# blachlylab/fade

Hardware: NVIDIA B200
Metric: annotate_reads_per_sec (higher is better)
Workload: dtype int16

## Files before the change

fade_b200/csrc/fadegpu.cu:

```cuda
#include <cuda_runtime.h>
#include <algorithm>
#include <cstdio>
#include <cstdlib>
#include <cstring>
#include <new>
#include <chrono>
#include <condition_variable>
#include <deque>
#include <functional>
#include <exception>
#include <mutex>
#include <thread>
#include <string>
#include <vector>
#ifdef _OPENMP
#include <omp.h>
#endif
#include "../../include/fadegpu.h"
#include "kernels.cuh"

using namespace fade;

static_assert(FADEGPU_MAX_OPS == OPS_CAP, "ABI ops capacity must match the kernels");
static_assert(sizeof(AlnOut) == 32 + 4 * OPS_CAP, "AlnOut layout");
static_assert(sizeof(AlnDesc) == 40, "AlnDesc layout");
static_assert(sizeof(PairResult) == sizeof(fadegpu_pair_result) && sizeof(fadegpu_pair_result) == 32, "fadegpu_pair_result layout");
static_assert(PAIR_R_OVERSIZE == FADEGPU_R_OVERSIZE, "oversize flag");

static thread_local std::string g_last_error;

constexpr int MAX_SETS = 4;

struct fadegpu_ctx {
    int device = 0;
    cudaStream_t stream = nullptr;
    fadegpu_params p{};
    SwConsts k{};
    int32_t n_contigs = 0;
    std::vector<std::string> names;
    std::vector<int64_t> clen, coff;
    int64_t total_bases = 0, padded_bases = 0;
    uint32_t *d_two = nullptr, *d_n = nullptr, *d_x = nullptr;
    int64_t *d_xpos = nullptr;
    uint8_t *d_xchr = nullptr;
    int64_t n_x = 0;
    size_t ref_bytes = 0;
    cudaStream_t tstream = nullptr;
    unsigned next_set = 0;
    struct ScratchSet {
        cudaEvent_t ev_fill = nullptr, ev_trace = nullptr;
        bool used = false;
        uint32_t *d_ck = nullptr;
        size_t ck_bytes = 0;
        uint8_t *d_gen = nullptr;
        size_t gen_bytes = 0;
        unsigned int *d_cursor = nullptr;
        uint8_t *d_trace = nullptr;
        size_t trace_bytes = 0;
        unsigned int *d_qcount = nullptr;
    } scratch[MAX_SETS];
    int n_sets = 3;
    uint32_t *d_alu = nullptr;
    int sm_count = 148;
    int host_threads = 1;
    cudaStream_t stream2 = nullptr;
    cudaStream_t stream3 = nullptr;
    int64_t *d_clen = nullptr, *d_coff = nullptr;
    std::string err;
    std::thread worker;
    std::mutex q_mu;
    std::condition_variable q_cv, done_cv;
    std::deque<std::pair<fadegpu_batch *, int64_t>> jobs;
    bool worker_stop = false, worker_busy = false;
    std::mutex submit_mu;
    std::vector<fadegpu_batch *> batches;
    struct PairBufs {
        fadegpu_batch *b = nullptr;
        char *h_stage = nullptr, *d_raw = nullptr;
        size_t stage_bytes = 0, raw_bytes = 0;
        uint32_t *d_two = nullptr, *d_n = nullptr, *d_x = nullptr, *d_chunk_x = nullptr;
        size_t two_bytes = 0, n_bytes = 0, x_bytes = 0, chunk_bytes = 0;
        int64_t *d_xpos = nullptr, *d_clen = nullptr, *d_coff = nullptr;
        size_t xpos_bytes = 0, clen_bytes = 0, coff_bytes = 0;
        uint8_t *d_xchr = nullptr;
        size_t xchr_bytes = 0;
        uint32_t *d_spill = nullptr, *d_ops = nullptr;
        size_t spill_bytes = 0, ops_bytes = 0;
        fadegpu_pair_result *d_res = nullptr;
        size_t res_bytes = 0;
        int32_t *d_bad = nullptr;
    } pairs;
};

struct AlnTmp {
    int64_t start;
    int64_t so;
    int32_t read, tlen, cls, qlen, tid, key;
    uint32_t clip_left, clip_right;
};

struct Launch {
    int R;
    int aln_first, n_aln;
    int item_first, n_items;
    int tw_stride;
    int nblk_max;
    int qmax, tmax;
};

struct fadegpu_batch {
    fadegpu_ctx *ctx = nullptr;
    fadegpu_batch_view v{};
    AlnDesc *h_aln = nullptr, *d_aln = nullptr;
    WarpItem *h_items = nullptr, *d_items = nullptr;
    uint8_t *h_seq = nullptr, *d_seq = nullptr;
    AlnOut *h_out = nullptr, *d_out = nullptr;
    uint32_t *d_flags = nullptr;
    uint2 *d_fillres = nullptr;
    int64_t cap_items = 0, cap_seq = 0;
    std::vector<Launch> plan;
    int64_t n_reads = 0, n_aln = 0, n_items = 0, seq_bytes = 0;
    int qmax_all = 0, tmax_all = 0;
    fadegpu_stats st{};
    cudaEvent_t ev[6] = { nullptr, nullptr, nullptr, nullptr, nullptr, nullptr };
    bool in_flight = false;
    std::vector<std::vector<AlnTmp>> tl_aln;
    std::vector<uint32_t> order;
    int32_t *h_ridx = nullptr;
    std::vector<AlnTmp> all_aln;
    std::vector<int32_t> cnt;
    std::vector<int64_t> soff, aln_start;
    std::vector<int32_t> sorted_tlen;
    bool dev_binning = false;
    uint8_t *d_in_seq4 = nullptr;
    int64_t *d_in_seq_off = nullptr, *d_in_pos = nullptr, *d_start = nullptr, *d_aln_start = nullptr;
    int32_t *d_in_lq = nullptr, *d_in_tid = nullptr, *d_in_alen = nullptr, *d_in_cl = nullptr, *d_in_cr = nullptr;
    int32_t *d_key = nullptr, *d_tlen = nullptr, *d_hist = nullptr, *d_keybase = nullptr, *d_cursor = nullptr;
    int32_t *d_ridx = nullptr;
    uint8_t *d_rflags = nullptr;
    uint8_t *d_gate = nullptr;
    const uint4 *d_view_meta = nullptr;
    int32_t *d_over = nullptr, *h_over = nullptr;
    unsigned long long *d_stats = nullptr;
    int32_t *h_hist = nullptr, *h_keybase = nullptr;
    unsigned long long *h_stats = nullptr;
    int64_t *h_aln_start = nullptr;
    uint8_t *h_c_seq4 = nullptr;
    int64_t *h_c_seq_off = nullptr, *h_c_pos = nullptr;
    int32_t *h_c_lq = nullptr, *h_c_tid = nullptr, *h_c_alen = nullptr, *h_c_cl = nullptr, *h_c_cr = nullptr, *h_c_read = nullptr;
    int32_t *d_in_read = nullptr;
    int64_t n_c = 0, seq_c = 0;
    bool pulled = false;
    int64_t *d_src_off = nullptr;
    const uint8_t *d_view_seq4 = nullptr;
    std::vector<int32_t> idx;
    BinArgs ba{};
    bool ba_valid = false;
    AlnDesc *d_aln_scratch = nullptr;
    int64_t *d_i64_scratch = nullptr;
    cudaEvent_t ev_prep = nullptr, ev_ready = nullptr;
    int mode = 0;
    int64_t job_seq_bytes = 0;
    cudaEvent_t ev_kernels = nullptr;
    bool queued = false;
    int submit_rc = 0;
    std::string submit_err;
};

extern "C" { static void drain_submits(fadegpu_ctx *c); }

namespace {

std::mutex g_err_mu;

int fail(fadegpu_ctx *ctx, int code, const std::string &msg)
{
    std::lock_guard<std::mutex> g(g_err_mu);
    if (ctx) ctx->err = msg;
    g_last_error = msg;
    return code;
}

int cuda_fail(fadegpu_ctx *ctx, cudaError_t e, const char *what)
{
    std::string m = std::string(what) + ": " + cudaGetErrorString(e);
    return fail(ctx, e == cudaErrorMemoryAllocation ? FADEGPU_E_OOM : FADEGPU_E_CUDA, m);
}

#define CU(ctx, call)                                              \
    do {                                                           \
        cudaError_t e__ = (call);                                  \
        if (e__ != cudaSuccess) return cuda_fail(ctx, e__, #call); \
    } while (0)

template <typename T>
void free_host(T *&p) { if (p) cudaFreeHost(p); p = nullptr; }
template <typename T>
void free_dev(T *&p) { if (p) cudaFree(p); p = nullptr; }

void free_reference(fadegpu_ctx *c)
{
    free_dev(c->d_two); free_dev(c->d_n); free_dev(c->d_x); free_dev(c->d_xpos); free_dev(c->d_xchr);
    free_dev(c->d_clen); free_dev(c->d_coff);
    c->n_x = 0; c->ref_bytes = 0; c->n_contigs = 0; c->total_bases = c->padded_bases = 0;
    c->names.clear(); c->clen.clear(); c->coff.clear();
}

int upload_contig_tables(fadegpu_ctx *c)
{
    const size_t nb = std::max<size_t>(1, (size_t)c->n_contigs) * sizeof(int64_t);
    CU(c, cudaMalloc(&c->d_clen, nb)); CU(c, cudaMalloc(&c->d_coff, nb));
    if (c->n_contigs > 0) {
        CU(c, cudaMemcpy(c->d_clen, c->clen.data(), (size_t)c->n_contigs * 8, cudaMemcpyHostToDevice));
        CU(c, cudaMemcpy(c->d_coff, c->coff.data(), (size_t)c->n_contigs * 8, cudaMemcpyHostToDevice));
    }
    return 0;
}

RefDev ref_dev(const fadegpu_ctx *c)
{
    RefDev r;
    r.planes.two = c->d_two; r.planes.nmask = c->d_n; r.planes.xmask = c->d_x;
    r.xpos = c->d_xpos; r.xchr = c->d_xchr; r.n_x = c->n_x;
    return r;
}

int cls_rank(int cls)
{
    for (int k = 0; k < N_ROW_CLASSES; ++k) if (ROW_CLASSES[k] == cls) return k;
    return N_ROW_CLASSES;
}

int class_of(const fadegpu_ctx *c, int qlen, int tlen)
{
    if (c->p.flags & FADEGPU_F_FORCE_GENERIC) return 0;
    if (qlen > QMAX_FAST || tlen > TMAX_PACKED) return 0;
    for (int k = 0; k < N_ROW_CLASSES; ++k) if (qlen <= FG * ROW_CLASSES[k]) return ROW_CLASSES[k];
    return 0;
}

size_t ck_words_of(int R) { return (size_t)(2 * R + 2); }

int ensure_dev(fadegpu_ctx *c, void **p, size_t *have, size_t bytes)
{
    if (bytes <= *have) return 0;
    if (*p) cudaFree(*p);
    *p = nullptr; *have = 0;
    CU(c, cudaMalloc(p, bytes));
    *have = bytes;
    return 0;
}

size_t align256(size_t x) { return (x + 255) & ~(size_t)255; }

size_t trace_scratch_bytes(int R, int64_t n)
{
    return align256((size_t)n * sizeof(LaneCtl)) + 2 * align256((size_t)n * 8) +
           align256((size_t)((n + 1) / 2) * trace_tile_bytes(R));
}

constexpr int GEN_SLOTS_MAX = 8192;
constexpr size_t GEN_BUDGET = (size_t)4 << 30;

size_t gen_slot_bytes(int qmax, int tmax)
{
    size_t b = (size_t)8 * qmax + (((size_t)qmax + 15) & ~(size_t)15) + (size_t)qmax * tmax;
    return (b + 15) & ~(size_t)15;
}

int build_plan(fadegpu_ctx *c, fadegpu_batch *b, int64_t n_aln, const int64_t *cls_first, const int32_t *sorted_tlen,
               int qmax_all, int tmax_all, int gen_qmax, int gen_tmax)
{
    int64_t n_items = 0;
    size_t ck_needed = 0, gen_needed = 0, trace_needed = 0;
    b->plan.clear();
    b->st.n_generic = 0;
    for (int rk = 0; rk <= N_ROW_CLASSES; ++rk) {
        const int R = rk < N_ROW_CLASSES ? ROW_CLASSES[rk] : 0;
        const int64_t first_aln = cls_first[rk], last_aln = cls_first[rk + 1];
        if (last_aln <= first_aln) continue;
        if (R == 0) {
            Launch L{};
            L.R = 0; L.aln_first = (int)first_aln; L.n_aln = (int)(last_aln - first_aln); L.qmax = gen_qmax; L.tmax = gen_tmax;
            b->plan.push_back(L);
            gen_needed = std::max(gen_needed, gen_slot_bytes(gen_qmax, gen_tmax));
            b->st.n_generic += last_aln - first_aln;
            continue;
        }
        const size_t cw = ck_words_of(R);
        int64_t a0 = first_aln;
        while (a0 < last_aln) {
            Launch L{};
            L.R = R; L.aln_first = (int)a0; L.item_first = (int)n_items; L.qmax = qmax_all; L.tmax = tmax_all;
            size_t words = 0;
            int nblk_max = 1;
            int64_t a1 = a0;
            while (a1 < last_aln) {
                const int nblk = num_blocks(sorted_tlen[a1]);
                const size_t wds = (size_t)(nblk - 1) * cw * 32;
                if (a1 > a0 && (words + wds) * 4 > (size_t)c->p.scratch_bytes) break;
                if (n_items >= b->cap_items) return fail(c, FADEGPU_E_STATE, "fadegpu_submit: internal error (item capacity)");
                WarpItem &it = b->h_items[n_items++];
                it.ck_off = (int64_t)words;
                it.first = (int32_t)(a1 - a0);
                it.nblk = (int16_t)nblk;
                it.pad = 0;
                it.nsteps = sorted_tlen[a1] + FG - 1;
                words += wds;
                nblk_max = std::max(nblk_max, nblk);
                a1 = std::min<int64_t>(a1 + 8, last_aln);
            }
            L.n_aln = (int)(a1 - a0);
            L.n_items = (int)(n_items - L.item_first);
            L.tw_stride = tw_stride_for(nblk_max);
            L.nblk_max = nblk_max;
            ck_needed = std::max(ck_needed, words * 4);
            trace_needed = std::max(trace_needed, trace_scratch_bytes(R, L.n_aln));
            b->plan.push_back(L);
            a0 = a1;
        }
    }
    b->n_aln = n_aln; b->n_items = n_items;
    b->qmax_all = qmax_all; b->tmax_all = tmax_all;
    b->st.n_aligned = n_aln;
    b->st.scratch_bytes = (int64_t)ck_needed;
    if (n_aln > 0) gen_needed = std::max(gen_needed, gen_slot_bytes(qmax_all, tmax_all));
    for (int l = 0; l < (b->plan.empty() ? 0 : c->n_sets); ++l) {
        fadegpu_ctx::ScratchSet &ln = c->scratch[l];
        if (ck_needed) { int rc = ensure_dev(c, (void **)&ln.d_ck, &ln.ck_bytes, ck_needed); if (rc) return rc; }
        if (trace_needed) { int rc = ensure_dev(c, (void **)&ln.d_trace, &ln.trace_bytes, trace_needed); if (rc) return rc; }
        if (gen_needed) {
            const size_t want = std::min<size_t>(GEN_BUDGET, gen_needed * 1024);
            int rc = ensure_dev(c, (void **)&ln.d_gen, &ln.gen_bytes, std::max(want, gen_needed));
            if (rc) return rc;
        }
    }
    return 0;
}

struct PlanTarget {
    RefDev ref;
    int tags_only;
    uint32_t *ops_spill;
    int ops_cap;
};

PlanTarget batch_target(const fadegpu_ctx *c)
{
    return PlanTarget{ ref_dev(c), (c->p.flags & FADEGPU_F_TAGS_ONLY) ? 1 : 0, nullptr, 0 };
}

int run_plan(fadegpu_ctx *c, fadegpu_batch *b, const PlanTarget &pt, float *fill_ms, float *trace_ms, float *gen_ms,
             int *launches, cudaEvent_t dep)
{
    const bool timed = fill_ms != nullptr;
    cudaEvent_t e0 = nullptr, e1 = nullptr, e2 = nullptr;
    if (timed) {
        CU(c, cudaEventCreate(&e0)); CU(c, cudaEventCreate(&e1)); CU(c, cudaEventCreate(&e2));
        *fill_ms = *trace_ms = *gen_ms = 0.f;
    }
    int nl = 0;
    cudaStream_t sf = c->stream, st = c->tstream;
    if (dep) CU(c, cudaStreamWaitEvent(sf, dep, 0));
    for (const Launch &L : b->plan) {
        fadegpu_ctx::ScratchSet &ln = c->scratch[c->next_set++ % (unsigned)c->n_sets];
        if (ln.used) CU(c, cudaStreamWaitEvent(sf, ln.ev_trace, 0));
        ln.used = true;
        const uint8_t *seq = b->dev_binning ? b->d_in_seq4 : b->d_seq;
        if (L.R != 0) {
            KernelArgs a;
            a.aln = b->d_aln + L.aln_first;
            a.n_aln = L.n_aln;
            a.items = b->d_items + L.item_first;
            a.n_items = L.n_items;
            a.seq = seq;
            a.ref = pt.ref;
            a.ck = ln.d_ck;
            a.fillres = b->d_fillres + (size_t)L.item_first * 32;
            a.aln_flags = b->d_flags + L.aln_first;
            a.out = b->d_out + L.aln_first;
            a.k = c->k;
            a.min_length = c->p.min_length;
            a.tw_stride = L.tw_stride;
            {
                uint8_t *p = ln.d_trace;
                a.state = reinterpret_cast<LaneCtl *>(p); p += align256((size_t)L.n_aln * sizeof(LaneCtl));
                a.queue[0] = reinterpret_cast<unsigned long long *>(p); p += align256((size_t)L.n_aln * 8);
                a.queue[1] = reinterpret_cast<unsigned long long *>(p); p += align256((size_t)L.n_aln * 8);
                a.tiles = reinterpret_cast<uint32_t *>(p);
                a.qcount = ln.d_qcount;
                a.round = 0;
                a.max_rounds = L.nblk_max + FG;
                a.tags_only = pt.tags_only;
            }
            a.ops_spill = pt.ops_spill ? pt.ops_spill + (size_t)L.aln_first * pt.ops_cap : nullptr;
            a.ops_cap = pt.ops_cap;
            CU(c, cudaMemsetAsync(a.aln_flags, 0, (size_t)L.n_aln * sizeof(uint32_t), sf));
            CU(c, cudaMemsetAsync(ln.d_qcount, 0, 2 * sizeof(unsigned int), sf));
            if (timed) CU(c, cudaEventRecord(e0, sf));
            CU(c, launch_fill(L.R, a, sf));
            if (timed) CU(c, cudaEventRecord(e1, sf));
            CU(c, cudaEventRecord(ln.ev_fill, sf));
            CU(c, cudaStreamWaitEvent(st, ln.ev_fill, 0));
            nl += 1;
            CU(c, launch_trace(L.R, a, st, c->sm_count, &nl));
            GenericArgs ga;
            ga.aln = a.aln; ga.n_aln = L.n_aln; ga.aln_flags = a.aln_flags; ga.seq = a.seq; ga.ref = a.ref;
            ga.out = a.out; ga.cursor = ln.d_cursor; ga.scratch = ln.d_gen;
            ga.qmax = L.qmax; ga.tmax = L.tmax;
            ga.slot_bytes = (int64_t)gen_slot_bytes(L.qmax, L.tmax);
            ga.n_slots = (int)std::max<size_t>(1, std::min<size_t>(GEN_SLOTS_MAX, ln.gen_bytes / (size_t)ga.slot_bytes));
            ga.chunk = 64;
            ga.open = c->p.gap_open; ga.extend = c->p.gap_extend; ga.match = c->p.match; ga.mismatch = c->p.mismatch;
            ga.min_length = c->p.min_length; ga.tags_only = pt.tags_only;
            ga.ops_spill = a.ops_spill; ga.ops_cap = a.ops_cap;
            if (timed) CU(c, cudaEventRecord(e2, st));
            CU(c, cudaMemsetAsync(ln.d_cursor, 0, sizeof(unsigned int), st));
            CU(c, launch_generic(ga, ga.n_slots, st));
            nl += 1;
            if (timed) {
                cudaEvent_t e3;
                CU(c, cudaEventCreate(&e3));
                CU(c, cudaEventRecord(e3, st));
                CU(c, cudaEventSynchronize(e3));
                float t;
                cudaEventElapsedTime(&t, e0, e1); *fill_ms += t;
                cudaEventElapsedTime(&t, e1, e2); *trace_ms += t;
                cudaEventElapsedTime(&t, e2, e3); *gen_ms += t;
                cudaEventDestroy(e3);
            }
            CU(c, cudaEventRecord(ln.ev_trace, st));
        } else {
            GenericArgs ga;
            ga.aln = b->d_aln + L.aln_first; ga.n_aln = L.n_aln; ga.aln_flags = nullptr; ga.seq = seq;
            ga.ref = pt.ref; ga.out = b->d_out + L.aln_first; ga.cursor = ln.d_cursor; ga.scratch = ln.d_gen;
            ga.qmax = L.qmax; ga.tmax = L.tmax;
            ga.slot_bytes = (int64_t)gen_slot_bytes(L.qmax, L.tmax);
            ga.n_slots = (int)std::max<size_t>(1, std::min<size_t>(GEN_SLOTS_MAX, ln.gen_bytes / (size_t)ga.slot_bytes));
            ga.n_slots = std::min(ga.n_slots, std::max(L.n_aln, 1));
            ga.chunk = 1;
            ga.open = c->p.gap_open; ga.extend = c->p.gap_extend; ga.match = c->p.match; ga.mismatch = c->p.mismatch;
            ga.min_length = c->p.min_length; ga.tags_only = pt.tags_only;
            ga.ops_spill = pt.ops_spill ? pt.ops_spill + (size_t)L.aln_first * pt.ops_cap : nullptr;
            ga.ops_cap = pt.ops_cap;
            CU(c, cudaEventRecord(ln.ev_fill, sf));
            CU(c, cudaStreamWaitEvent(st, ln.ev_fill, 0));
            if (timed) CU(c, cudaEventRecord(e0, st));
            CU(c, cudaMemsetAsync(ln.d_cursor, 0, sizeof(unsigned int), st));
            CU(c, launch_generic(ga, ga.n_slots, st));
            nl += 1;
            if (timed) {
                CU(c, cudaEventRecord(e1, st));
                CU(c, cudaEventSynchronize(e1));
                float t;
                cudaEventElapsedTime(&t, e0, e1); *gen_ms += t;
            }
            CU(c, cudaEventRecord(ln.ev_trace, st));
        }
    }
    if (timed) { cudaEventDestroy(e0); cudaEventDestroy(e1); cudaEventDestroy(e2); }
    CU(c, cudaEventRecord(b->ev[5], sf));
    CU(c, cudaEventRecord(b->ev_kernels, b->plan.empty() ? sf : st));
    if (launches) *launches = nl;
    return 0;
}

int join_kernels(fadegpu_ctx *c, fadegpu_batch *b, cudaStream_t s)
{
    CU(c, cudaStreamWaitEvent(s, b->ev_kernels, 0));
    return 0;
}

}

extern "C" {

int fadegpu_abi_version(void) { return FADEGPU_ABI_VERSION; }

int fadegpu_device_count(int *n)
{
    if (!n) return fail(nullptr, FADEGPU_E_ARG, "fadegpu_device_count: null argument");
    int c = 0;
    cudaError_t e = cudaGetDeviceCount(&c);
    if (e != cudaSuccess) { *n = 0; return cuda_fail(nullptr, e, "cudaGetDeviceCount"); }
    *n = c;
    return FADEGPU_OK;
}

int fadegpu_default_params(fadegpu_params *p)
{
    if (!p) return fail(nullptr, FADEGPU_E_ARG, "fadegpu_default_params: null argument");
    p->window_size = 300;
    p->min_length = 5;
    p->gap_open = 10;
    p->gap_extend = 2;
    p->match = 2;
    p->mismatch = -3;
    p->flags = 0;
    p->scratch_bytes = 0;
    p->host_threads = 0;
    p->reserved = 0;
    return FADEGPU_OK;
}

const char *fadegpu_last_error(const fadegpu_ctx *ctx)
{
    static thread_local std::string copy;
    std::lock_guard<std::mutex> g(g_err_mu);
    copy = ctx ? ctx->err : g_last_error;
    return copy.c_str();
}

int fadegpu_create(int device, const fadegpu_params *p, fadegpu_ctx **out)
{
    if (!out) return fail(nullptr, FADEGPU_E_ARG, "fadegpu_create: null out");
    *out = nullptr;
    fadegpu_params pp;
    fadegpu_default_params(&pp);
    if (p) pp = *p;
    if (pp.gap_open < pp.gap_extend || pp.gap_extend <= 0 || pp.match <= 0 || pp.mismatch > 0 ||
        pp.match > 100 || pp.mismatch < -100 || pp.gap_open > 1000 || pp.window_size < 0)
        return fail(nullptr, FADEGPU_E_ARG, "fadegpu_create: unsupported scoring / window parameters");
    setenv("CUDA_DEVICE_MAX_CONNECTIONS", "32", 0);
    int n = 0;
    cudaError_t e = cudaGetDeviceCount(&n);
    if (e != cudaSuccess || n <= 0)
        return fail(nullptr, FADEGPU_E_NODEV, std::string("fadegpu_create: no CUDA device (") +
                                                  (e != cudaSuccess ? cudaGetErrorString(e) : "count 0") + "); there is no CPU fallback");
    if (device < 0 || device >= n) return fail(nullptr, FADEGPU_E_ARG, "fadegpu_create: bad device index");
    fadegpu_ctx *c = new (std::nothrow) fadegpu_ctx();
    if (!c) return fail(nullptr, FADEGPU_E_OOM, "fadegpu_create: out of host memory");
    c->device = device;
    c->p = pp;
    if (c->p.scratch_bytes <= 0) c->p.scratch_bytes = (int64_t)8 << 30;
    {
        int hw = 1;
#ifdef _OPENMP
        hw = std::max(1, omp_get_num_procs());
#endif
        c->host_threads = c->p.host_threads > 0 ? std::min(c->p.host_threads, 4 * hw) : hw;
    }
    c->k = make_consts(pp.gap_open, pp.gap_extend, pp.match, pp.mismatch);
    if (pp.flags & FADEGPU_F_NO_SHORTCUT) c->k.shortcut = 0;
    int prio[4] = { 0, -1, -2, -2 };
    if (const char *pv = getenv("FADEGPU_PRIO")) sscanf(pv, "%d,%d,%d,%d", &prio[0], &prio[1], &prio[2], &prio[3]);
    if ((e = cudaSetDevice(device)) != cudaSuccess || (e = cudaStreamCreateWithPriority(&c->stream, cudaStreamNonBlocking, prio[0])) != cudaSuccess ||
        (e = cudaMalloc(&c->d_alu, 64)) != cudaSuccess ||
        (e = cudaStreamCreateWithPriority(&c->tstream, cudaStreamNonBlocking, prio[1])) != cudaSuccess ||
        (e = cudaStreamCreateWithPriority(&c->stream2, cudaStreamNonBlocking, prio[2])) != cudaSuccess ||
        (e = cudaStreamCreateWithPriority(&c->stream3, cudaStreamNonBlocking, prio[3])) != cudaSuccess ||
        (e = cudaDeviceGetAttribute(&c->sm_count, cudaDevAttrMultiProcessorCount, device)) != cudaSuccess) {
        int rc = cuda_fail(nullptr, e, "fadegpu_create");
        delete c;
        return rc;
    }
    if (const char *ev = getenv("FADEGPU_SCRATCH_SETS")) c->n_sets = std::min(MAX_SETS, std::max(2, atoi(ev)));
    for (int l = 0; l < c->n_sets; ++l) {
        fadegpu_ctx::ScratchSet &ln = c->scratch[l];
        if ((e = cudaEventCreateWithFlags(&ln.ev_fill, cudaEventDisableTiming)) != cudaSuccess ||
            (e = cudaEventCreateWithFlags(&ln.ev_trace, cudaEventDisableTiming)) != cudaSuccess ||
            (e = cudaMalloc(&ln.d_cursor, sizeof(unsigned int))) != cudaSuccess ||
            (e = cudaMalloc(&ln.d_qcount, 2 * sizeof(unsigned int))) != cudaSuccess) {
            int rc = cuda_fail(nullptr, e, "fadegpu_create");
            fadegpu_destroy(c);
            return rc;
        }
    }
    *out = c;
    return FADEGPU_OK;
}

void fadegpu_destroy(fadegpu_ctx *c)
{
    if (!c) return;
    if (c->worker.joinable()) {
        { std::lock_guard<std::mutex> lk(c->q_mu); c->worker_stop = true; }
        c->q_cv.notify_all();
        c->worker.join();
    }
    cudaSetDevice(c->device);
    {
        fadegpu_ctx::PairBufs &pb = c->pairs;
        if (pb.b) fadegpu_free_batch(pb.b);
        free_host(pb.h_stage);
        free_dev(pb.d_raw); free_dev(pb.d_two); free_dev(pb.d_n); free_dev(pb.d_x); free_dev(pb.d_chunk_x);
        free_dev(pb.d_xpos); free_dev(pb.d_xchr); free_dev(pb.d_clen); free_dev(pb.d_coff); free_dev(pb.d_spill);
        free_dev(pb.d_ops); free_dev(pb.d_res); free_dev(pb.d_bad);
    }
    if (c->stream) cudaStreamSynchronize(c->stream);
    if (c->stream2) { cudaStreamSynchronize(c->stream2); cudaStreamDestroy(c->stream2); }
    if (c->stream3) { cudaStreamSynchronize(c->stream3); cudaStreamDestroy(c->stream3); }
    free_reference(c);
    if (c->tstream) { cudaStreamSynchronize(c->tstream); cudaStreamDestroy(c->tstream); }
    for (auto &ln : c->scratch) {
        if (ln.ev_fill) cudaEventDestroy(ln.ev_fill);
        if (ln.ev_trace) cudaEventDestroy(ln.ev_trace);
    }
    for (auto &ln : c->scratch) { free_dev(ln.d_ck); free_dev(ln.d_gen); free_dev(ln.d_cursor); free_dev(ln.d_trace); free_dev(ln.d_qcount); }
    free_dev(c->d_alu);
    if (c->stream) cudaStreamDestroy(c->stream);
    delete c;
}

int fadegpu_load_reference(fadegpu_ctx *c, int32_t n_contigs, const char *const *names,
                           const int64_t *lengths, const char *const *seqs)
{
    if (!c) return fail(nullptr, FADEGPU_E_ARG, "fadegpu_load_reference: null ctx");
    if (n_contigs <= 0 || !lengths || !seqs) return fail(c, FADEGPU_E_ARG, "fadegpu_load_reference: bad arguments");
    drain_submits(c);
    std::lock_guard<std::mutex> submit_guard(c->submit_mu);
    CU(c, cudaSetDevice(c->device));
    { CU(c, cudaStreamSynchronize(c->stream)); CU(c, cudaStreamSynchronize(c->tstream)); }
    free_reference(c);
    c->n_contigs = n_contigs;
    int64_t off = 0, total = 0;
    for (int t = 0; t < n_contigs; ++t) {
        if (lengths[t] < 0 || !seqs[t]) { free_reference(c); return fail(c, FADEGPU_E_ARG, "fadegpu_load_reference: bad contig"); }
        c->names.emplace_back(names && names[t] ? names[t] : "");
        c->clen.push_back(lengths[t]);
        c->coff.push_back(off);
        total += lengths[t];
        off += (lengths[t] + 31) & ~(int64_t)31;
    }
    c->total_bases = total;
    c->padded_bases = off + 32;
    const size_t w2 = (size_t)(c->padded_bases / 16), w1 = (size_t)(c->padded_bases / 32);
    std::vector<uint32_t> two, nm, xm;
    try { two.assign(w2, 0u); nm.assign(w1, 0u); xm.assign(w1, 0u); }
    catch (...) { free_reference(c); return fail(c, FADEGPU_E_OOM, "fadegpu_load_reference: out of host memory"); }
    uint8_t lut[256];
    for (int i = 0; i < 256; ++i) lut[i] = 8;
    lut['A'] = lut['a'] = 0; lut['C'] = lut['c'] = 1; lut['T'] = lut['t'] = 2; lut['G'] = lut['g'] = 3;
    lut['N'] = lut['n'] = 4;
    for (int t = 0; t < n_contigs; ++t) {
        const unsigned char *s = reinterpret_cast<const unsigned char *>(seqs[t]);
        const int64_t len = lengths[t], base = c->coff[t];
        const int64_t nwords = (len + 31) / 32;
#pragma omp parallel for schedule(static) num_threads(std::max(1, c->host_threads))
        for (int64_t wd = 0; wd < nwords; ++wd) {
            uint32_t a0 = 0, a1 = 0, n = 0, x = 0;
            const int64_t p0 = wd * 32;
            const int lim = (int)std::min<int64_t>(32, len - p0);
            for (int b = 0; b < lim; ++b) {
                const uint8_t v = lut[s[p0 + b]];
                const uint32_t code = v & 3u;
                if (b < 16) a0 |= code << (2 * b); else a1 |= code << (2 * (b - 16));
                n |= (uint32_t)((v >> 2) & 1u) << b;
                x |= (uint32_t)((v >> 3) & 1u) << b;
            }
            const size_t gw = (size_t)((base + p0) / 32);
            two[2 * gw] = a0; two[2 * gw + 1] = a1; nm[gw] = n; xm[gw] = x;
        }
    }
    std::vector<int64_t> xpos;
    std::vector<uint8_t> xchr;
    for (int t = 0; t < n_contigs; ++t) {
        const unsigned char *s = reinterpret_cast<const unsigned char *>(seqs[t]);
        const int64_t len = lengths[t], base = c->coff[t];
        for (int64_t wd = 0; wd * 32 < len; ++wd) {
            const uint32_t x = xm[(size_t)((base + wd * 32) / 32)];
            if (!x) continue;
            for (int b = 0; b < 32; ++b)
                if ((x >> b) & 1u) {
                    unsigned char ch = s[wd * 32 + b];
                    if (ch >= 'a' && ch <= 'z') ch = (unsigned char)(ch - 32);
                    xpos.push_back(base + wd * 32 + b);
                    xchr.push_back(ch);
                }
        }
    }
    c->n_x = (int64_t)xpos.size();
    cudaError_t e;
    if ((e = cudaMalloc(&c->d_two, w2 * 4)) != cudaSuccess || (e = cudaMalloc(&c->d_n, w1 * 4)) != cudaSuccess ||
        (e = cudaMalloc(&c->d_x, w1 * 4)) != cudaSuccess ||
        (e = cudaMalloc(&c->d_xpos, std::max<size_t>(1, xpos.size()) * 8)) != cudaSuccess ||
        (e = cudaMalloc(&c->d_xchr, std::max<size_t>(1, xchr.size()))) != cudaSuccess) {
        free_reference(c);
        return cuda_fail(c, e, "fadegpu_load_reference: cudaMalloc");
    }
    CU(c, cudaMemcpy(c->d_two, two.data(), w2 * 4, cudaMemcpyHostToDevice));
    CU(c, cudaMemcpy(c->d_n, nm.data(), w1 * 4, cudaMemcpyHostToDevice));
    CU(c, cudaMemcpy(c->d_x, xm.data(), w1 * 4, cudaMemcpyHostToDevice));
    if (!xpos.empty()) {
        CU(c, cudaMemcpy(c->d_xpos, xpos.data(), xpos.size() * 8, cudaMemcpyHostToDevice));
        CU(c, cudaMemcpy(c->d_xchr, xchr.data(), xchr.size(), cudaMemcpyHostToDevice));
    }
    c->ref_bytes = w2 * 4 + 2 * w1 * 4 + xpos.size() * 9;
    { int rc = upload_contig_tables(c); if (rc) return rc; }
    return FADEGPU_OK;
}

int fadegpu_share_reference(fadegpu_ctx *dst, const fadegpu_ctx *src)
{
    if (!dst || !src) return fail(dst, FADEGPU_E_ARG, "fadegpu_share_reference: null ctx");
    if (!src->d_two) return fail(dst, FADEGPU_E_STATE, "fadegpu_share_reference: source has no reference");
    drain_submits(dst);
    std::lock_guard<std::mutex> submit_guard(dst->submit_mu);
    CU(dst, cudaSetDevice(dst->device));
    { CU(dst, cudaStreamSynchronize(dst->stream)); CU(dst, cudaStreamSynchronize(dst->tstream)); }
    if (dst->device != src->device) {
        int can = 0;
        if (cudaDeviceCanAccessPeer(&can, dst->device, src->device) == cudaSuccess && can) {
            const cudaError_t pe = cudaDeviceEnablePeerAccess(src->device, 0);
            if (pe != cudaSuccess) cudaGetLastError();
        }
    }
    free_reference(dst);
    dst->n_contigs = src->n_contigs; dst->names = src->names; dst->clen = src->clen; dst->coff = src->coff;
    dst->total_bases = src->total_bases; dst->padded_bases = src->padded_bases; dst->n_x = src->n_x;
    const size_t w2 = (size_t)(src->padded_bases / 16), w1 = (size_t)(src->padded_bases / 32);
    const size_t nx = std::max<size_t>(1, (size_t)src->n_x);
    CU(dst, cudaMalloc(&dst->d_two, w2 * 4)); CU(dst, cudaMalloc(&dst->d_n, w1 * 4)); CU(dst, cudaMalloc(&dst->d_x, w1 * 4));
    CU(dst, cudaMalloc(&dst->d_xpos, nx * 8)); CU(dst, cudaMalloc(&dst->d_xchr, nx));
    CU(dst, cudaMemcpyPeer(dst->d_two, dst->device, src->d_two, src->device, w2 * 4));
    CU(dst, cudaMemcpyPeer(dst->d_n, dst->device, src->d_n, src->device, w1 * 4));
    CU(dst, cudaMemcpyPeer(dst->d_x, dst->device, src->d_x, src->device, w1 * 4));
    if (src->n_x > 0) {
        CU(dst, cudaMemcpyPeer(dst->d_xpos, dst->device, src->d_xpos, src->device, (size_t)src->n_x * 8));
        CU(dst, cudaMemcpyPeer(dst->d_xchr, dst->device, src->d_xchr, src->device, (size_t)src->n_x));
    }
    dst->ref_bytes = src->ref_bytes;
    { int rc = upload_contig_tables(dst); if (rc) return rc; }
    return FADEGPU_OK;
}

int fadegpu_reference_info(const fadegpu_ctx *c, int32_t *n_contigs, int64_t *total_bases, int64_t *device_bytes)
{
    if (!c) return fail(nullptr, FADEGPU_E_ARG, "fadegpu_reference_info: null ctx");
    if (n_contigs) *n_contigs = c->n_contigs;
    if (total_bases) *total_bases = c->total_bases;
    if (device_bytes) *device_bytes = (int64_t)c->ref_bytes;
    return FADEGPU_OK;
}

void fadegpu_free_batch(fadegpu_batch *b)
{
    if (!b) return;
    fadegpu_ctx *c = b->ctx;
    if (c) {
        std::unique_lock<std::mutex> lk(c->q_mu);
        c->done_cv.wait(lk, [&] { return !b->queued; });
        c->batches.erase(std::remove(c->batches.begin(), c->batches.end(), b), c->batches.end());
    }
    if (c) { cudaSetDevice(c->device); if (c->stream) cudaStreamSynchronize(c->stream); if (c->tstream) cudaStreamSynchronize(c->tstream); if (c->stream2) cudaStreamSynchronize(c->stream2); if (c->stream3) cudaStreamSynchronize(c->stream3); }
    fadegpu_batch_view &v = b->v;
    free_host(v.seq4); free_host(v.seq_off); free_host(v.l_qseq); free_host(v.tid); free_host(v.pos);
    free_host(v.aligned_len); free_host(v.clip_left); free_host(v.clip_right);
    free_host(v.gate); free_host(v.meta);
    free_host(v.flags); free_host(v.score); free_host(v.beg_query); free_host(v.end_query);
    free_host(v.beg_ref); free_host(v.end_ref); free_host(v.win_start); free_host(v.n_ops); free_host(v.ops);
    free_host(b->h_aln); free_host(b->h_items); free_host(b->h_seq); free_host(b->h_out); free_host(b->h_ridx);
    free_dev(b->d_aln); free_dev(b->d_items); free_dev(b->d_seq); free_dev(b->d_out); free_dev(b->d_flags);
    free_dev(b->d_fillres);
    free_dev(b->d_in_seq4); free_dev(b->d_in_seq_off); free_dev(b->d_in_pos); free_dev(b->d_in_lq); free_dev(b->d_in_tid);
    free_dev(b->d_in_alen); free_dev(b->d_in_cl); free_dev(b->d_in_cr); free_dev(b->d_key); free_dev(b->d_tlen); free_dev(b->d_start);
    free_dev(b->d_aln_start); free_dev(b->d_hist); free_dev(b->d_keybase); free_dev(b->d_cursor);
    free_dev(b->d_ridx); free_dev(b->d_rflags);
    free_dev(b->d_gate); free_dev(b->d_over); free_host(b->h_over); free_dev(b->d_stats);
    free_host(b->h_hist); free_host(b->h_keybase); free_host(b->h_stats); free_host(b->h_aln_start);
    free_host(b->h_c_seq4); free_host(b->h_c_seq_off); free_host(b->h_c_pos); free_host(b->h_c_lq); free_host(b->h_c_tid);
    free_host(b->h_c_alen); free_host(b->h_c_cl); free_host(b->h_c_cr); free_host(b->h_c_read); free_dev(b->d_in_read); free_dev(b->d_src_off);
    free_dev(b->d_aln_scratch); free_dev(b->d_i64_scratch);
    if (b->ev_prep) cudaEventDestroy(b->ev_prep);
    if (b->ev_ready) cudaEventDestroy(b->ev_ready);
    if (b->ev_kernels) cudaEventDestroy(b->ev_kernels);
    for (auto &e : b->ev) if (e) { cudaEventDestroy(e); e = nullptr; }
    delete b;
}

int fadegpu_alloc_batch(fadegpu_ctx *c, int64_t max_reads, int64_t max_seq_bytes, fadegpu_batch **out)
{
    if (!c || !out) return fail(c, FADEGPU_E_ARG, "fadegpu_alloc_batch: null argument");
    *out = nullptr;
    if (max_reads <= 0 || max_seq_bytes <= 0 || max_reads > (int64_t)1 << 30)
        return fail(c, FADEGPU_E_ARG, "fadegpu_alloc_batch: bad sizes");
    CU(c, cudaSetDevice(c->device));
    fadegpu_batch *b = new (std::nothrow) fadegpu_batch();
    if (!b) return fail(c, FADEGPU_E_OOM, "fadegpu_alloc_batch: out of host memory");
    b->ctx = c;
    fadegpu_batch_view &v = b->v;
    v.max_reads = max_reads; v.max_seq_bytes = max_seq_bytes;
    const size_t n = (size_t)max_reads;
    b->cap_items = (max_reads + 7) / 8 + 8;
    b->cap_seq = max_seq_bytes + 16;
    cudaError_t e = cudaSuccess;
    auto H = [&](auto **p, size_t bytes) { if (e == cudaSuccess) e = cudaHostAlloc((void **)p, std::max<size_t>(bytes, 16), cudaHostAllocDefault); };
    auto D = [&](auto **p, size_t bytes) { if (e == cudaSuccess) e = cudaMalloc((void **)p, std::max<size_t>(bytes, 16)); };
    H(&v.seq4, (size_t)max_seq_bytes + 16); H(&v.seq_off, (n + 1) * 8); H(&v.l_qseq, n * 4); H(&v.tid, n * 4);
    H(&v.pos, n * 8); H(&v.aligned_len, n * 4); H(&v.clip_left, n * 4); H(&v.clip_right, n * 4);
    H(&v.flags, n); H(&v.gate, n); H(&v.meta, n * sizeof(fadegpu_read_meta));
    if (!(c->p.flags & FADEGPU_F_NO_SCATTER)) {
        H(&v.score, n * 4); H(&v.beg_query, n * 4); H(&v.end_query, n * 4); H(&v.beg_ref, n * 4);
        H(&v.end_ref, n * 4); H(&v.win_start, n * 8); H(&v.n_ops, n * 4); H(&v.ops, n * 4 * FADEGPU_MAX_OPS);
    }
    H(&b->h_items, (size_t)b->cap_items * sizeof(WarpItem));
    H(&b->h_out, n * sizeof(AlnOut)); H(&b->h_ridx, n * 4);
    D(&b->d_aln, n * sizeof(AlnDesc)); D(&b->d_items, (size_t)b->cap_items * sizeof(WarpItem));
    D(&b->d_out, n * sizeof(AlnOut)); D(&b->d_flags, n * 4);
    D(&b->d_fillres, (size_t)b->cap_items * 32 * sizeof(uint2));
    D(&b->d_in_seq4, (size_t)max_seq_bytes + 32 * n + 16); D(&b->d_in_seq_off, (n + 1) * 8); D(&b->d_in_pos, n * 8);
    D(&b->d_in_read, n * 4);
    D(&b->d_in_lq, n * 4); D(&b->d_in_tid, n * 4); D(&b->d_in_alen, n * 4); D(&b->d_in_cl, n * 4); D(&b->d_in_cr, n * 4);
    D(&b->d_key, n * 4); D(&b->d_tlen, n * 4); D(&b->d_start, n * 8); D(&b->d_aln_start, n * 8);
    D(&b->d_hist, (size_t)BIN_KEYS * 4); D(&b->d_keybase, (size_t)BIN_KEYS * 4); D(&b->d_cursor, (size_t)BIN_KEYS * 4);
    D(&b->d_ridx, n * 4); D(&b->d_rflags, n);
    D(&b->d_gate, n); D(&b->d_over, (size_t)OVER_CAP * 4); H(&b->h_over, (size_t)OVER_CAP * 4);
    D(&b->d_stats, 128); D(&b->d_src_off, n * 8);
    H(&b->h_hist, (size_t)BIN_KEYS * 4); H(&b->h_keybase, (size_t)BIN_KEYS * 4); H(&b->h_stats, 128); H(&b->h_aln_start, n * 8);
    if (e == cudaSuccess) e = cudaHostGetDevicePointer((void **)&b->d_view_seq4, v.seq4, 0);
    if (e == cudaSuccess) e = cudaHostGetDevicePointer((void **)&b->d_view_meta, v.meta, 0);
    if (e == cudaSuccess) e = cudaEventCreate(&b->ev_prep);
    if (e == cudaSuccess) e = cudaEventCreate(&b->ev_ready);
    if (e == cudaSuccess) e = cudaEventCreateWithFlags(&b->ev_kernels, cudaEventDisableTiming);
    for (auto &ev : b->ev) if (e == cudaSuccess) e = cudaEventCreate(&ev);
    if (e != cudaSuccess) {
        int rc = cuda_fail(c, e, "fadegpu_alloc_batch");
        fadegpu_free_batch(b);
        return rc;
    }
    { std::lock_guard<std::mutex> lk(c->q_mu); c->batches.push_back(b); }
    *out = b;
    return FADEGPU_OK;
}

int fadegpu_get_batch_view(fadegpu_batch *b, fadegpu_batch_view *view)
{
    if (!b || !view) return fail(b ? b->ctx : nullptr, FADEGPU_E_ARG, "fadegpu_get_batch_view: null argument");
    *view = b->v;
    return FADEGPU_OK;
}

static int ensure_host_staging(fadegpu_ctx *c, fadegpu_batch *b)
{
    if (b->h_aln) return 0;
    const size_t n = (size_t)b->v.max_reads;
    CU(c, cudaHostAlloc((void **)&b->h_aln, n * sizeof(AlnDesc), cudaHostAllocDefault));
    CU(c, cudaHostAlloc((void **)&b->h_seq, (size_t)b->cap_seq, cudaHostAllocDefault));
    CU(c, cudaMalloc((void **)&b->d_seq, (size_t)b->cap_seq));
    return 0;
}

static int gather_reads(fadegpu_ctx *c, fadegpu_batch *b, int64_t n, const fadegpu_inputs &in);
static int queue_submit(fadegpu_ctx *c, fadegpu_batch *b, int64_t n, int mode, int64_t seq_bytes);
static bool batch_in_flight(fadegpu_ctx *c, fadegpu_batch *b);

int fadegpu_submit_inputs(fadegpu_ctx *c, fadegpu_batch *b, int64_t n_reads, const fadegpu_inputs *in)
{
    if (!c || !b || b->ctx != c || !in) return fail(c, FADEGPU_E_ARG, "fadegpu_submit: bad ctx/batch/inputs");
    if (!c->d_two) return fail(c, FADEGPU_E_STATE, "fadegpu_submit: no reference loaded");
    if (batch_in_flight(c, b)) return fail(c, FADEGPU_E_STATE, "fadegpu_submit: batch already in flight (call fadegpu_wait)");
    if (n_reads < 0 || n_reads > b->v.max_reads) return fail(c, FADEGPU_E_ARG, "fadegpu_submit: n_reads out of range");
    if (n_reads > 0 && (!in->seq4 || !in->seq_off || !in->l_qseq || !in->tid || !in->pos || !in->aligned_len ||
                        !in->clip_left || !in->clip_right))
        return fail(c, FADEGPU_E_ARG, "fadegpu_submit: null input array");
    if (!(c->p.flags & FADEGPU_F_HOST_BINNING)) {
        CU(c, cudaSetDevice(c->device));
        { int rc = gather_reads(c, b, n_reads, *in); if (rc) return rc; }
        return queue_submit(c, b, n_reads, 0 , 0);
    }
    std::lock_guard<std::mutex> submit_guard(c->submit_mu);
    CU(c, cudaSetDevice(c->device));
    { int rc = ensure_host_staging(c, b); if (rc) return rc; }
    const int64_t n = n_reads;
    b->n_reads = n;
    b->plan.clear();
    b->dev_binning = false;
    memset(&b->st, 0, sizeof(b->st));
    b->st.n_reads = n;

    const auto t_begin = std::chrono::steady_clock::now();
    auto ms_since = [](std::chrono::steady_clock::time_point t0) {
        return std::chrono::duration<float, std::milli>(std::chrono::steady_clock::now() - t0).count();
    };
    const int nthr = std::max(1, c->host_threads);
    b->st.host_threads = nthr;
    if ((int)b->tl_aln.size() < nthr) b->tl_aln.resize((size_t)nthr);
    const uint32_t floor_u = (uint32_t)c->p.min_length;
    const int64_t W = c->p.window_size;
    const int64_t seq_total = n > 0 ? in->seq_off[n] : 0;
    int64_t cells = 0, n_over = 0;
    int bad = 0;
#pragma omp parallel num_threads(nthr) reduction(+ : cells) reduction(| : bad)
    {
        int tix = 0, tn = 1;
#ifdef _OPENMP
        tix = omp_get_thread_num(); tn = omp_get_num_threads();
#endif
        std::vector<AlnTmp> &loc = b->tl_aln[(size_t)tix];
        loc.clear();
        const int64_t lo = n * tix / tn, hi = n * (tix + 1) / tn;
        for (int64_t r = lo; r < hi; ++r) {
            const uint32_t cl = (uint32_t)in->clip_left[r], cr = (uint32_t)in->clip_right[r];
            const bool need = (cl != 0 && !(cl <= floor_u)) || (cr != 0 && !(cr <= floor_u));
            if (!need) continue;
            const int32_t tid = in->tid[r];
            const int32_t ql = in->l_qseq[r];
            if (tid < 0 || tid >= c->n_contigs || ql <= 0) continue;
            const int64_t so = in->seq_off[r];
            if (so < 0 || so + (ql + 1) / 2 > seq_total) { bad = 1; continue; }
            int64_t start = in->pos[r] - W;
            if (start < 0) start = 0;
            int64_t end = in->pos[r] + (int64_t)in->aligned_len[r] + W;
            if (end > c->clen[tid]) end = c->clen[tid];
            if (end <= start) continue;
            if (end - start > 0x7fffffff || (end - start) * (int64_t)ql > ((int64_t)1 << 31)) {
#pragma omp critical(fadegpu_oversize)
                { if (n_over < OVER_CAP) b->h_over[n_over] = (int32_t)r; ++n_over; }
                continue;
            }
            const int tlen = (int)(end - start);
            const int cls = class_of(c, ql, tlen);
            const int rk = cls_rank(cls);
            const int key = bin_key(rk, tlen);
            loc.push_back(AlnTmp{ start, so, (int32_t)r, tlen, cls, ql, tid, key, cl, cr });
            cells += (int64_t)ql * tlen;
        }
    }
    if (bad & 1) return fail(c, FADEGPU_E_ARG, "fadegpu_submit: seq_off / l_qseq inconsistent");
    b->st.cells = cells;
    b->st.n_oversize = n_over;
    b->st.host_classify_ms = ms_since(t_begin);
    const auto t_sort = std::chrono::steady_clock::now();

    int64_t n_aln = 0;
    for (int t = 0; t < nthr; ++t) n_aln += (int64_t)b->tl_aln[(size_t)t].size();
    std::vector<AlnTmp> &all = b->all_aln;
    std::vector<uint32_t> &order = b->order;
    all.resize((size_t)n_aln);
    order.resize((size_t)n_aln);
    const int KEYS = BIN_KEYS;
    std::vector<int32_t> &hist = b->cnt;
    hist.resize((size_t)nthr * (size_t)(KEYS + 1));
    std::vector<int64_t> toff((size_t)nthr + 1, 0);
    std::vector<int> kmin((size_t)nthr, KEYS), kmax((size_t)nthr, -1);
    for (int t = 0; t < nthr; ++t) toff[(size_t)t + 1] = toff[(size_t)t] + (int64_t)b->tl_aln[(size_t)t].size();
#pragma omp parallel num_threads(nthr)
    {
        int t = 0;
#ifdef _OPENMP
        t = omp_get_thread_num();
#endif
        if (t < nthr) {
            const auto &loc = b->tl_aln[(size_t)t];
            int32_t *h = hist.data() + (size_t)t * (size_t)(KEYS + 1);
            memset(h, 0, (size_t)(KEYS + 1) * sizeof(int32_t));
            if (!loc.empty()) memcpy(all.data() + toff[(size_t)t], loc.data(), loc.size() * sizeof(AlnTmp));
            int lo = KEYS, hi = -1;
            for (const AlnTmp &a : loc) { ++h[a.key]; lo = std::min(lo, a.key); hi = std::max(hi, a.key); }
            kmin[(size_t)t] = lo; kmax[(size_t)t] = hi;
        }
    }
    int64_t cls_first[N_ROW_CLASSES + 2];
    {
        int64_t run = 0;
        int klo = KEYS, khi = -1;
        for (int t = 0; t < nthr; ++t) { klo = std::min(klo, kmin[(size_t)t]); khi = std::max(khi, kmax[(size_t)t]); }
        for (int rk = 0; rk <= N_ROW_CLASSES; ++rk) cls_first[rk] = -1;
        for (int key = std::max(klo, 0); key <= khi; ++key) {
            const int rk = key / KEYS_PER_CLASS;
            if (cls_first[rk] < 0) cls_first[rk] = run;
            for (int t = 0; t < nthr; ++t) {
                int32_t &hv = hist[(size_t)t * (size_t)(KEYS + 1) + (size_t)key];
                const int32_t c0 = hv;
                hv = (int32_t)run;
                run += c0;
            }
        }
        cls_first[N_ROW_CLASSES + 1] = n_aln;
        for (int rk = N_ROW_CLASSES; rk >= 0; --rk) if (cls_first[rk] < 0) cls_first[rk] = cls_first[rk + 1];
    }
#pragma omp parallel num_threads(nthr)
    {
        int t = 0;
#ifdef _OPENMP
        t = omp_get_thread_num();
#endif
        if (t < nthr) {
            int32_t *h = hist.data() + (size_t)t * (size_t)(KEYS + 1);
            const int64_t o0 = toff[(size_t)t], o1 = toff[(size_t)t + 1];
            for (int64_t kx = o0; kx < o1; ++kx) order[(size_t)h[all[(size_t)kx].key]++] = (uint32_t)kx;
        }
    }

    b->st.host_sort_ms = ms_since(t_sort);
    const auto t_gather = std::chrono::steady_clock::now();
    std::vector<int64_t> &soff = b->soff;
    soff.resize((size_t)n_aln + 1);
    int qmax_all = 1, tmax_all = 1;
    {
        int64_t o = 0;
        for (int64_t kx = 0; kx < n_aln; ++kx) {
            soff[(size_t)kx] = o;
            const AlnTmp &a = all[order[(size_t)kx]];
            o += (a.qlen + 1) / 2;
            qmax_all = std::max(qmax_all, a.qlen);
            tmax_all = std::max(tmax_all, a.tlen);
        }
        soff[(size_t)n_aln] = o;
    }
    const int64_t seq_bytes = soff[(size_t)n_aln];
    if (seq_bytes > b->cap_seq) return fail(c, FADEGPU_E_ARG, "fadegpu_submit: read bases exceed max_seq_bytes");
    b->aln_start.resize((size_t)n_aln);
#pragma omp parallel for schedule(static) num_threads(nthr)
    for (int64_t kx = 0; kx < n_aln; ++kx) {
        const AlnTmp &a = all[order[(size_t)kx]];
        if (kx + 8 < n_aln) {
            const uint8_t *pf = in->seq4 + all[order[(size_t)kx + 8]].so;
            __builtin_prefetch(pf); __builtin_prefetch(pf + 64);
        }
        AlnDesc &d = b->h_aln[kx];
        const int ql = a.qlen;
        d.gstart = c->coff[a.tid] + a.start;
        d.seq_off = soff[(size_t)kx];
        d.tlen = a.tlen;
        d.qlen = ql;
        d.clip_left = a.clip_left;
        d.clip_right = a.clip_right;
        d.read = a.read;
        d.pad = 0;
        b->aln_start[(size_t)kx] = a.start;
        memcpy(b->h_seq + d.seq_off, in->seq4 + a.so, (size_t)((ql + 1) / 2));
    }

    b->st.host_gather_ms = ms_since(t_gather);
    std::vector<int32_t> &stl = b->sorted_tlen;
    stl.resize((size_t)n_aln);
    for (int64_t kx = 0; kx < n_aln; ++kx) {
        const AlnTmp &t = all[order[(size_t)kx]];
        stl[(size_t)kx] = (t.cls != 0 && t.tlen > TMAX_FAST) ? key_tlen(t.key % KEYS_PER_CLASS) : t.tlen;
    }
    int gq = 1, gt = 1;
    for (int64_t kx = cls_first[N_ROW_CLASSES]; kx < n_aln; ++kx) { gq = std::max(gq, b->h_aln[kx].qlen); gt = std::max(gt, b->h_aln[kx].tlen); }
    b->seq_bytes = seq_bytes;
    { int rc = build_plan(c, b, n_aln, cls_first, stl.data(), qmax_all, tmax_all, gq, gt); if (rc) return rc; }
    const int64_t n_items = b->n_items;

    CU(c, cudaEventRecord(b->ev[0], c->stream2));
    if (n_aln > 0) {
        CU(c, cudaMemcpyAsync(b->d_aln, b->h_aln, (size_t)n_aln * sizeof(AlnDesc), cudaMemcpyHostToDevice, c->stream2));
        if (n_items > 0)
            CU(c, cudaMemcpyAsync(b->d_items, b->h_items, (size_t)n_items * sizeof(WarpItem), cudaMemcpyHostToDevice, c->stream2));
        CU(c, cudaMemcpyAsync(b->d_seq, b->h_seq, (size_t)seq_bytes, cudaMemcpyHostToDevice, c->stream2));
    }
    b->st.h2d_bytes = n_aln * (int64_t)sizeof(AlnDesc) + n_items * (int64_t)sizeof(WarpItem) + seq_bytes;
    CU(c, cudaEventRecord(b->ev_ready, c->stream2));
    CU(c, cudaStreamWaitEvent(c->stream, b->ev_ready, 0));
    CU(c, cudaEventRecord(b->ev[1], c->stream));
    int nl = 0;
    { int rc = run_plan(c, b, batch_target(c), nullptr, nullptr, nullptr, &nl, b->ev_ready); if (rc) return rc; }
    b->st.kernel_launches = nl;
    { int rc = join_kernels(c, b, c->stream3); if (rc) return rc; }
    CU(c, cudaEventRecord(b->ev[2], c->stream3));
    if (n_aln > 0)
        CU(c, cudaMemcpyAsync(b->h_out, b->d_out, (size_t)n_aln * sizeof(AlnOut), cudaMemcpyDeviceToHost, c->stream3));
    b->st.d2h_bytes = n_aln * (int64_t)sizeof(AlnOut);
    CU(c, cudaEventRecord(b->ev[3], c->stream3));
    b->in_flight = true;
    b->st.host_submit_ms = ms_since(t_begin);
    return FADEGPU_OK;
}

static int gather_reads(fadegpu_ctx *c, fadegpu_batch *b, int64_t n, const fadegpu_inputs &in)
{
    const auto t0 = std::chrono::steady_clock::now();
    if (!b->h_c_seq4) {
        const size_t m = (size_t)b->v.max_reads;
        auto H = [&](auto **p, size_t bytes) { return cudaHostAlloc((void **)p, std::max<size_t>(bytes, 16), cudaHostAllocDefault); };
        CU(c, H(&b->h_c_seq4, (size_t)b->cap_seq + 16)); CU(c, H(&b->h_c_seq_off, (m + 1) * 8)); CU(c, H(&b->h_c_pos, m * 8));
        CU(c, H(&b->h_c_lq, m * 4)); CU(c, H(&b->h_c_tid, m * 4)); CU(c, H(&b->h_c_alen, m * 4));
        CU(c, H(&b->h_c_cl, m * 4)); CU(c, H(&b->h_c_cr, m * 4)); CU(c, H(&b->h_c_read, m * 4));
    }
    const uint32_t floor_u = (uint32_t)c->p.min_length;
    const int T = (int)std::max<int64_t>(1, std::min<int64_t>(std::min(c->host_threads, 64), n / 4096));
    std::vector<int64_t> cnt((size_t)T + 1, 0), bytes((size_t)T + 1, 0);
    b->idx.resize((size_t)std::max<int64_t>(n, 1));
    int32_t *const idx = b->idx.data();
#pragma omp parallel for schedule(static, 1) num_threads(T)
    for (int t = 0; t < T; ++t) {
        const int64_t r0 = n * t / T, r1 = n * (t + 1) / T;
        int64_t k = 0, by = 0;
        int32_t *out = idx + r0;
        for (int64_t r = r0; r < r1; ++r) {
            const uint32_t cl = (uint32_t)in.clip_left[r], cr = (uint32_t)in.clip_right[r];
            const int nd = (int)(cl > floor_u) | (int)(cr > floor_u);
            const int ql = in.l_qseq[r];
            out[k] = (int32_t)r;
            k += nd;
            by += nd ? (int64_t)((ql > 0 ? ql + 1 : 0) >> 1) : 0;
        }
        cnt[(size_t)t + 1] = k; bytes[(size_t)t + 1] = by;
    }
    for (int t = 0; t < T; ++t) { cnt[(size_t)t + 1] += cnt[(size_t)t]; bytes[(size_t)t + 1] += bytes[(size_t)t]; }
    if (bytes[(size_t)T] > b->cap_seq) return fail(c, FADEGPU_E_ARG, "fadegpu_submit: sequence bytes exceed max_seq_bytes");
    int bad = 0;
#pragma omp parallel for schedule(static, 1) reduction(| : bad) num_threads(T)
    for (int t = 0; t < T; ++t) {
        const int32_t *ix = idx + n * t / T;
        const int64_t m = cnt[(size_t)t + 1] - cnt[(size_t)t];
        int64_t k = cnt[(size_t)t], by = bytes[(size_t)t];
        constexpr int D = 12;
        for (int64_t i = 0; i < m; ++i) {
            if (i + 2 * D < m) {
                const int64_t rr = ix[i + 2 * D];
                __builtin_prefetch(&in.seq_off[rr]); __builtin_prefetch(&in.pos[rr]); __builtin_prefetch(&in.tid[rr]);
                __builtin_prefetch(&in.aligned_len[rr]); __builtin_prefetch(&in.l_qseq[rr]);
            }
            if (i + D < m) {
                const uint8_t *p = in.seq4 + in.seq_off[ix[i + D]];
                __builtin_prefetch(p); __builtin_prefetch(p + 64);
            }
            const int64_t r = ix[i];
            const int ql = in.l_qseq[r];
            const int64_t nb = ql > 0 ? (ql + 1) / 2 : 0;
            if (in.seq_off[r] < 0 || (nb > 0 && in.seq_off[r + 1] - in.seq_off[r] < nb)) bad = 1;
            else memcpy(b->h_c_seq4 + by, in.seq4 + in.seq_off[r], (size_t)nb);
            b->h_c_seq_off[k] = by; b->h_c_pos[k] = in.pos[r];
            b->h_c_lq[k] = ql; b->h_c_tid[k] = in.tid[r]; b->h_c_alen[k] = in.aligned_len[r];
            b->h_c_cl[k] = in.clip_left[r]; b->h_c_cr[k] = in.clip_right[r]; b->h_c_read[k] = (int32_t)r;
            ++k; by += nb;
        }
    }
    if (bad) return fail(c, FADEGPU_E_ARG, "fadegpu_submit: seq_off / l_qseq inconsistent");
    b->n_c = cnt[(size_t)T]; b->seq_c = bytes[(size_t)T];
    b->h_c_seq_off[b->n_c] = b->seq_c;
    b->n_reads = n;
    b->st.host_gather_ms = std::chrono::duration<float, std::milli>(std::chrono::steady_clock::now() - t0).count();
    b->st.host_threads = T;
    return FADEGPU_OK;
}

enum SubmitMode : int {
    MODE_GATHERED = 0,
    MODE_VIEW = 1,
    MODE_COMPACT = 2
};

static int plan_from_histogram(fadegpu_ctx *c, fadegpu_batch *b, int64_t n_aln)
{
    int64_t cls_first[N_ROW_CLASSES + 2];
    std::vector<int32_t> &stl = b->sorted_tlen;
    stl.resize((size_t)n_aln);
    int64_t run = 0;
    for (int rk = 0; rk <= N_ROW_CLASSES; ++rk) {
        cls_first[rk] = run;
        const int k0 = rk * KEYS_PER_CLASS, k1 = k0 + KEYS_PER_CLASS;
        for (int key = k0; key < k1; ++key) {
            const int32_t cnt = b->h_hist[key];
            b->h_keybase[key] = (int32_t)run;
            if (!cnt) continue;
            const int tl = rk == N_ROW_CLASSES ? (int)b->h_stats[5] : key_tlen(key - k0);
            std::fill(stl.begin() + run, stl.begin() + run + cnt, tl);
            run += cnt;
        }
    }
    cls_first[N_ROW_CLASSES + 1] = run;
    if (run != n_aln) return fail(c, FADEGPU_E_CUDA, "fadegpu_submit: internal error (histogram does not add up)");
    return build_plan(c, b, n_aln, cls_first, stl.data(), std::max(1, (int)b->h_stats[2]), std::max(1, (int)b->h_stats[3]),
                      std::max(1, (int)b->h_stats[4]), std::max(1, (int)b->h_stats[5]));
}

static int submit_device_binning(fadegpu_ctx *c, fadegpu_batch *b, int64_t n_reads, int mode, int64_t seq_bytes)
{
    const auto t_begin = std::chrono::steady_clock::now();
    auto ms_since = [](std::chrono::steady_clock::time_point t0) {
        return std::chrono::duration<float, std::milli>(std::chrono::steady_clock::now() - t0).count();
    };
    const bool pull = mode != MODE_GATHERED;
    b->n_reads = n_reads;
    b->plan.clear();
    b->dev_binning = true;
    b->mode = mode;
    {
        const float g = pull ? 0.f : b->st.host_gather_ms; const int32_t th = pull ? 1 : b->st.host_threads;
        memset(&b->st, 0, sizeof(b->st));
        b->st.host_gather_ms = g; b->st.host_threads = th;
    }
    b->st.n_reads = n_reads;
    b->n_aln = 0; b->n_items = 0;
    b->ba_valid = false;
    cudaStream_t s2 = c->stream2;
    CU(c, cudaEventRecord(b->ev[0], s2));
    b->pulled = pull;
    const fadegpu_batch_view &v = b->v;
    const int64_t n = pull ? n_reads : b->n_c;
    const int64_t seq_total = mode == MODE_COMPACT ? seq_bytes : mode == MODE_VIEW ? (n > 0 ? v.seq_off[n] : 0) : b->seq_c;
    int64_t n_aln = 0, up_bytes = 0;
    memset(b->h_stats, 0, 128);
    if (n > 0) {
        auto up = [&](void *d, const void *h, size_t bytes) { up_bytes += (int64_t)bytes; return cudaMemcpyAsync(d, h, bytes, cudaMemcpyHostToDevice, s2); };
        if (mode == MODE_COMPACT) CU(c, up(b->d_gate, v.gate, (size_t)n));
        else {
            if (!pull) CU(c, up(b->d_in_seq4, b->h_c_seq4, (size_t)seq_total));
            CU(c, up(b->d_in_seq_off, pull ? v.seq_off : b->h_c_seq_off, (size_t)(n + 1) * 8));
            CU(c, up(b->d_in_lq, pull ? v.l_qseq : b->h_c_lq, (size_t)n * 4)); CU(c, up(b->d_in_tid, pull ? v.tid : b->h_c_tid, (size_t)n * 4));
            CU(c, up(b->d_in_pos, pull ? v.pos : b->h_c_pos, (size_t)n * 8)); CU(c, up(b->d_in_alen, pull ? v.aligned_len : b->h_c_alen, (size_t)n * 4));
            CU(c, up(b->d_in_cl, pull ? v.clip_left : b->h_c_cl, (size_t)n * 4)); CU(c, up(b->d_in_cr, pull ? v.clip_right : b->h_c_cr, (size_t)n * 4));
            if (!pull) CU(c, up(b->d_in_read, b->h_c_read, (size_t)n * 4));
        }
        CU(c, cudaMemsetAsync(b->d_hist, 0, (size_t)BIN_KEYS * 4, s2));
        CU(c, cudaMemsetAsync(b->d_cursor, 0, (size_t)BIN_KEYS * 4, s2));
        CU(c, cudaMemsetAsync(b->d_stats, 0, 128, s2));
        BinArgs ba{};
        ba.seq4 = b->d_in_seq4; ba.seq_off = b->d_in_seq_off; ba.l_qseq = b->d_in_lq; ba.tid = b->d_in_tid; ba.pos = b->d_in_pos;
        ba.aligned_len = b->d_in_alen; ba.clip_left = b->d_in_cl; ba.clip_right = b->d_in_cr;
        ba.read = pull ? nullptr : b->d_in_read;
        ba.seq_cursor = pull ? b->d_stats + 8 : nullptr; ba.src_off = b->d_src_off;
        ba.gate = mode == MODE_COMPACT ? b->d_gate : nullptr; ba.host_meta = b->d_view_meta; ba.over_list = b->d_over;
        ba.n = n; ba.seq_total = seq_total; ba.clen = c->d_clen; ba.coff = c->d_coff; ba.n_contigs = c->n_contigs;
        ba.window = c->p.window_size; ba.min_length = c->p.min_length; ba.flags = c->p.flags;
        ba.key = b->d_key; ba.tlen = b->d_tlen; ba.start = b->d_start; ba.hist = b->d_hist; ba.stats = b->d_stats;
        ba.keybase = b->d_keybase; ba.cursor = b->d_cursor; ba.aln = b->d_aln; ba.aln_start = b->d_aln_start;
        b->ba = ba; b->ba_valid = true;
        CU(c, launch_bin_classify(ba, c->sm_count, s2));
        CU(c, cudaMemcpyAsync(b->h_hist, b->d_hist, (size_t)BIN_KEYS * 4, cudaMemcpyDeviceToHost, s2));
        CU(c, cudaMemcpyAsync(b->h_stats, b->d_stats, 128, cudaMemcpyDeviceToHost, s2));
        CU(c, cudaMemcpyAsync(b->h_over, b->d_over, (size_t)OVER_CAP * 4, cudaMemcpyDeviceToHost, s2));
        CU(c, cudaEventRecord(b->ev_prep, s2));
        CU(c, cudaEventSynchronize(b->ev_prep));
        b->st.host_classify_ms = ms_since(t_begin);
        if (b->h_stats[6] & 1ull) return fail(c, FADEGPU_E_ARG, "fadegpu_submit: seq_off / l_qseq inconsistent");
        b->st.n_oversize = (int64_t)b->h_stats[11];
        const auto t_sort = std::chrono::steady_clock::now();
        n_aln = (int64_t)b->h_stats[1];
        b->st.cells = (int64_t)b->h_stats[0];
        { int rc = plan_from_histogram(c, b, n_aln); if (rc) return rc; }
        b->st.host_sort_ms = ms_since(t_sort);
        if (n_aln > 0) {
            CU(c, up(b->d_keybase, b->h_keybase, (size_t)BIN_KEYS * 4));
            if (b->n_items > 0) CU(c, up(b->d_items, b->h_items, (size_t)b->n_items * sizeof(WarpItem)));
            CU(c, launch_bin_scatter(ba, c->sm_count, s2));
            if (pull) CU(c, launch_seq_pull(b->d_view_seq4, b->d_aln, b->d_src_off, (int)n_aln, b->d_in_seq4, c->sm_count, s2));
        }
    }
    if (n_reads > 0) {
        CU(c, cudaMemsetAsync(b->d_rflags, 0, (size_t)n_reads, s2));
        CU(c, cudaMemsetAsync(b->d_ridx, 0xff, (size_t)n_reads * 4, s2));
    }
    CU(c, cudaEventRecord(b->ev_ready, s2));
    CU(c, cudaEventRecord(b->ev[4], s2));
    CU(c, cudaStreamWaitEvent(c->stream, b->ev_ready, 0));
    CU(c, cudaEventRecord(b->ev[1], c->stream));
    int nl = 0;
    { int rc = run_plan(c, b, batch_target(c), nullptr, nullptr, nullptr, &nl, b->ev_ready); if (rc) return rc; }
    b->st.kernel_launches = nl + (n > 0 ? 1 : 0) + (n_aln > 0 ? (pull ? 3 : 2) : 0);
    cudaStream_t s3 = c->stream3;
    { int rc = join_kernels(c, b, s3); if (rc) return rc; }
    CU(c, cudaEventRecord(b->ev[2], s3));
    if (n_aln > 0) CU(c, launch_result_index(b->d_out, (int)n_aln, n_reads, b->d_rflags, b->d_ridx, b->d_stats + 7, c->sm_count, s3));
    if (n_reads > 0) {
        CU(c, cudaMemcpyAsync(b->v.flags, b->d_rflags, (size_t)n_reads, cudaMemcpyDeviceToHost, s3));
        CU(c, cudaMemcpyAsync(b->h_ridx, b->d_ridx, (size_t)n_reads * 4, cudaMemcpyDeviceToHost, s3));
    }
    if (n_aln > 0) CU(c, cudaMemcpyAsync(b->h_stats + 7, b->d_stats + 7, 8, cudaMemcpyDeviceToHost, s3));
    if (n_aln > 0) {
        CU(c, cudaMemcpyAsync(b->h_out, b->d_out, (size_t)n_aln * sizeof(AlnOut), cudaMemcpyDeviceToHost, s3));
        CU(c, cudaMemcpyAsync(b->h_aln_start, b->d_aln_start, (size_t)n_aln * 8, cudaMemcpyDeviceToHost, s3));
    }
    b->st.h2d_bytes = up_bytes + (pull ? (int64_t)b->h_stats[10] * (int64_t)sizeof(fadegpu_read_meta) : 0);
    b->st.d2h_bytes = n_aln * (int64_t)(sizeof(AlnOut) + 8) + n_reads * 5 + (n > 0 ? (int64_t)BIN_KEYS * 4 + 128 + OVER_CAP * 4 : 0);
    if (pull && n_aln > 0) CU(c, cudaMemcpyAsync(b->h_stats + 8, b->d_stats + 8, 8, cudaMemcpyDeviceToHost, s3));
    CU(c, cudaEventRecord(b->ev[3], s3));
    b->in_flight = true;
    b->st.host_submit_ms = ms_since(t_begin);
    return FADEGPU_OK;
}

static void worker_main(fadegpu_ctx *c);

static fadegpu_inputs view_inputs(const fadegpu_batch_view &v)
{
    fadegpu_inputs in;
    in.seq4 = v.seq4; in.seq_off = v.seq_off; in.l_qseq = v.l_qseq; in.tid = v.tid; in.pos = v.pos;
    in.aligned_len = v.aligned_len; in.clip_left = v.clip_left; in.clip_right = v.clip_right;
    return in;
}

static int submit_stages(fadegpu_ctx *c, fadegpu_batch *b, int64_t n, int mode, int64_t seq_bytes)
{
    if (cudaSetDevice(c->device) != cudaSuccess) return fail(c, FADEGPU_E_CUDA, "fadegpu_submit: cudaSetDevice failed");
    return submit_device_binning(c, b, n, mode, seq_bytes);
}

static int queue_submit(fadegpu_ctx *c, fadegpu_batch *b, int64_t n, int mode, int64_t seq_bytes)
{
    if (c->p.flags & FADEGPU_F_SYNC_SUBMIT) {
        std::lock_guard<std::mutex> g(c->submit_mu);
        return submit_stages(c, b, n, mode, seq_bytes);
    }
    std::lock_guard<std::mutex> lk(c->q_mu);
    if (!c->worker.joinable()) {
        try { c->worker = std::thread(worker_main, c); }
        catch (const std::exception &e) { return fail(c, FADEGPU_E_STATE, std::string("fadegpu_submit: cannot start the submit thread: ") + e.what()); }
    }
    b->queued = true; b->submit_rc = 0; b->mode = mode; b->job_seq_bytes = seq_bytes;
    b->in_flight = true;
    c->jobs.emplace_back(b, n);
    c->q_cv.notify_one();
    return FADEGPU_OK;
}

static void worker_main(fadegpu_ctx *c)
{
    cudaSetDevice(c->device);
    std::unique_lock<std::mutex> lk(c->q_mu);
    for (;;) {
        c->q_cv.wait(lk, [&] { return c->worker_stop || !c->jobs.empty(); });
        if (c->jobs.empty()) return;
        auto job = c->jobs.front();
        c->jobs.pop_front();
        c->worker_busy = true;
        const int mode = job.first->mode;
        const int64_t seq_bytes = job.first->job_seq_bytes;
        lk.unlock();
        int rc;
        std::string err;
        {
            std::lock_guard<std::mutex> g(c->submit_mu);
            rc = submit_stages(c, job.first, job.second, mode, seq_bytes);
            if (rc) { std::lock_guard<std::mutex> ge(g_err_mu); err = c->err; }
        }
        lk.lock();
        job.first->submit_rc = rc;
        job.first->submit_err = err;
        job.first->queued = false;
        c->worker_busy = false;
        c->done_cv.notify_all();
    }
}

static void drain_submits(fadegpu_ctx *c)
{
    std::unique_lock<std::mutex> lk(c->q_mu);
    c->done_cv.wait(lk, [&] { return c->jobs.empty() && !c->worker_busy; });
}

static bool batch_in_flight(fadegpu_ctx *c, fadegpu_batch *b)
{
    std::lock_guard<std::mutex> lk(c->q_mu);
    return b->in_flight;
}

int fadegpu_submit(fadegpu_ctx *c, fadegpu_batch *b, int64_t n_reads)
{
    if (!c || !b || b->ctx != c) return fail(c, FADEGPU_E_ARG, "fadegpu_submit: bad ctx/batch");
    const fadegpu_batch_view &v = b->v;
    if (n_reads < 0 || n_reads > v.max_reads) return fail(c, FADEGPU_E_ARG, "fadegpu_submit: n_reads out of range");
    if (n_reads > 0 && (v.seq_off[n_reads] < 0 || v.seq_off[n_reads] > v.max_seq_bytes))
        return fail(c, FADEGPU_E_ARG, "fadegpu_submit: seq_off[n] exceeds max_seq_bytes");
    if (!(c->p.flags & FADEGPU_F_HOST_BINNING)) {
        if (!c->d_two) return fail(c, FADEGPU_E_STATE, "fadegpu_submit: no reference loaded");
        if (batch_in_flight(c, b)) return fail(c, FADEGPU_E_STATE, "fadegpu_submit: batch already in flight (call fadegpu_wait)");
        return queue_submit(c, b, n_reads, MODE_VIEW, 0);
    }
    fadegpu_inputs in = view_inputs(v);
    return fadegpu_submit_inputs(c, b, n_reads, &in);
}

int fadegpu_submit_compact(fadegpu_ctx *c, fadegpu_batch *b, int64_t n_reads, int64_t seq_bytes)
{
    if (!c || !b || b->ctx != c) return fail(c, FADEGPU_E_ARG, "fadegpu_submit_compact: bad ctx/batch");
    const fadegpu_batch_view &v = b->v;
    if (n_reads < 0 || n_reads > v.max_reads) return fail(c, FADEGPU_E_ARG, "fadegpu_submit_compact: n_reads out of range");
    if (seq_bytes < 0 || seq_bytes > v.max_seq_bytes || seq_bytes > (int64_t)0xffffffffll)
        return fail(c, FADEGPU_E_ARG, "fadegpu_submit_compact: seq_bytes out of range");
    if (!c->d_two) return fail(c, FADEGPU_E_STATE, "fadegpu_submit_compact: no reference loaded");
    if (batch_in_flight(c, b)) return fail(c, FADEGPU_E_STATE, "fadegpu_submit_compact: batch already in flight (call fadegpu_wait)");
    if (c->p.flags & FADEGPU_F_HOST_BINNING) {
        fadegpu_batch_view &w = b->v;
        for (int64_t k = 0; k < n_reads; ++k) {
            const fadegpu_read_meta &m = w.meta[k];
            w.seq_off[k] = m.seq_off; w.l_qseq[k] = m.l_qseq; w.tid[k] = m.tid; w.pos[k] = m.pos;
            w.aligned_len[k] = m.aligned_len; w.clip_left[k] = (int32_t)m.clip_left; w.clip_right[k] = (int32_t)m.clip_right;
        }
        w.seq_off[n_reads] = seq_bytes;
        fadegpu_inputs in = view_inputs(w);
        return fadegpu_submit_inputs(c, b, n_reads, &in);
    }
    return queue_submit(c, b, n_reads, MODE_COMPACT, seq_bytes);
}

int fadegpu_wait(fadegpu_ctx *c, fadegpu_batch *b)
{
    if (!c || !b || b->ctx != c) return fail(c, FADEGPU_E_ARG, "fadegpu_wait: bad ctx/batch");
    {
        std::unique_lock<std::mutex> lk(c->q_mu);
        if (!b->in_flight) { lk.unlock(); return fail(c, FADEGPU_E_STATE, "fadegpu_wait: batch not submitted"); }
        c->done_cv.wait(lk, [&] { return !b->queued; });
        b->in_flight = false;
        if (b->submit_rc) {
            const int rc = b->submit_rc;
            b->submit_rc = 0;
            lk.unlock();
            return fail(c, rc, b->submit_err);
        }
    }
    CU(c, cudaSetDevice(c->device));
    CU(c, cudaEventSynchronize(b->ev[3]));
    float t;
    if (cudaEventElapsedTime(&t, b->ev[1], b->ev[2]) == cudaSuccess) b->st.kernel_ms = t;
    if (cudaEventElapsedTime(&t, b->ev[0], b->ev[3]) == cudaSuccess) b->st.total_ms = t;
    if (b->dev_binning && b->pulled) {
        if (b->n_aln > 0) b->st.h2d_bytes += (int64_t)b->h_stats[8];
        b->pulled = false;
    }
    const auto t_scatter = std::chrono::steady_clock::now();
    fadegpu_batch_view &v = b->v;
    const int64_t n = b->n_reads;
    const bool scatter = !(c->p.flags & FADEGPU_F_NO_SCATTER) && v.score != nullptr;
    const bool walk = scatter || !b->dev_binning;
    const int nthr = walk ? (int)std::max<int64_t>(1, std::min<int64_t>(c->host_threads, b->n_aln / 8192 + 1)) : 1;
    const int64_t *wstart = b->dev_binning ? b->h_aln_start : b->aln_start.data();
    int64_t bad = 0;
    if (b->dev_binning) {
        if (b->n_aln > 0 && (int64_t)b->h_stats[7] != b->n_aln) bad = 1;
    } else {
        memset(v.flags, 0, (size_t)n);
        memset(b->h_ridx, 0xff, (size_t)n * sizeof(int32_t));
    }
#pragma omp parallel for schedule(static) reduction(+ : bad) num_threads(nthr) if (nthr > 1)
    for (int64_t k = 0; k < (walk ? b->n_aln : 0); ++k) {
        const AlnOut &o = b->h_out[k];
        const int64_t r = o.read;
        if (r < 0 || r >= n || (o.flags & 0x80000000u) || !(o.flags & 1u) || (!b->dev_binning && b->h_aln[k].read != (int32_t)r)) { ++bad; continue; }
        if (!b->dev_binning) {
            v.flags[r] = (uint8_t)(o.flags & 0xff);
            b->h_ridx[r] = (int32_t)k;
        } else if (b->h_ridx[r] != (int32_t)k) { ++bad; continue; }
        if (!scatter) continue;
        v.score[r] = o.score; v.beg_query[r] = o.beg_query; v.end_query[r] = o.end_query;
        v.beg_ref[r] = o.beg_ref; v.end_ref[r] = o.end_ref; v.n_ops[r] = o.n_ops;
        v.win_start[r] = wstart[k];
        memcpy(v.ops + (size_t)r * FADEGPU_MAX_OPS, o.ops, sizeof(o.ops));
    }
    for (int64_t k = 0; k < std::min<int64_t>(b->st.n_oversize, OVER_CAP); ++k) {
        const int64_t r = b->h_over[k];
        if (r >= 0 && r < n) v.flags[r] = FADEGPU_R_OVERSIZE;
    }
    b->st.host_wait_ms = std::chrono::duration<float, std::milli>(std::chrono::steady_clock::now() - t_scatter).count();
    if (bad) return fail(c, FADEGPU_E_CUDA, "fadegpu_wait: a kernel did not produce a result record (internal error)");
    return FADEGPU_OK;
}

int fadegpu_get_results(const fadegpu_batch *b, fadegpu_results_view *r)
{
    if (!b || !r) return fail(nullptr, FADEGPU_E_ARG, "fadegpu_get_results: null argument");
    if (b->in_flight) return fail(b->ctx, FADEGPU_E_STATE, "fadegpu_get_results: batch in flight (call fadegpu_wait)");
    static_assert(sizeof(fadegpu_result) == sizeof(AlnOut), "fadegpu_result must mirror AlnOut");
    r->n_results = b->n_aln;
    r->results = reinterpret_cast<const fadegpu_result *>(b->h_out);
    r->win_start = b->dev_binning ? b->h_aln_start : b->aln_start.data();
    r->result_index = b->h_ridx;
    return FADEGPU_OK;
}

int fadegpu_get_stats(const fadegpu_batch *b, fadegpu_stats *s)
{
    if (!b || !s) return fail(nullptr, FADEGPU_E_ARG, "fadegpu_get_stats: null argument");
    *s = b->st;
    return FADEGPU_OK;
}

int fadegpu_get_timeline(const fadegpu_batch *b, const fadegpu_batch *origin, float ms[6])
{
    if (!b || !origin || !ms || b->ctx != origin->ctx) return fail(b ? b->ctx : nullptr, FADEGPU_E_ARG, "fadegpu_get_timeline: bad arguments");
    for (int k = 0; k < 6; ++k)
        if (cudaEventElapsedTime(&ms[k], origin->ev[0], b->ev[k]) != cudaSuccess) { cudaGetLastError(); ms[k] = -1.f; }
    return FADEGPU_OK;
}

static int replay_binning(fadegpu_ctx *c, fadegpu_batch *b, cudaEvent_t *dep)
{
    *dep = nullptr;
    if (!b->dev_binning || !b->ba_valid) return 0;
    const size_t n = (size_t)b->v.max_reads;
    if (!b->d_aln_scratch) {
        CU(c, cudaMalloc((void **)&b->d_aln_scratch, n * sizeof(AlnDesc)));
        CU(c, cudaMalloc((void **)&b->d_i64_scratch, 2 * n * sizeof(int64_t)));
    }
    cudaStream_t s2 = c->stream2;
    CU(c, cudaMemsetAsync(b->d_hist, 0, (size_t)BIN_KEYS * 4, s2));
    CU(c, cudaMemsetAsync(b->d_cursor, 0, (size_t)BIN_KEYS * 4, s2));
    CU(c, cudaMemsetAsync(b->d_stats, 0, 128, s2));
    BinArgs ba = b->ba;
    ba.gate = nullptr;
    CU(c, launch_bin_classify(ba, c->sm_count, s2));
    if (b->n_aln > 0) {
        ba.aln = b->d_aln_scratch; ba.aln_start = b->d_i64_scratch; ba.src_off = b->d_i64_scratch + n;
        if (ba.seq_cursor) ba.seq_cursor = b->d_stats + 9;
        CU(c, launch_bin_scatter(ba, c->sm_count, s2));
    }
    CU(c, cudaEventRecord(b->ev_ready, s2));
    *dep = b->ev_ready;
    return 0;
}

static int replay_pass(fadegpu_ctx *c, fadegpu_batch *b)
{
    cudaEvent_t dep = nullptr;
    { int rc = replay_binning(c, b, &dep); if (rc) return rc; }
    { int rc = run_plan(c, b, batch_target(c), nullptr, nullptr, nullptr, nullptr, dep); if (rc) return rc; }
    return 0;
}

static int replay_join(fadegpu_ctx *c, fadegpu_batch *b)
{
    { int rc = join_kernels(c, b, c->stream); if (rc) return rc; }
    return 0;
}

int fadegpu_replay_batches(fadegpu_ctx *c, fadegpu_batch *const *batches, int32_t n_batches, int32_t iters, float *ms_out)
{
    if (!c || !batches || n_batches <= 0 || iters <= 0) return fail(c, FADEGPU_E_ARG, "fadegpu_replay_batches: bad arguments");
    for (int32_t i = 0; i < n_batches; ++i) {
        fadegpu_batch *b = batches[i];
        if (!b || b->ctx != c) return fail(c, FADEGPU_E_ARG, "fadegpu_replay_batches: bad batch");
        if (b->in_flight) return fail(c, FADEGPU_E_STATE, "fadegpu_replay_batches: batch in flight");
        if (b->plan.empty() && b->n_aln > 0) return fail(c, FADEGPU_E_STATE, "fadegpu_replay_batches: nothing submitted");
    }
    drain_submits(c);
    std::lock_guard<std::mutex> submit_guard(c->submit_mu);
    CU(c, cudaSetDevice(c->device));
    cudaEvent_t e0, e1;
    CU(c, cudaEventCreate(&e0)); CU(c, cudaEventCreate(&e1));
    CU(c, cudaDeviceSynchronize());
    CU(c, cudaEventRecord(e0, c->stream));
    CU(c, cudaStreamWaitEvent(c->stream2, e0, 0));
    for (int32_t it = 0; it < iters; ++it)
        for (int32_t i = 0; i < n_batches; ++i) { int rc = replay_pass(c, batches[i]); if (rc) return rc; }
    for (int32_t i = 0; i < n_batches; ++i) { int rc = replay_join(c, batches[i]); if (rc) return rc; }
    CU(c, cudaEventRecord(e1, c->stream));
    CU(c, cudaEventSynchronize(e1));
    float ms = 0;
    CU(c, cudaEventElapsedTime(&ms, e0, e1));
    cudaEventDestroy(e0); cudaEventDestroy(e1);
    if (ms_out) *ms_out = ms;
    return FADEGPU_OK;
}

int fadegpu_replay_kernels(fadegpu_ctx *c, fadegpu_batch *b, int32_t iters, float *ms_out)
{
    if (!c || !b || b->ctx != c || iters <= 0) return fail(c, FADEGPU_E_ARG, "fadegpu_replay_kernels: bad arguments");
    if (b->in_flight) return fail(c, FADEGPU_E_STATE, "fadegpu_replay_kernels: batch in flight");
    if (b->plan.empty() && b->n_aln > 0) return fail(c, FADEGPU_E_STATE, "fadegpu_replay_kernels: nothing submitted");
    drain_submits(c);
    {
        std::lock_guard<std::mutex> submit_guard(c->submit_mu);
        CU(c, cudaSetDevice(c->device));
        float f = 0, t = 0, g = 0;
        int rc = run_plan(c, b, batch_target(c), &f, &t, &g, nullptr, nullptr);
        if (rc) return rc;
        b->st.fill_ms = f; b->st.trace_ms = t; b->st.generic_ms = g;
    }
    fadegpu_batch *one[1] = { b };
    return fadegpu_replay_batches(c, one, 1, iters, ms_out);
}

static void parallel_copy(char *dst, const char *src, size_t bytes, int nthr)
{
    const int T = (int)std::max<size_t>(1, std::min<size_t>((size_t)std::max(1, nthr), bytes >> 20));
#pragma omp parallel for schedule(static, 1) num_threads(T) if (T > 1)
    for (int t = 0; t < T; ++t) {
        const size_t lo = bytes * (size_t)t / (size_t)T, hi = bytes * (size_t)(t + 1) / (size_t)T;
        memcpy(dst + lo, src + lo, hi - lo);
    }
}

static size_t align16(size_t x) { return (x + 15) & ~(size_t)15; }

static int refuse_in_flight(fadegpu_ctx *c, const char *fn)
{
    std::lock_guard<std::mutex> lk(c->q_mu);
    for (const fadegpu_batch *b : c->batches)
        if (b->in_flight)
            return fail(c, FADEGPU_E_STATE, std::string(fn) + ": a batch of this ctx is in flight (call fadegpu_wait)");
    return 0;
}

struct StagedCall {
    const char *fn, *item;
    int64_t n, qbytes, n_over;
    int32_t max_ops;
    size_t raw;
    size_t o_tbeg, o_tend;
    std::function<void(char *h_stage)> stage;
    std::function<int(fadegpu_batch *b, const char *d_raw, BinArgs &ba, int *launches)> prep;
    std::function<int(fadegpu_batch *b, RefDev *ref, int *launches)> reference;
};

static int align_staged(fadegpu_ctx *c, const StagedCall &sc, fadegpu_pair_result *out, uint32_t *ops_out,
                        fadegpu_stats *stats_out, std::chrono::steady_clock::time_point t_begin)
{
    const int64_t n = sc.n, qbytes = sc.qbytes;
    const int32_t max_ops = sc.max_ops;
    fadegpu_stats st{};
    st.n_reads = n;
    st.n_oversize = sc.n_over;
    if (n == 0) {
        if (stats_out) *stats_out = st;
        return FADEGPU_OK;
    }
    std::lock_guard<std::mutex> submit_guard(c->submit_mu);
    CU(c, cudaSetDevice(c->device));
    fadegpu_ctx::PairBufs &pb = c->pairs;
    if (!pb.b || pb.b->v.max_reads < n || pb.b->v.max_seq_bytes < qbytes + 16) {
        int64_t nr = n, sb = qbytes + 16;
        if (pb.b) {
            nr = std::max(nr, pb.b->v.max_reads); sb = std::max(sb, pb.b->v.max_seq_bytes);
            fadegpu_free_batch(pb.b);
            pb.b = nullptr;
        }
        int rc = fadegpu_alloc_batch(c, nr, sb, &pb.b);
        if (rc) return rc;
    }
    fadegpu_batch *b = pb.b;
    const size_t raw = sc.raw;
    if (pb.stage_bytes < raw) {
        free_host(pb.h_stage);
        pb.stage_bytes = 0;
        CU(c, cudaHostAlloc((void **)&pb.h_stage, raw, cudaHostAllocDefault));
        pb.stage_bytes = raw;
    }
    sc.stage(pb.h_stage);
    {
        int rc = 0;
        auto grow = [&](auto **p, size_t *have, size_t bytes) { if (!rc) rc = ensure_dev(c, (void **)p, have, std::max<size_t>(bytes, 16)); };
        grow(&pb.d_raw, &pb.raw_bytes, raw);
        grow(&pb.d_res, &pb.res_bytes, (size_t)n * sizeof(fadegpu_pair_result));
        if (max_ops > 0) {
            grow(&pb.d_spill, &pb.spill_bytes, (size_t)n * (size_t)max_ops * 4);
            grow(&pb.d_ops, &pb.ops_bytes, (size_t)n * (size_t)max_ops * 4);
        }
        if (rc) return rc;
        if (!pb.d_bad) CU(c, cudaMalloc((void **)&pb.d_bad, sizeof(int32_t)));
    }
    b->n_reads = n;
    b->plan.clear();
    b->dev_binning = true;
    b->ba_valid = false;
    b->n_aln = 0; b->n_items = 0;
    memset(&b->st, 0, sizeof(b->st));
    memset(b->h_stats, 0, 128);
    cudaStream_t s2 = c->stream2;
    CU(c, cudaEventRecord(b->ev[0], s2));
    CU(c, cudaMemcpyAsync(pb.d_raw, pb.h_stage, raw, cudaMemcpyHostToDevice, s2));
    int64_t h2d = (int64_t)raw;
    CU(c, cudaEventRecord(b->ev[4], s2));
    CU(c, cudaMemsetAsync(b->d_hist, 0, (size_t)BIN_KEYS * 4, s2));
    CU(c, cudaMemsetAsync(b->d_cursor, 0, (size_t)BIN_KEYS * 4, s2));
    CU(c, cudaMemsetAsync(b->d_stats, 0, 128, s2));
    CU(c, cudaMemsetAsync(pb.d_bad, 0x7f, sizeof(int32_t), s2));
    BinArgs ba{};
    ba.seq4 = b->d_in_seq4; ba.seq_off = b->d_in_seq_off; ba.l_qseq = b->d_in_lq; ba.tid = b->d_in_tid; ba.pos = b->d_in_pos;
    ba.aligned_len = b->d_in_alen; ba.clip_left = b->d_in_cl; ba.clip_right = b->d_in_cr;
    ba.read = nullptr; ba.seq_cursor = nullptr; ba.src_off = b->d_src_off; ba.gate = nullptr; ba.host_meta = nullptr;
    ba.over_list = b->d_over;
    ba.n = n; ba.seq_total = qbytes; ba.window = 0; ba.min_length = 0; ba.flags = c->p.flags;
    ba.key = b->d_key; ba.tlen = b->d_tlen; ba.start = b->d_start; ba.hist = b->d_hist; ba.stats = b->d_stats;
    ba.keybase = b->d_keybase; ba.cursor = b->d_cursor; ba.aln = b->d_aln; ba.aln_start = b->d_aln_start;
    int n_prep = 0;
    { int rc = sc.prep(b, pb.d_raw, ba, &n_prep); if (rc) return rc; }
    CU(c, launch_bin_classify(ba, c->sm_count, s2));
    CU(c, cudaMemcpyAsync(b->h_hist, b->d_hist, (size_t)BIN_KEYS * 4, cudaMemcpyDeviceToHost, s2));
    CU(c, cudaMemcpyAsync(b->h_stats, b->d_stats, 128, cudaMemcpyDeviceToHost, s2));
    CU(c, cudaMemcpyAsync(b->h_over, pb.d_bad, sizeof(int32_t), cudaMemcpyDeviceToHost, s2));
    CU(c, cudaEventRecord(b->ev_prep, s2));
    CU(c, cudaEventSynchronize(b->ev_prep));
    const int32_t bad = b->h_over[0];
    if (bad >= 0 && bad < n)
        return fail(c, FADEGPU_E_ARG, std::string(sc.fn) + ": the query of " + sc.item + " " + std::to_string(bad) +
                                          " holds a letter outside the BAM nt16 alphabet =ACMGRSVTWYHKDBN");
    if (b->h_stats[6] & 1ull) return fail(c, FADEGPU_E_CUDA, std::string(sc.fn) + ": internal error (query offsets)");
    const int64_t n_aln = (int64_t)b->h_stats[1];
    PlanTarget pt{};
    { int rc = sc.reference(b, &pt.ref, &n_prep); if (rc) return rc; }
    { int rc = plan_from_histogram(c, b, n_aln); if (rc) return rc; }
    if (n_aln > 0) {
        CU(c, cudaMemcpyAsync(b->d_keybase, b->h_keybase, (size_t)BIN_KEYS * 4, cudaMemcpyHostToDevice, s2));
        if (b->n_items > 0)
            CU(c, cudaMemcpyAsync(b->d_items, b->h_items, (size_t)b->n_items * sizeof(WarpItem), cudaMemcpyHostToDevice, s2));
        h2d += (int64_t)BIN_KEYS * 4 + b->n_items * (int64_t)sizeof(WarpItem);
        CU(c, launch_bin_scatter(ba, c->sm_count, s2));
    }
    CU(c, cudaEventRecord(b->ev_ready, s2));
    CU(c, cudaStreamWaitEvent(c->stream, b->ev_ready, 0));
    CU(c, cudaEventRecord(b->ev[1], c->stream));
    pt.tags_only = 0;
    pt.ops_spill = max_ops > 0 ? pb.d_spill : nullptr;
    pt.ops_cap = max_ops;
    int nl = 0;
    { int rc = run_plan(c, b, pt, nullptr, nullptr, nullptr, &nl, b->ev_ready); if (rc) return rc; }
    cudaStream_t s3 = c->stream3;
    { int rc = join_kernels(c, b, s3); if (rc) return rc; }
    CU(c, cudaEventRecord(b->ev[2], s3));
    CU(c, launch_pair_results(n, reinterpret_cast<const int64_t *>(pb.d_raw), reinterpret_cast<const int64_t *>(pb.d_raw + sc.o_tbeg),
                              reinterpret_cast<const int64_t *>(pb.d_raw + sc.o_tend), b->d_aln, b->d_out, (int)n_aln, pb.d_spill,
                              max_ops, reinterpret_cast<PairResult *>(pb.d_res), pb.d_ops, b->d_stats + 7, c->sm_count, s3));
    CU(c, cudaMemcpyAsync(out, pb.d_res, (size_t)n * sizeof(fadegpu_pair_result), cudaMemcpyDeviceToHost, s3));
    if (max_ops > 0)
        CU(c, cudaMemcpyAsync(ops_out, pb.d_ops, (size_t)n * (size_t)max_ops * 4, cudaMemcpyDeviceToHost, s3));
    CU(c, cudaMemcpyAsync(b->h_stats + 7, b->d_stats + 7, 8, cudaMemcpyDeviceToHost, s3));
    CU(c, cudaEventRecord(b->ev[3], s3));
    CU(c, cudaEventSynchronize(b->ev[3]));
    if ((int64_t)b->h_stats[7] != n_aln)
        return fail(c, FADEGPU_E_CUDA, std::string(sc.fn) + ": a kernel did not produce a result record (internal error)");
    st.n_aligned = n_aln;
    st.n_generic = b->st.n_generic;
    st.cells = (int64_t)b->h_stats[0];
    st.h2d_bytes = h2d;
    st.d2h_bytes = n * (int64_t)(sizeof(fadegpu_pair_result) + 4 * (size_t)max_ops) + (int64_t)BIN_KEYS * 4 + 128 + 4 + 8;
    st.kernel_launches = nl + n_prep + 1 + (n_aln > 0 ? 2 : 1);
    st.scratch_bytes = b->st.scratch_bytes;
    float t;
    if (cudaEventElapsedTime(&t, b->ev[1], b->ev[2]) == cudaSuccess) st.kernel_ms = t;
    if (cudaEventElapsedTime(&t, b->ev[0], b->ev[3]) == cudaSuccess) st.total_ms = t;
    st.host_threads = c->host_threads;
    st.host_submit_ms = std::chrono::duration<float, std::milli>(std::chrono::steady_clock::now() - t_begin).count();
    b->st = st;
    if (stats_out) *stats_out = st;
    return FADEGPU_OK;
}

int fadegpu_align_pairs(fadegpu_ctx *c, int64_t n_pairs, const fadegpu_pairs *in, int32_t max_ops,
                        fadegpu_pair_result *out, uint32_t *ops_out, fadegpu_stats *stats_out)
{
    if (!c) return fail(nullptr, FADEGPU_E_ARG, "fadegpu_align_pairs: null ctx");
    if (n_pairs < 0 || n_pairs > ((int64_t)1 << 30) || max_ops < 0)
        return fail(c, FADEGPU_E_ARG, "fadegpu_align_pairs: n_pairs or max_ops out of range");
    if (n_pairs > 0 && (!in || !in->query_off || !in->target_off || !out || (max_ops > 0 && !ops_out)))
        return fail(c, FADEGPU_E_ARG, "fadegpu_align_pairs: null argument");
    { int rc = refuse_in_flight(c, "fadegpu_align_pairs"); if (rc) return rc; }
    const auto t_begin = std::chrono::steady_clock::now();
    const int64_t n = n_pairs;
    int64_t qbytes = 0, tbytes = 0, n_over = 0;
    if (n > 0) {
        const int64_t *qo = in->query_off, *to = in->target_off;
        if (qo[0] < 0 || to[0] < 0) return fail(c, FADEGPU_E_ARG, "fadegpu_align_pairs: negative offset");
        for (int64_t k = 0; k < n; ++k) {
            const int64_t ql = qo[k + 1] - qo[k], tl = to[k + 1] - to[k];
            if (ql < 0 || tl < 0)
                return fail(c, FADEGPU_E_ARG, "fadegpu_align_pairs: offsets decrease at pair " + std::to_string(k));
            if (ql > 0 && tl > 0 && (tl > 0x7fffffff || ql * tl > PAIR_MAX_CELLS)) ++n_over;
        }
        qbytes = qo[n] - qo[0]; tbytes = to[n] - to[0];
        if ((qbytes > 0 && !in->query) || (tbytes > 0 && !in->target))
            return fail(c, FADEGPU_E_ARG, "fadegpu_align_pairs: null sequence array");
    }
    const size_t o_toff = align16((size_t)(n + 1) * 8), o_q = o_toff + align16((size_t)(n + 1) * 8);
    const size_t o_t = o_q + align16((size_t)qbytes);
    const int64_t n_words = n + (tbytes >> 5) + 2;
    const int64_t n_chunks = (n_words + PAIR_CHUNK_WORDS - 1) / PAIR_CHUNK_WORDS;
    fadegpu_ctx::PairBufs &pb = c->pairs;
    PairArgs pa{};
    StagedCall sc;
    sc.fn = "fadegpu_align_pairs"; sc.item = "pair";
    sc.n = n; sc.qbytes = qbytes; sc.n_over = n_over; sc.max_ops = max_ops;
    sc.raw = o_t + align16((size_t)tbytes);
    sc.o_tbeg = o_toff; sc.o_tend = o_toff + 8;
    sc.stage = [&](char *h) {
        int64_t *hq = reinterpret_cast<int64_t *>(h), *ht = reinterpret_cast<int64_t *>(h + o_toff);
        const int64_t q0 = in->query_off[0], t0 = in->target_off[0];
        for (int64_t k = 0; k <= n; ++k) { hq[k] = in->query_off[k] - q0; ht[k] = in->target_off[k] - t0; }
        if (qbytes) parallel_copy(h + o_q, in->query + q0, (size_t)qbytes, c->host_threads);
        if (tbytes) parallel_copy(h + o_t, in->target + t0, (size_t)tbytes, c->host_threads);
    };
    sc.prep = [&](fadegpu_batch *b, const char *d, BinArgs &ba, int *launches) -> int {
        int rc = 0;
        auto grow = [&](auto **p, size_t *have, size_t bytes) { if (!rc) rc = ensure_dev(c, (void **)p, have, std::max<size_t>(bytes, 16)); };
        grow(&pb.d_two, &pb.two_bytes, (size_t)n_words * 8); grow(&pb.d_n, &pb.n_bytes, (size_t)n_words * 4);
        grow(&pb.d_x, &pb.x_bytes, (size_t)n_words * 4); grow(&pb.d_chunk_x, &pb.chunk_bytes, (size_t)n_chunks * 4);
        grow(&pb.d_clen, &pb.clen_bytes, (size_t)n * 8); grow(&pb.d_coff, &pb.coff_bytes, (size_t)n * 8);
        if (rc) return rc;
        pa.n = n;
        pa.qoff = reinterpret_cast<const int64_t *>(d); pa.toff = reinterpret_cast<const int64_t *>(d + o_toff);
        pa.query = d + o_q; pa.target = d + o_t;
        pa.seq_off = b->d_in_seq_off; pa.pos = b->d_in_pos; pa.l_qseq = b->d_in_lq; pa.tid = b->d_in_tid;
        pa.aligned_len = b->d_in_alen; pa.clip_left = b->d_in_cl; pa.clip_right = b->d_in_cr;
        pa.clen = pb.d_clen; pa.coff = pb.d_coff; pa.seq4 = b->d_in_seq4; pa.bad = pb.d_bad;
        pa.two = pb.d_two; pa.nmask = pb.d_n; pa.xmask = pb.d_x; pa.n_words = n_words;
        pa.chunk_x = pb.d_chunk_x; pa.n_x = b->d_stats + 12;
        CU(c, launch_pair_prep(pa, c->sm_count, c->stream2));
        CU(c, launch_pair_pack_targets(pa, c->stream2));
        *launches += 2;
        ba.clen = pb.d_clen; ba.coff = pb.d_coff; ba.n_contigs = (int32_t)n;
        return 0;
    };
    sc.reference = [&](fadegpu_batch *b, RefDev *ref, int *launches) -> int {
        const int64_t n_x = (int64_t)b->h_stats[12];
        int rc = ensure_dev(c, (void **)&pb.d_xpos, &pb.xpos_bytes, std::max<size_t>(16, (size_t)n_x * 8));
        if (!rc) rc = ensure_dev(c, (void **)&pb.d_xchr, &pb.xchr_bytes, std::max<size_t>(16, (size_t)n_x));
        if (rc) return rc;
        pa.xpos = pb.d_xpos; pa.xchr = pb.d_xchr;
        if (n_x > 0) { CU(c, launch_pair_xlist(pa, c->stream2)); ++*launches; }
        ref->planes.two = pb.d_two; ref->planes.nmask = pb.d_n; ref->planes.xmask = pb.d_x;
        ref->xpos = pb.d_xpos; ref->xchr = pb.d_xchr; ref->n_x = n_x;
        return 0;
    };
    return align_staged(c, sc, out, ops_out, stats_out, t_begin);
}

int fadegpu_align_regions(fadegpu_ctx *c, int64_t n_regions, const fadegpu_regions *in, int32_t max_ops,
                          fadegpu_pair_result *out, uint32_t *ops_out, fadegpu_stats *stats_out)
{
    if (!c) return fail(nullptr, FADEGPU_E_ARG, "fadegpu_align_regions: null ctx");
    if (n_regions < 0 || n_regions > ((int64_t)1 << 30) || max_ops < 0)
        return fail(c, FADEGPU_E_ARG, "fadegpu_align_regions: n_regions or max_ops out of range");
    if (n_regions > 0 && (!in || !in->query_off || !in->tid || !in->start || !in->end || !in->strand || !out ||
                          (max_ops > 0 && !ops_out)))
        return fail(c, FADEGPU_E_ARG, "fadegpu_align_regions: null argument");
    { int rc = refuse_in_flight(c, "fadegpu_align_regions"); if (rc) return rc; }
    if (c->n_contigs <= 0) return fail(c, FADEGPU_E_STATE, "fadegpu_align_regions: no reference is loaded");
    const auto t_begin = std::chrono::steady_clock::now();
    const int64_t n = n_regions;
    int64_t qbytes = 0, n_over = 0;
    if (n > 0) {
        const int64_t *qo = in->query_off;
        if (qo[0] < 0) return fail(c, FADEGPU_E_ARG, "fadegpu_align_regions: negative offset");
        for (int64_t k = 0; k < n; ++k) {
            const int64_t ql = qo[k + 1] - qo[k];
            if (ql < 0) return fail(c, FADEGPU_E_ARG, "fadegpu_align_regions: offsets decrease at region " + std::to_string(k));
            const int32_t tid = in->tid[k];
            const int64_t s = in->start[k], e = in->end[k];
            if (tid < 0 || tid >= c->n_contigs || s < 0 || s > e || e > c->clen[(size_t)tid] || in->strand[k] > 1) {
                const std::string at = "fadegpu_align_regions: region " + std::to_string(k) + ": ";
                if (tid < 0 || tid >= c->n_contigs)
                    return fail(c, FADEGPU_E_ARG, at + "tid " + std::to_string(tid) + " is not a contig of the reference");
                if (s < 0 || s > e || e > c->clen[(size_t)tid])
                    return fail(c, FADEGPU_E_ARG, at + "[" + std::to_string(s) + ", " + std::to_string(e) +
                                                      ") is not an interval of contig " + std::to_string(tid) + " (length " +
                                                      std::to_string(c->clen[(size_t)tid]) + ")");
                return fail(c, FADEGPU_E_ARG, at + "strand " + std::to_string(in->strand[k]) + " is neither 0 nor 1");
            }
            const int64_t tl = e - s;
            if (ql > 0 && tl > 0 && (tl > 0x7fffffff || ql * tl > PAIR_MAX_CELLS)) ++n_over;
        }
        qbytes = qo[n] - qo[0];
        if (qbytes > 0 && !in->query) return fail(c, FADEGPU_E_ARG, "fadegpu_align_regions: null sequence array");
    }
    const size_t o_tid = align16((size_t)(n + 1) * 8), o_start = o_tid + align16((size_t)n * 4);
    const size_t o_end = o_start + align16((size_t)n * 8), o_strand = o_end + align16((size_t)n * 8);
    const size_t o_q = o_strand + align16((size_t)n);
    StagedCall sc;
    sc.fn = "fadegpu_align_regions"; sc.item = "region";
    sc.n = n; sc.qbytes = qbytes; sc.n_over = n_over; sc.max_ops = max_ops;
    sc.raw = o_q + align16((size_t)qbytes);
    sc.o_tbeg = o_start; sc.o_tend = o_end;
    sc.stage = [&](char *h) {
        int64_t *hq = reinterpret_cast<int64_t *>(h);
        const int64_t q0 = in->query_off[0];
        for (int64_t k = 0; k <= n; ++k) hq[k] = in->query_off[k] - q0;
        memcpy(h + o_tid, in->tid, (size_t)n * 4);
        memcpy(h + o_start, in->start, (size_t)n * 8);
        memcpy(h + o_end, in->end, (size_t)n * 8);
        memcpy(h + o_strand, in->strand, (size_t)n);
        if (qbytes) parallel_copy(h + o_q, in->query + q0, (size_t)qbytes, c->host_threads);
    };
    sc.prep = [&](fadegpu_batch *b, const char *d, BinArgs &ba, int *launches) -> int {
        RegionArgs ra{};
        ra.n = n;
        ra.query = d + o_q; ra.qoff = reinterpret_cast<const int64_t *>(d);
        ra.rtid = reinterpret_cast<const int32_t *>(d + o_tid);
        ra.start = reinterpret_cast<const int64_t *>(d + o_start); ra.end = reinterpret_cast<const int64_t *>(d + o_end);
        ra.strand = reinterpret_cast<const uint8_t *>(d + o_strand);
        ra.seq_off = b->d_in_seq_off; ra.pos = b->d_in_pos; ra.l_qseq = b->d_in_lq; ra.tid = b->d_in_tid;
        ra.aligned_len = b->d_in_alen; ra.clip_left = b->d_in_cl; ra.clip_right = b->d_in_cr;
        ra.seq4 = b->d_in_seq4; ra.bad = c->pairs.d_bad;
        CU(c, launch_region_prep(ra, c->sm_count, c->stream2));
        *launches += 1;
        ba.clen = c->d_clen; ba.coff = c->d_coff; ba.n_contigs = c->n_contigs;
        return 0;
    };
    sc.reference = [&](fadegpu_batch *, RefDev *ref, int *) -> int { *ref = ref_dev(c); return 0; };
    return align_staged(c, sc, out, ops_out, stats_out, t_begin);
}

int fadegpu_measure_alu_peak(fadegpu_ctx *c, double *ops_per_sec_out, double *sm_clock_mhz_out)
{
    if (!c || !ops_per_sec_out) return fail(c, FADEGPU_E_ARG, "fadegpu_measure_alu_peak: null argument");
    CU(c, cudaSetDevice(c->device));
    cudaDeviceProp prop;
    CU(c, cudaGetDeviceProperties(&prop, c->device));
    const int blocks = prop.multiProcessorCount * 8, threads = 256, iters = 4096;
    cudaEvent_t e0, e1;
    CU(c, cudaEventCreate(&e0)); CU(c, cudaEventCreate(&e1));
    double best = 0;
    for (int rep = 0; rep < 5; ++rep) {
        CU(c, cudaEventRecord(e0, c->stream));
        CU(c, launch_alu_peak(c->d_alu, iters, blocks, threads, c->stream));
        CU(c, cudaEventRecord(e1, c->stream));
        CU(c, cudaEventSynchronize(e1));
        float ms = 0;
        CU(c, cudaEventElapsedTime(&ms, e0, e1));
        const double ops = (double)blocks * threads * (double)iters * 64.0;
        if (rep > 0 && ms > 0) best = std::max(best, ops / (ms * 1e-3));
    }
    cudaEventDestroy(e0); cudaEventDestroy(e1);
    *ops_per_sec_out = best;
    if (sm_clock_mhz_out) {
        int khz = 0;
        cudaDeviceGetAttribute(&khz, cudaDevAttrClockRate, c->device);
        *sm_clock_mhz_out = khz / 1000.0;
    }
    return FADEGPU_OK;
}

}
```

fade_b200/csrc/kernels.cu:

```cuda
#include "kernels.cuh"
#include <algorithm>
#include <cstdio>
#include <cstdlib>

namespace fade {

namespace {

constexpr unsigned FULL = 0xffffffffu;

#define FADE_SMALL_KERNEL __launch_bounds__(128, 16)


__device__ __forceinline__ uint32_t stage_targets(const KernelArgs &a, const AlnDesc &da, const AlnDesc &db, int g,
                                                  int step0, int nsteps, uint16_t *tw)
{
    const int TW = nsteps + FG + 1;
    uint32_t w = 0;
    for (int idx = g; idx < TW; idx += FG) {
        const int j = step0 + idx - FG;
        int ca = C_TPAD, cb = C_TPAD;
        if (j >= 0 && j < da.tlen) ca = ref_code(a.ref.planes, da.gstart + j);
        if (j >= 0 && j < db.tlen) cb = ref_code(a.ref.planes, db.gstart + j);
        w |= (ca == C_WILD ? 1u : 0u) | (cb == C_WILD ? 2u : 0u);
        tw[idx] = (uint16_t)t_sel(ca, cb);
    }
    return w;
}

template <int R, int STEP>
__device__ __forceinline__ void stage_pair(const KernelArgs &a, const AlnDesc &da, const AlnDesc &db,
                                           int g, int nblk, uint16_t *tw, uint32_t (&qs)[query_words<R, STEP>()],
                                           uint8_t *qc, uint32_t &wild)
{
    uint32_t w = stage_targets(a, da, db, g, 0, FBLK * min(nblk, FILL_CHUNK_BLOCKS), tw);
    const uint8_t *sa = a.seq + da.seq_off, *sb = a.seq + db.seq_off;
#pragma unroll
    for (int r = 0; r < R; ++r) {
        const int i = g * R + r;
        int ca = C_QPAD, cb = C_QPAD;
        if (i < da.qlen) ca = rc_query_code(sa, da.qlen, i);
        if (i < db.qlen) cb = rc_query_code(sb, db.qlen, i);
        w |= (ca == C_WILD ? 1u : 0u) | (cb == C_WILD ? 2u : 0u);
        set_query<STEP>(qs, r, ca, cb);
        if (qc) qc[i] = (uint8_t)(ca | (cb << 4));
    }
    wild = w;
}

__device__ __forceinline__ AlnDesc load_desc(const KernelArgs &a, int idx)
{
    AlnDesc d;
    if (idx < a.n_aln) d = a.aln[idx];
    else { d.gstart = 0; d.seq_off = 0; d.tlen = 0; d.qlen = 0; d.clip_left = d.clip_right = 0; d.read = -1; d.pad = 0; }
    return d;
}

template <int R, int STEP>
__global__ void __launch_bounds__(FILL_THREADS, (R <= 19 ? 5 : 1)) sw_fill_kernel(const KernelArgs a)
{
    extern __shared__ __align__(16) unsigned char smem_raw[];
    const int lane = threadIdx.x & 31, wib = threadIdx.x >> 5;
    const int g = lane & (FG - 1), q = lane >> 3;
    const int w = blockIdx.x * (FILL_THREADS / 32) + wib;
    if (w >= a.n_items) return;
    const WarpItem item = a.items[w];
    const int ia = item.first + 2 * q, ib = ia + 1;
    const AlnDesc da = load_desc(a, ia), db = load_desc(a, ib);
    uint16_t *tw = reinterpret_cast<uint16_t *>(smem_raw) + (size_t)(wib * 4 + q) * a.tw_stride;
    const int nblk = item.nblk;
    const SwConsts k = a.k;

    uint32_t H[R], E[R], qs[query_words<R, STEP>()];
    uint32_t wild;
    stage_pair<R, STEP>(a, da, db, g, nblk, tw, qs, nullptr, wild);
#pragma unroll
    for (int r = 0; r < R; ++r) { H[r] = 0u; E[r] = k.neg_o; }
    uint32_t hu_prev = 0u, fout = k.neg_o, M = 0u, Mprev = 0u;
    int blk_lo = 0, blk_hi = 0;
    __syncwarp();

    constexpr int CW = ck_words<R>();
    uint32_t *ckw = a.ck + item.ck_off + lane;
    const uint16_t *twp = tw + (FG - g);
    const int nsteps = item.nsteps;
    for (int c = 0; c < nblk; ++c) {
        if (c > 0 && (c % FILL_CHUNK_BLOCKS) == 0) {
            __syncwarp();
            wild |= stage_targets(a, da, db, g, c * FBLK, FBLK * min(nblk - c, FILL_CHUNK_BLOCKS), tw);
            twp = tw + (FG - g) - c * FBLK;
            __syncwarp();
        }
        const int ulim = min(FBLK, nsteps - c * FBLK);
#pragma unroll 2
        for (int u = 0; u < ulim; ++u) {
            const int t = c * FBLK + u;
            uint32_t hu = __shfl_up_sync(FULL, H[R - 1], 1, FG);
            uint32_t fin = __shfl_up_sync(FULL, fout, 1, FG);
            if (g == 0) { hu = 0u; fin = k.neg_o; }
            const uint32_t ts = twp[t];
            score_step<R, STEP>(H, E, qs, M, ts, hu_prev, fin, fout, k);
            hu_prev = hu;
        }
        if (c + 1 < nblk) {
            uint32_t *p = ckw + (size_t)c * CW * 32;
#pragma unroll
            for (int r = 0; r < R; ++r) { p[r * 32] = H[r]; p[(R + r) * 32] = E[r]; }
            p[(2 * R) * 32] = hu_prev;
            p[(2 * R + 1) * 32] = fout;
        }
        if (M != Mprev) {
            if ((M ^ Mprev) & 0xffffu) blk_lo = c;
            if ((M ^ Mprev) >> 16) blk_hi = c;
            Mprev = M;
        }
    }
    a.fillres[(size_t)w * 32 + lane] = make_uint2(M, (uint32_t)blk_lo | ((uint32_t)blk_hi << 16));
    if ((wild & 1u) && ia < a.n_aln) a.aln_flags[ia] = 1u;
    if ((wild & 2u) && ib < a.n_aln) a.aln_flags[ib] = 1u;
}

__device__ __forceinline__ unsigned long long pack_req(int aln, int blk, uint32_t scanmask)
{
    return (unsigned long long)(uint32_t)aln | ((unsigned long long)(uint32_t)(blk & 0xffff) << 32) |
           ((unsigned long long)(scanmask & 0xffu) << 48);
}

struct GlobalAcc {
    const uint8_t *seq;
    int qlen;
    RefPlanes planes;
    int64_t gstart;
    __device__ __forceinline__ int qcode(int i) const { return rc_query_code(seq, qlen, i); }
    __device__ __forceinline__ int tcode(int j) const { return ref_code(planes, gstart + j); }
};

template <int R>
__global__ void FADE_SMALL_KERNEL trace_init_kernel(const KernelArgs a)
{
    for (int aln = blockIdx.x * blockDim.x + threadIdx.x; aln < a.n_aln; aln += gridDim.x * blockDim.x) {
        a.out[aln].read = -1;
        a.out[aln].flags = 0x80000000u;
        if (a.aln_flags[aln] & 1u) continue;
        const AlnDesc d = a.aln[aln];
        LaneCtl &c = a.state[aln];
        const int w = aln >> 3, q = (aln & 7) >> 1, half = aln & 1;
        const uint2 *fr = a.fillres + (size_t)w * 32 + q * FG;
        for (int g = 0; g < FG; ++g) {
            const uint2 v = fr[g];
            c.best[g] = half ? lane_hi(v.x) : lane_lo(v.x);
            c.blk[g] = half ? (int)(v.y >> 16) : (int)(v.y & 0xffffu);
        }
        ctl_init(c, d.qlen, d.tlen);
        if (c.phase != 2 && a.tags_only && !score_may_accept(c.S, d.clip_left, d.clip_right, a.min_length)) {
            AlnOut o;
            o.score = c.S; o.end_query = o.end_ref = o.beg_query = o.beg_ref = 0; o.n_ops = 0;
            o.flags = R_ALIGNED | R_SCORE_ONLY; o.read = d.read;
            for (int k = 0; k < OPS_CAP; ++k) o.ops[k] = 0;
            a.out[aln] = o;
        } else if (c.phase == 2) {
            AlnOut o;
            finalize_result(c, o, d.read, d.clip_left, d.clip_right, a.min_length);
            a.out[aln] = o;
        } else {
            const unsigned slot = atomicAdd(&a.qcount[0], 1u);
            a.queue[0][slot] = pack_req(aln, c.next_blk, ctl_scanmask(c));
        }
    }
}

template <int R, int MODE, int STEP = 0>
__device__ __forceinline__ void replay_round(const KernelArgs &a, int round, unsigned warp0, unsigned nwarps,
                                             uint16_t (*tws_all)[40])
{
    constexpr bool TAGGED = MODE == 0;
    constexpr bool SCAN_ONLY = MODE == 2;
    constexpr int RW = trace_words<R>();
    constexpr int CW = ck_words<R>();
    constexpr int MUL = TAGGED ? 16 : 1;
    const int lane = threadIdx.x & 31, wib = threadIdx.x >> 5;
    const int g = lane & (FG - 1), q = lane >> 3;
    const int rin = round & 1;
    const unsigned cnt = a.qcount[rin];
    const unsigned long long *queue = a.queue[rin];
    const unsigned npairs = (cnt + 1u) >> 1;
    const unsigned nquads = (npairs + 3u) >> 2;
    const SwConsts k = a.k;
    const uint32_t e_init = TAGGED ? k.neg_o16 : k.neg_o;
    uint16_t *tws = tws_all[wib * 4 + q];
    for (unsigned quad = warp0; quad < nquads; quad += nwarps) {
        const unsigned pair = quad * 4u + (unsigned)q;
        int aln[2], blk[2], half[2], S[2];
        uint32_t smask[2];
        AlnDesc d[2];
        const uint32_t *ckp[2];
#pragma unroll
        for (int L = 0; L < 2; ++L) {
            const unsigned ri = pair * 2u + (unsigned)L;
            if (ri < cnt) {
                const unsigned long long rq = queue[ri];
                aln[L] = (int)(uint32_t)(rq & 0xffffffffu);
                blk[L] = (int)((rq >> 32) & 0xffffu);
                smask[L] = (uint32_t)((rq >> 48) & 0xffu);
                d[L] = a.aln[aln[L]];
                const WarpItem it = a.items[aln[L] >> 3];
                ckp[L] = a.ck + it.ck_off + (((aln[L] & 7) >> 1) * FG + g);
                half[L] = aln[L] & 1;
                S[L] = a.state[aln[L]].S * MUL;
            } else {
                aln[L] = -1; blk[L] = 0; smask[L] = 0; half[L] = 0; S[L] = -1; ckp[L] = a.ck;
                d[L].gstart = 0; d[L].seq_off = 0; d[L].tlen = 0; d[L].qlen = 0;
            }
        }
        uint32_t H[R], E[R], qs[query_words<R, STEP>()], hu_prev, fout;
        {
            const uint32_t *p0 = ckp[0] + (size_t)(blk[0] > 0 ? blk[0] - 1 : 0) * CW * 32;
            const uint32_t *p1 = ckp[1] + (size_t)(blk[1] > 0 ? blk[1] - 1 : 0) * CW * 32;
            const bool z0 = blk[0] == 0, z1 = blk[1] == 0;
            const int sh0 = half[0] * 16, sh1 = half[1] * 16;
            auto mix = [&](uint32_t w0, uint32_t w1) {
                const uint32_t w = ((w0 >> sh0) & 0xffffu) | ((w1 >> sh1) << 16);
                return TAGGED ? to_tagged(w) : w;
            };
#pragma unroll
            for (int r = 0; r < R; ++r) {
                H[r] = mix(z0 ? 0u : p0[r * 32], z1 ? 0u : p1[r * 32]);
                E[r] = mix(z0 ? k.neg_o : p0[(R + r) * 32], z1 ? k.neg_o : p1[(R + r) * 32]);
            }
            hu_prev = mix(z0 ? 0u : p0[(2 * R) * 32], z1 ? 0u : p1[(2 * R) * 32]);
            fout = mix(z0 ? k.neg_o : p0[(2 * R + 1) * 32], z1 ? k.neg_o : p1[(2 * R + 1) * 32]);
        }
        {
            const uint8_t *s0 = a.seq + d[0].seq_off, *s1 = a.seq + d[1].seq_off;
#pragma unroll
            for (int r = 0; r < R; ++r) {
                const int i = g * R + r;
                const int ca = i < d[0].qlen ? rc_query_code(s0, d[0].qlen, i) : C_QPAD;
                const int cb = i < d[1].qlen ? rc_query_code(s1, d[1].qlen, i) : C_QPAD;
                set_query<STEP>(qs, r, ca, cb);
            }
            __syncwarp();
            for (int x = g; x < FBLK + FG - 1; x += FG) {
                const int j0 = blk[0] * FBLK - (FG - 1) + x, j1 = blk[1] * FBLK - (FG - 1) + x;
                const int ca = (j0 >= 0 && j0 < d[0].tlen) ? ref_code(a.ref.planes, d[0].gstart + j0) : C_TPAD;
                const int cb = (j1 >= 0 && j1 < d[1].tlen) ? ref_code(a.ref.planes, d[1].gstart + j1) : C_TPAD;
                tws[x] = (uint16_t)t_sel(ca, cb);
            }
            __syncwarp();
        }
        uint32_t *tile = a.tiles + (size_t)pair * tile_words<R>();
        const bool store = aln[0] >= 0;
        bool need0 = (smask[0] >> g) & 1u, need1 = (smask[1] >> g) & 1u;
        const uint16_t *twp = tws + (FG - 1 - g);
        for (int u = 0; u < FBLK; ++u) {
            uint32_t hu = __shfl_up_sync(FULL, H[R - 1], 1, FG);
            uint32_t fin = __shfl_up_sync(FULL, fout, 1, FG);
            if (g == 0) { hu = 0u; fin = e_init; }
            const uint32_t ts = twp[u];
            uint32_t cmax = 0u;
            if constexpr (SCAN_ONLY) {
                score_step<R, STEP>(H, E, qs, cmax, ts, hu_prev, fin, fout, k);
            } else {
                uint32_t trw[RW];
                if (TAGGED) trace_step_tagged<R>(H, E, qs, ts, hu_prev, fin, fout, k, trw, cmax);
                else trace_step_plain<R>(H, E, qs, ts, hu_prev, fin, fout, k, trw, cmax);
                if (store) {
#pragma unroll
                    for (int w = 0; w < RW; ++w) tile[tile_index<R>(u, g, w)] = trw[w];
                }
            }
            hu_prev = hu;
            if (need0 && lane_lo(cmax) == S[0]) {
                need0 = false;
                int fr = 0;
#pragma unroll
                for (int r = R - 1; r >= 0; --r) if (lane_lo(H[r]) == S[0]) fr = r;
                a.state[aln[0]].fj[g] = blk[0] * FBLK + u - g;
                a.state[aln[0]].fr[g] = fr;
            }
            if (need1 && lane_hi(cmax) == S[1]) {
                need1 = false;
                int fr = 0;
#pragma unroll
                for (int r = R - 1; r >= 0; --r) if (lane_hi(H[r]) == S[1]) fr = r;
                a.state[aln[1]].fj[g] = blk[1] * FBLK + u - g;
                a.state[aln[1]].fr[g] = fr;
            }
            if (SCAN_ONLY && !__any_sync(FULL, need0 || need1)) break;
        }
    }
}

template <int R, int MODE, int STEP = 0>
__global__ void __launch_bounds__(128) trace_replay_kernel(const KernelArgs a)
{
    __shared__ uint16_t tws_all[16][40];
    if (blockIdx.x == 0 && threadIdx.x == 0) a.qcount[(a.round & 1) ^ 1] = 0u;
    replay_round<R, MODE, STEP>(a, a.round, blockIdx.x * (blockDim.x >> 5) + (threadIdx.x >> 5),
                                gridDim.x * (blockDim.x >> 5), tws_all);
}

struct AdvanceSmem {
    LaneCtl ctl;
    AlnOut out;
};
static_assert(sizeof(LaneCtl) % 4 == 0 && sizeof(AlnOut) % 4 == 0, "word-copyable");

template <int R, bool SPILL>
__device__ __forceinline__ void advance_round(const KernelArgs &a, int round, unsigned warp0, unsigned nwarps,
                                              AdvanceSmem *smem_all)
{
    constexpr int RW = trace_words<R>();
    constexpr int CTLW = (int)(sizeof(LaneCtl) / 4), OUTW = (int)(sizeof(AlnOut) / 4);
    AdvanceSmem &sm = smem_all[threadIdx.x >> 5];
    const int rin = round & 1;
    const unsigned cnt = a.qcount[rin];
    const unsigned long long *queue = a.queue[rin];
    const int l = threadIdx.x & 31;
    const SwConsts &k = a.k;
    const bool tile_valid = !(round == 0 && k.shortcut);
    for (unsigned idx = warp0; idx < cnt; idx += nwarps) {
        const int aln = (int)(uint32_t)(queue[idx] & 0xffffffffu);
        const AlnDesc d = a.aln[aln];
        LaneCtl &c = sm.ctl;
        {
            const uint32_t *src = reinterpret_cast<const uint32_t *>(&a.state[aln]);
            uint32_t *dst = reinterpret_cast<uint32_t *>(&c);
            for (int w = l; w < CTLW; w += 32) dst[w] = src[w];
        }
        __syncwarp();
        const uint32_t *tile = a.tiles + (size_t)(idx >> 1) * tile_words<R>();
        const int sh = 16 * (int)(idx & 1u);
        GlobalAcc acc;
        acc.seq = a.seq + d.seq_off; acc.qlen = d.qlen; acc.planes = a.ref.planes; acc.gstart = d.gstart;
        int go = 1;
        if (l == 0) {
            c.cur_blk = c.next_blk;
            if (c.phase == 0 && !ctl_select_end<R>(c)) go = 0;
        }
        go = __shfl_sync(FULL, go, 0);
        __syncwarp();
        bool done = false;
        int need = -1;
        if (go) {
            int i = 0, j = 0, mode = 0, hval = 0, gval = 0, nrev = 0, cur_blk_ = 0;
            uint32_t cur = 0;
            if (l == 0) {
                i = c.i; j = c.j; mode = c.mode; hval = c.hval; gval = c.gval; nrev = c.nrev; cur = c.cur;
                cur_blk_ = c.cur_blk;
            }
            i = __shfl_sync(FULL, i, 0); j = __shfl_sync(FULL, j, 0); mode = __shfl_sync(FULL, mode, 0);
            hval = __shfl_sync(FULL, hval, 0); gval = __shfl_sync(FULL, gval, 0); nrev = __shfl_sync(FULL, nrev, 0);
            cur = __shfl_sync(FULL, cur, 0);
            const int cur_blk = __shfl_sync(FULL, cur_blk_, 0);
            auto push_n = [&](uint32_t op, int n) {
                if (cur != 0 && (cur & 0xf) == op) { cur += 16u * (uint32_t)n; return; }
                if (cur != 0) {
                    if (l == 0) {
                        c.ring[nrev % OPS_CAP] = cur;
                        if (SPILL && a.ops_spill) a.ops_spill[(size_t)aln * a.ops_cap + nrev % a.ops_cap] = cur;
                    }
                    ++nrev;
                }
                cur = ((uint32_t)n << 4) | op;
            };
            int forced = 0;
            for (;;) {
                if (i < 0 || j < 0) { done = true; break; }
                if (mode == 0 && hval <= 0) { done = true; break; }
                if (mode == 0) {
                    const int ii = i - l, jj = j - l;
                    const bool valid = ii >= 0 && jj >= 0;
                    const int g = valid ? ii / R : 0, r = valid ? ii - g * R : 0;
                    const int t = jj + g;
                    const bool inblk = valid && tile_valid && (t / FBLK) == cur_blk;
                    uint32_t nib = 0;
                    int sc = 0;
                    bool eq = false;
                    if (valid && (inblk || forced > 0)) {
                        eq = acc.qcode(ii) == acc.tcode(jj);
                        sc = eq ? k.match : k.mismatch;
                    }
                    if (inblk && forced == 0)
                        nib = (tile[tile_index<R>(t % FBLK, g, r >> 2)] >> (sh + 4 * (r & 3))) & 0xfu;
                    const bool diag = forced > 0 ? (valid && l < forced) : (inblk && (nib >> 2) == 2u);
                    if (!diag) sc = 0;
                    int pre = sc;
#pragma unroll
                    for (int o = 1; o < 32; o <<= 1) {
                        const int v = __shfl_up_sync(FULL, pre, o);
                        if (l >= o) pre += v;
                    }
                    const int hv = hval - (pre - sc);
                    const bool ok = diag && hv > 0;
                    const unsigned bad = __ballot_sync(FULL, !ok);
                    const int L = bad ? __ffs(bad) - 1 : 32;
                    if (L > 0) {
                        const unsigned lim = L == 32 ? 0xffffffffu : ((1u << L) - 1u);
                        const unsigned eqm = __ballot_sync(FULL, eq) & lim;
                        int kx = 0;
                        while (kx < L) {
                            const unsigned bit = (eqm >> kx) & 1u;
                            const unsigned diff = ((bit ? ~eqm : eqm) & lim) >> kx;
                            int run = diff ? __ffs(diff) - 1 : L - kx;
                            push_n(bit ? OP_EQ : OP_X, run);
                            kx += run;
                        }
                        const int hlast = __shfl_sync(FULL, hv - sc, L - 1);
                        hval = hlast;
                        i -= L; j -= L;
                        if (forced > 0) forced -= L;
                        continue;
                    }
                    if (!__shfl_sync(FULL, (int)inblk, 0)) {
                        bool proven = false;
                        int steps = 0;
                        if (k.shortcut) {
                            int rem = hval, pi = i, pj = j;
                            for (;;) {
                                const int qi = pi - l, qj = pj - l;
                                const bool v2 = qi >= 0 && qj >= 0;
                                int s2 = 0;
                                if (v2) s2 = acc.qcode(qi) == acc.tcode(qj) ? k.match : k.mismatch;
                                int p2 = s2;
#pragma unroll
                                for (int o = 1; o < 32; o <<= 1) {
                                    const int v = __shfl_up_sync(FULL, p2, o);
                                    if (l >= o) p2 += v;
                                }
                                const int rl = rem - p2;
                                const unsigned hit = __ballot_sync(FULL, v2 && rl <= 0);
                                const unsigned inv = __ballot_sync(FULL, !v2);
                                const int fh = hit ? __ffs(hit) - 1 : 32, fi = inv ? __ffs(inv) - 1 : 32;
                                if (fh < fi) {
                                    proven = __shfl_sync(FULL, rl, fh) == 0;
                                    steps += fh + 1;
                                    break;
                                }
                                if (fi < 32) break;
                                rem = __shfl_sync(FULL, rl, 31);
                                steps += 32; pi -= 32; pj -= 32;
                            }
                        }
                        if (proven) { forced = steps; continue; }
                        const int g0 = i / R;
                        need = (j + g0) / FBLK;
                        break;
                    }
                    const uint32_t n0 = __shfl_sync(FULL, nib, 0);
                    if ((n0 >> 2) == 1u) { push_n(OP_I, 1); --i; mode = 1; gval = hval; }
                    else { push_n(OP_D, 1); --j; mode = 2; gval = hval; }
                } else {
                    const int g = i / R, r = i - g * R;
                    const int t = j + g;
                    if (t / FBLK != cur_blk || !tile_valid) { need = t / FBLK; break; }
                    const uint32_t nib = (tile[tile_index<R>(t % FBLK, g, r >> 2)] >> (sh + 4 * (r & 3))) & 0xfu;
                    if (mode == 1) {
                        if (!(nib & 2u)) { hval = gval + k.open; mode = 0; }
                        else { push_n(OP_I, 1); --i; gval += k.extend; }
                    } else {
                        if (!(nib & 1u)) { hval = gval + k.open; mode = 0; }
                        else { push_n(OP_D, 1); --j; gval += k.extend; }
                    }
                }
            }
            if (done && cur != 0) {
                if (l == 0) {
                    c.ring[nrev % OPS_CAP] = cur;
                    if (SPILL && a.ops_spill) a.ops_spill[(size_t)aln * a.ops_cap + nrev % a.ops_cap] = cur;
                }
                ++nrev; cur = 0;
            }
            if (l == 0) {
                c.i = i; c.j = j; c.mode = mode; c.hval = hval; c.gval = gval; c.cur = cur; c.nrev = nrev;
                if (done) { c.phase = 2; c.next_blk = -1; } else c.next_blk = need;
            }
        }
        __syncwarp();
        const bool fin = c.phase == 2;
        if (l == 0) {
            if (fin) finalize_result(c, sm.out, d.read, d.clip_left, d.clip_right, a.min_length);
            else if (round + 1 < a.max_rounds) {
                const unsigned slot = atomicAdd(&a.qcount[rin ^ 1], 1u);
                a.queue[rin ^ 1][slot] = pack_req(aln, c.next_blk, ctl_scanmask(c));
            }
        }
        __syncwarp();
        if (fin) {
            const uint32_t *src = reinterpret_cast<const uint32_t *>(&sm.out);
            uint32_t *dst = reinterpret_cast<uint32_t *>(&a.out[aln]);
            for (int w = l; w < OUTW; w += 32) dst[w] = src[w];
        } else {
            const uint32_t *src = reinterpret_cast<const uint32_t *>(&c);
            uint32_t *dst = reinterpret_cast<uint32_t *>(&a.state[aln]);
            for (int w = l; w < CTLW; w += 32) dst[w] = src[w];
        }
        __syncwarp();
    }
}

template <int R, bool SPILL>
__global__ void FADE_SMALL_KERNEL trace_advance_kernel(const KernelArgs a)
{
    __shared__ AdvanceSmem adv[4];
    advance_round<R, SPILL>(a, a.round, blockIdx.x * (blockDim.x >> 5) + (threadIdx.x >> 5), gridDim.x * (blockDim.x >> 5), adv);
}

template <int R, bool TAGGED>
__global__ void __launch_bounds__(128) trace_tail_kernel(const KernelArgs a)
{
    __shared__ uint16_t tws_all[16][40];
    __shared__ AdvanceSmem adv[4];
    for (int r = a.round; r < a.max_rounds; ++r) {
        if (a.qcount[r & 1] == 0u) break;
        __syncthreads();
        if (threadIdx.x == 0) a.qcount[(r & 1) ^ 1] = 0u;
        __syncthreads();
        replay_round<R, TAGGED ? 0 : 1>(a, r, threadIdx.x >> 5, blockDim.x >> 5, tws_all);
        __threadfence_block();
        __syncthreads();
        advance_round<R, true>(a, r, threadIdx.x >> 5, blockDim.x >> 5, adv);
        __threadfence_block();
        __syncthreads();
    }
}

__device__ __forceinline__ int map_char(int c)
{
    switch (c) {
    case 'A': return 0;
    case 'C': return 1;
    case 'T': return 2;
    case 'G': return 3;
    case 'N': return 4;
    default: return 5;
    }
}

__device__ int ref_char(const RefDev &rf, int64_t p)
{
    const int c = ref_code(rf.planes, p);
    if (c < 4) return "ACTG"[c];
    if (c == C_N) return 'N';
    int64_t lo = 0, hi = rf.n_x - 1;
    while (lo <= hi) {
        const int64_t mid = (lo + hi) >> 1;
        const int64_t v = rf.xpos[mid];
        if (v == p) return rf.xchr[mid];
        if (v < p) lo = mid + 1; else hi = mid - 1;
    }
    return '?';
}

__global__ void __launch_bounds__(128) sw_generic_kernel(const GenericArgs a)
{
    const int slot = blockIdx.x * blockDim.x + threadIdx.x;
    if (slot >= a.n_slots) return;
    uint8_t *sc = a.scratch + (size_t)slot * a.slot_bytes;
    int32_t *Hc = reinterpret_cast<int32_t *>(sc);
    int32_t *Ec = Hc + a.qmax;
    uint8_t *qch = reinterpret_cast<uint8_t *>(Ec + a.qmax);
    uint8_t *trc = qch + ((a.qmax + 15) & ~15);
    const int o = a.open, e = a.extend;
    const char nt16[] = "=ACMGRSVTWYHKDBN";
    const uint8_t comp16[16] = { 0, 8, 4, 12, 2, 10, 6, 14, 1, 9, 5, 13, 3, 11, 7, 15 };
    unsigned idx = 0, idx_end = 0;
    for (;;) {
        if (idx >= idx_end) {
            idx = atomicAdd(a.cursor, (unsigned)a.chunk);
            if (idx >= (unsigned)a.n_aln) break;
            idx_end = min(idx + (unsigned)a.chunk, (unsigned)a.n_aln);
        }
        const unsigned cur_idx = idx++;
        if (a.aln_flags && !(a.aln_flags[cur_idx] & 1u)) continue;
        const AlnDesc d = a.aln[cur_idx];
        const int qlen = d.qlen, tlen = d.tlen;
        AlnOut out;
        out.read = d.read;
        for (int kk = 0; kk < OPS_CAP; ++kk) out.ops[kk] = 0;
        if (qlen <= 0 || tlen <= 0 || qlen > a.qmax || tlen > a.tmax) {
            out.score = out.end_query = out.end_ref = out.beg_query = out.beg_ref = out.n_ops = 0;
            out.flags = R_ALIGNED | R_GENERIC;
            a.out[cur_idx] = out;
            continue;
        }
        const uint8_t *s4 = a.seq + d.seq_off;
        for (int i = 0; i < qlen; ++i) {
            qch[i] = (uint8_t)nt16[comp16[nt16_at(s4, qlen - 1 - i)]];
            Hc[i] = 0;
            Ec[i] = -(1 << 28);
        }
        int best = 0, bi = 0, bj = 0;
        for (int j = 0; j < tlen; ++j) {
            const int tch = ref_char(a.ref, d.gstart + j);
            const int tcd = map_char(tch);
            int hdiag = 0, hup = 0, f = -(1 << 28);
            for (int i = 0; i < qlen; ++i) {
                const int hleft = Hc[i];
                const int e_opn = hleft - o, e_ext = Ec[i] - e;
                int tb = 0, ev, fv;
                if (e_opn > e_ext) { ev = e_opn; tb |= T_EOPEN; } else ev = e_ext;
                const int f_opn = hup - o, f_ext = f - e;
                if (f_opn > f_ext) { fv = f_opn; tb |= T_FOPEN; } else fv = f_ext;
                const int qcd = map_char(qch[i]);
                const int s = (qcd == 5 || tcd == 5) ? 0 : (qcd == tcd ? a.match : a.mismatch);
                int hd = hdiag + s;
                if (hd < 0) hd = 0;
                int h = hd;
                if (ev > h) h = ev;
                if (fv > h) h = fv;
                if (h == hd) tb |= (h == 0) ? T_ZERO : T_DIAG;
                else tb |= (h == fv) ? T_F : T_E;
                trc[(size_t)i * tlen + j] = (uint8_t)tb;
                hdiag = hleft; hup = h; f = fv;
                Ec[i] = ev; Hc[i] = h;
                if (h > best) { best = h; bi = i; bj = j; }
            }
        }
        out.score = best;
        if (best > 0 && a.tags_only && !score_may_accept(best, d.clip_left, d.clip_right, a.min_length)) {
            out.end_query = out.end_ref = out.beg_query = out.beg_ref = out.n_ops = 0;
            out.flags = R_ALIGNED | R_GENERIC | R_SCORE_ONLY;
            a.out[cur_idx] = out;
            continue;
        }
        if (best <= 0) {
            out.end_query = out.end_ref = out.beg_query = out.beg_ref = out.n_ops = 0;
            out.flags = R_ALIGNED | R_GENERIC;
            a.out[cur_idx] = out;
            continue;
        }
        uint32_t ring[OPS_CAP];
        int nrev = 0;
        uint32_t cur = 0;
        int i = bi, j = bj, state = 0;
        while (i >= 0 && j >= 0) {
            const int tb = trc[(size_t)i * tlen + j];
            uint32_t op;
            if (state == 0) {
                const int src = tb & 3;
                if (src == T_ZERO) break;
                if (src == T_DIAG) {
                    op = (qch[i] == (uint8_t)ref_char(a.ref, d.gstart + j)) ? OP_EQ : OP_X;
                    --i; --j;
                } else if (src == T_F) { state = 1; continue; }
                else { state = 2; continue; }
            } else if (state == 1) {
                op = OP_I; --i;
                if (tb & T_FOPEN) state = 0;
            } else {
                op = OP_D; --j;
                if (tb & T_EOPEN) state = 0;
            }
            if (cur != 0 && (cur & 0xf) == op) cur += 16;
            else {
                if (cur != 0) {
                    ring[nrev % OPS_CAP] = cur;
                    if (a.ops_spill) a.ops_spill[(size_t)cur_idx * a.ops_cap + nrev % a.ops_cap] = cur;
                    ++nrev;
                }
                cur = (1u << 4) | op;
            }
        }
        if (cur != 0) {
            ring[nrev % OPS_CAP] = cur;
            if (a.ops_spill) a.ops_spill[(size_t)cur_idx * a.ops_cap + nrev % a.ops_cap] = cur;
            ++nrev;
        }
        out.end_query = bi; out.end_ref = bj; out.beg_query = i + 1; out.beg_ref = j + 1;
        const int lead = i + 1, trail = qlen - 1 - bi;
        const int n = (lead > 0) + nrev + (trail > 0);
        out.n_ops = n;
        int wq = 0;
        if (lead > 0) out.ops[wq++] = ((uint32_t)lead << 4) | OP_S;
        for (int kk = nrev - 1; kk >= 0 && wq < OPS_CAP; --kk) {
            if (nrev - kk > OPS_CAP) break;
            out.ops[wq++] = ring[kk % OPS_CAP];
        }
        if (trail > 0 && wq < OPS_CAP && wq == n - 1) out.ops[wq++] = ((uint32_t)trail << 4) | OP_S;
        uint32_t flags = R_ALIGNED | R_GENERIC;
        if (n > OPS_CAP) flags |= R_OPS_TRUNC;
        const uint32_t first_op = lead > 0 ? (uint32_t)OP_S : (ring[(nrev - 1) % OPS_CAP] & 0xf);
        const uint32_t last_op = trail > 0 ? (uint32_t)OP_S : (ring[0] & 0xf);
        if (accept_side(true, best, n, first_op, last_op, lead, trail, d.clip_left, a.min_length)) flags |= R_ART_LEFT;
        if (accept_side(false, best, n, first_op, last_op, lead, trail, d.clip_right, a.min_length)) flags |= R_ART_RIGHT;
        out.flags = flags;
        a.out[cur_idx] = out;
    }
}

__global__ void FADE_SMALL_KERNEL bin_classify_kernel(const BinArgs a)
{
    const uint32_t floor_u = (uint32_t)a.min_length;
    unsigned long long cells = 0, bad = 0;
    int qmax = 0, tmax = 0, qmax_g = 0, tmax_g = 0, cnt = 0, fetched = 0;
    for (int64_t r = (int64_t)blockIdx.x * blockDim.x + threadIdx.x; r < a.n; r += (int64_t)gridDim.x * blockDim.x) {
        int key = -1;
        uint32_t cl, cr;
        bool need;
        if (a.gate) {
            const uint32_t g = a.gate[r];
            need = floor_u < 255u ? g > floor_u : g == 255u;
            cl = cr = 0;
            if (need) {
                const uint4 m0 = a.host_meta[2 * r], m1 = a.host_meta[2 * r + 1];
                ++fetched;
                a.pos[r] = (int64_t)(((unsigned long long)m0.y << 32) | m0.x);
                a.seq_off[r] = (int64_t)m0.z;
                a.l_qseq[r] = (int32_t)m0.w;
                a.tid[r] = (int32_t)m1.x;
                a.aligned_len[r] = (int32_t)m1.y;
                a.clip_left[r] = (int32_t)(cl = m1.z);
                a.clip_right[r] = (int32_t)(cr = m1.w);
                need = (cl != 0 && !(cl <= floor_u)) || (cr != 0 && !(cr <= floor_u));
            } else {
                a.clip_left[r] = 0; a.clip_right[r] = 0;
            }
        } else {
            cl = (uint32_t)a.clip_left[r]; cr = (uint32_t)a.clip_right[r];
            need = (cl != 0 && !(cl <= floor_u)) || (cr != 0 && !(cr <= floor_u));
        }
        if (need) {
            const int tid = a.tid[r], ql = a.l_qseq[r];
            if (tid >= 0 && tid < a.n_contigs && ql > 0) {
                const int64_t so = a.seq_off[r];
                if (so < 0 || so + (ql + 1) / 2 > a.seq_total) bad |= 1ull;
                else {
                    int64_t start = a.pos[r] - a.window;
                    if (start < 0) start = 0;
                    int64_t end = a.pos[r] + (int64_t)a.aligned_len[r] + a.window;
                    if (end > a.clen[tid]) end = a.clen[tid];
                    if (end > start) {
                        if (end - start > 0x7fffffff || (end - start) * (int64_t)ql > ((int64_t)1 << 31)) {
                            const unsigned long long slot = atomicAdd(&a.stats[11], 1ull);
                            if (slot < (unsigned long long)OVER_CAP) a.over_list[slot] = a.read ? a.read[r] : (int32_t)r;
                        } else {
                            const int tl = (int)(end - start);
                            const int rk = bin_rank(ql, tl, (a.flags & 1u) != 0);
                            key = bin_key(rk, tl);
                            a.tlen[r] = tl;
                            a.start[r] = start;
                            atomicAdd(&a.hist[key], 1);
                            cells += (unsigned long long)ql * (unsigned long long)tl;
                            ++cnt;
                            qmax = max(qmax, ql); tmax = max(tmax, tl);
                            if (rk == N_ROW_CLASSES) { qmax_g = max(qmax_g, ql); tmax_g = max(tmax_g, tl); }
                        }
                    }
                }
            }
        }
        a.key[r] = key;
    }
#pragma unroll
    for (int o = 16; o > 0; o >>= 1) {
        cells += __shfl_xor_sync(FULL, cells, o);
        bad |= __shfl_xor_sync(FULL, bad, o);
        cnt += __shfl_xor_sync(FULL, cnt, o);
        fetched += __shfl_xor_sync(FULL, fetched, o);
        qmax = max(qmax, __shfl_xor_sync(FULL, qmax, o)); tmax = max(tmax, __shfl_xor_sync(FULL, tmax, o));
        qmax_g = max(qmax_g, __shfl_xor_sync(FULL, qmax_g, o)); tmax_g = max(tmax_g, __shfl_xor_sync(FULL, tmax_g, o));
    }
    if ((threadIdx.x & 31) == 0) {
        if (cells) atomicAdd(&a.stats[0], cells);
        if (cnt) atomicAdd(&a.stats[1], (unsigned long long)cnt);
        if (qmax) atomicMax(&a.stats[2], (unsigned long long)qmax);
        if (tmax) atomicMax(&a.stats[3], (unsigned long long)tmax);
        if (qmax_g) atomicMax(&a.stats[4], (unsigned long long)qmax_g);
        if (tmax_g) atomicMax(&a.stats[5], (unsigned long long)tmax_g);
        if (bad) atomicOr(&a.stats[6], bad);
        if (fetched) atomicAdd(&a.stats[10], (unsigned long long)fetched);
    }
}

__global__ void FADE_SMALL_KERNEL bin_scatter_kernel(const BinArgs a)
{
    for (int64_t r = (int64_t)blockIdx.x * blockDim.x + threadIdx.x; r < a.n; r += (int64_t)gridDim.x * blockDim.x) {
        const int key = a.key[r];
        if (key < 0) continue;
        const int slot = a.keybase[key] + atomicAdd(&a.cursor[key], 1);
        AlnDesc d;
        d.gstart = a.coff[a.tid[r]] + a.start[r];
        d.seq_off = a.seq_off[r];
        if (a.seq_cursor) {
            const int64_t so = d.seq_off;
            const int ph = (int)(so & 15);
            const unsigned long long bytes = (unsigned long long)((ph + (a.l_qseq[r] + 1) / 2 + 15) & ~15);
            d.seq_off = (int64_t)atomicAdd(a.seq_cursor, bytes) + ph;
            a.src_off[slot] = so;
        }
        d.tlen = a.tlen[r];
        d.qlen = a.l_qseq[r];
        d.clip_left = (uint32_t)a.clip_left[r];
        d.clip_right = (uint32_t)a.clip_right[r];
        d.read = a.read ? a.read[r] : (int32_t)r;
        d.pad = 0;
        a.aln[slot] = d;
        a.aln_start[slot] = a.start[r];
    }
}

__global__ void FADE_SMALL_KERNEL seq_pull_kernel(const uint8_t *__restrict__ host_seq4, const AlnDesc *__restrict__ aln,
                                                       const int64_t *__restrict__ src_off, int n_aln, uint8_t *__restrict__ dst)
{
    const int lane = threadIdx.x & 7;
    for (int k = (blockIdx.x * blockDim.x + threadIdx.x) >> 3; k < n_aln; k += (gridDim.x * blockDim.x) >> 3) {
        const int64_t so = src_off[k];
        const int ph = (int)(so & 15);
        const int chunks = (ph + (aln[k].qlen + 1) / 2 + 15) >> 4;
        const uint4 *s = reinterpret_cast<const uint4 *>(host_seq4 + (so - ph));
        uint4 *d = reinterpret_cast<uint4 *>(dst + (aln[k].seq_off - ph));
        for (int i = lane; i < chunks; i += 8) d[i] = s[i];
    }
}

__global__ void FADE_SMALL_KERNEL result_index_kernel(const AlnOut *out, int n_aln, int64_t n_reads, uint8_t *flags, int32_t *ridx,
                                                      unsigned long long *n_ok)
{
    int ok = 0;
    for (int k = blockIdx.x * blockDim.x + threadIdx.x; k < n_aln; k += gridDim.x * blockDim.x) {
        const int r = out[k].read;
        const uint32_t f = out[k].flags;
        if (r >= 0 && (int64_t)r < n_reads && (f & 1u) && !(f & 0x80000000u)) { flags[r] = (uint8_t)(f & 0xffu); ridx[r] = k; ++ok; }
    }
    ok = __reduce_add_sync(FULL, ok);
    if ((threadIdx.x & 31) == 0 && ok) atomicAdd(n_ok, (unsigned long long)ok);
}

__device__ __forceinline__ int nt16_of_ascii(int ch)
{
    if (ch >= 'a' && ch <= 'z') ch -= 32;
    switch (ch) {
    case '=': return 0; case 'A': return 1; case 'C': return 2; case 'M': return 3;
    case 'G': return 4; case 'R': return 5; case 'S': return 6; case 'V': return 7;
    case 'T': return 8; case 'W': return 9; case 'Y': return 10; case 'H': return 11;
    case 'K': return 12; case 'D': return 13; case 'B': return 14; case 'N': return 15;
    default: return 16;
    }
}

__device__ __forceinline__ bool pack_query_nt16(const char *q, int64_t qlen, bool rc, uint8_t *dst, int l)
{
    const uint8_t comp16[16] = { 0, 8, 4, 12, 2, 10, 6, 14, 1, 9, 5, 13, 3, 11, 7, 15 };
    bool bad = false;
    for (int64_t b = l; b < (qlen + 1) / 2; b += 32) {
        uint32_t byte = 0;
        for (int h = 0; h < 2; ++h) {
            const int64_t i = 2 * b + h;
            if (i >= qlen) break;
            const int c = nt16_of_ascii((unsigned char)q[rc ? qlen - 1 - i : i]);
            bad |= c > 15;
            byte |= (uint32_t)(rc ? comp16[c & 15] : c & 15) << (h ? 0 : 4);
        }
        dst[b] = (uint8_t)byte;
    }
    return bad;
}

__global__ void FADE_SMALL_KERNEL pair_prep_kernel(const PairArgs a)
{
    const int l = threadIdx.x & 31;
    const int64_t nwarps = ((int64_t)gridDim.x * blockDim.x) >> 5;
    for (int64_t k = ((int64_t)blockIdx.x * blockDim.x + threadIdx.x) >> 5; k < a.n; k += nwarps) {
        const int64_t q0 = a.qoff[k], qlen = a.qoff[k + 1] - q0;
        const int64_t t0 = a.toff[k], tlen = a.toff[k + 1] - t0;
        const bool over = tlen > 0x7fffffff || qlen * tlen > PAIR_MAX_CELLS;
        if (l == 0) {
            a.seq_off[k] = q0;
            a.pos[k] = 0;
            a.l_qseq[k] = (int32_t)qlen;
            a.tid[k] = (int32_t)k;
            a.aligned_len[k] = over ? 0 : (int32_t)tlen;
            a.clip_left[k] = over ? 0 : (int32_t)qlen;
            a.clip_right[k] = 0;
            a.clen[k] = tlen;
            a.coff[k] = 32 * (k + (t0 >> 5));
        }
        const bool bad = pack_query_nt16(a.query + q0, qlen, true, a.seq4 + q0, l);
        if (__any_sync(0xffffffffu, bad) && l == 0) atomicMin(a.bad, (int32_t)k);
    }
}

__global__ void FADE_SMALL_KERNEL region_prep_kernel(const RegionArgs a)
{
    const int l = threadIdx.x & 31;
    const int64_t nwarps = ((int64_t)gridDim.x * blockDim.x) >> 5;
    for (int64_t k = ((int64_t)blockIdx.x * blockDim.x + threadIdx.x) >> 5; k < a.n; k += nwarps) {
        const int64_t q0 = a.qoff[k], qlen = a.qoff[k + 1] - q0;
        const int64_t tlen = a.end[k] - a.start[k];
        const bool over = tlen > 0x7fffffff || qlen * tlen > PAIR_MAX_CELLS;
        if (l == 0) {
            a.seq_off[k] = q0;
            a.pos[k] = a.start[k];
            a.l_qseq[k] = (int32_t)qlen;
            a.tid[k] = a.rtid[k];
            a.aligned_len[k] = over ? 0 : (int32_t)tlen;
            a.clip_left[k] = over ? 0 : (int32_t)qlen;
            a.clip_right[k] = 0;
        }
        const bool bad = pack_query_nt16(a.query + q0, qlen, a.strand[k] == 0, a.seq4 + q0, l);
        if (__any_sync(0xffffffffu, bad) && l == 0) atomicMin(a.bad, (int32_t)k);
    }
}

__device__ __forceinline__ int64_t pair_of_base(const PairArgs &a, int64_t p)
{
    int64_t lo = 0, hi = a.n - 1;
    while (lo < hi) {
        const int64_t mid = (lo + hi + 1) >> 1;
        if (a.coff[mid] <= p) lo = mid; else hi = mid - 1;
    }
    return lo;
}

constexpr int PAIR_WORDS_PER_THREAD = PAIR_CHUNK_WORDS / 256;
__global__ void __launch_bounds__(256) pair_pack_targets_kernel(const PairArgs a)
{
    __shared__ int warp_x[8];
    int nx = 0;
    for (int u = 0; u < PAIR_WORDS_PER_THREAD; ++u) {
        const int64_t w = (int64_t)blockIdx.x * PAIR_CHUNK_WORDS + threadIdx.x * PAIR_WORDS_PER_THREAD + u;
        if (w >= a.n_words) break;
        uint32_t a0 = 0, a1 = 0, nm = 0, xm = 0;
        if (a.n > 0) {
            const int64_t p0 = 32 * w, k = pair_of_base(a, p0);
            const int64_t local = p0 - a.coff[k], tlen = a.clen[k];
            if (local >= 0 && local < tlen) {
                const char *t = a.target + a.toff[k] + local;
                const int lim = (int)min((int64_t)32, tlen - local);
                for (int b = 0; b < lim; ++b) {
                    int ch = (unsigned char)t[b];
                    if (ch >= 'a' && ch <= 'z') ch -= 32;
                    const uint32_t code = ch == 'A' ? 0u : ch == 'C' ? 1u : ch == 'T' ? 2u : ch == 'G' ? 3u : 0u;
                    if (b < 16) a0 |= code << (2 * b); else a1 |= code << (2 * (b - 16));
                    if (ch == 'N') nm |= 1u << b;
                    else if (ch != 'A' && ch != 'C' && ch != 'G' && ch != 'T') xm |= 1u << b;
                }
            }
        }
        a.two[2 * w] = a0; a.two[2 * w + 1] = a1; a.nmask[w] = nm; a.xmask[w] = xm;
        nx += __popc(xm);
    }
    nx = __reduce_add_sync(FULL, nx);
    if ((threadIdx.x & 31) == 0) warp_x[threadIdx.x >> 5] = nx;
    __syncthreads();
    if (threadIdx.x == 0) {
        int t = 0;
        for (int i = 0; i < 8; ++i) t += warp_x[i];
        a.chunk_x[blockIdx.x] = (uint32_t)t;
        if (t) atomicAdd(a.n_x, (unsigned long long)t);
    }
}

__device__ __forceinline__ uint32_t block_exclusive_256(uint32_t v, uint32_t *total)
{
    __shared__ uint32_t warp_sum[8];
    const int l = threadIdx.x & 31, wi = threadIdx.x >> 5;
    uint32_t inc = v;
#pragma unroll
    for (int o = 1; o < 32; o <<= 1) {
        const uint32_t y = __shfl_up_sync(FULL, inc, o);
        if (l >= o) inc += y;
    }
    if (l == 31) warp_sum[wi] = inc;
    __syncthreads();
    uint32_t before = 0, all = 0;
    for (int i = 0; i < 8; ++i) { if (i < wi) before += warp_sum[i]; all += warp_sum[i]; }
    __syncthreads();
    *total = all;
    return before + inc - v;
}

__global__ void __launch_bounds__(256) pair_xlist_kernel(const PairArgs a)
{
    __shared__ uint32_t chunk_base;
    if (a.chunk_x[blockIdx.x] == 0) return;
    if (threadIdx.x == 0) chunk_base = 0;
    __syncthreads();
    {
        uint32_t part = 0;
        for (int64_t c = threadIdx.x; c < blockIdx.x; c += blockDim.x) part += a.chunk_x[c];
        part = __reduce_add_sync(FULL, part);
        if ((threadIdx.x & 31) == 0 && part) atomicAdd(&chunk_base, part);
    }
    __syncthreads();
    const int64_t w0 = (int64_t)blockIdx.x * PAIR_CHUNK_WORDS + threadIdx.x * PAIR_WORDS_PER_THREAD;
    uint32_t xm[PAIR_WORDS_PER_THREAD], cnt = 0;
    for (int u = 0; u < PAIR_WORDS_PER_THREAD; ++u) {
        xm[u] = w0 + u < a.n_words ? a.xmask[w0 + u] : 0u;
        cnt += __popc(xm[u]);
    }
    uint32_t total;
    int64_t slot = (int64_t)chunk_base + block_exclusive_256(cnt, &total);
    for (int u = 0; u < PAIR_WORDS_PER_THREAD; ++u) {
        if (!xm[u]) continue;
        const int64_t p0 = 32 * (w0 + u), k = pair_of_base(a, p0);
        const char *t = a.target + a.toff[k] + (p0 - a.coff[k]);
        for (uint32_t m = xm[u]; m; m &= m - 1) {
            const int b = __ffs(m) - 1;
            int ch = (unsigned char)t[b];
            if (ch >= 'a' && ch <= 'z') ch -= 32;
            a.xpos[slot] = p0 + b;
            a.xchr[slot] = (uint8_t)ch;
            ++slot;
        }
    }
}

__global__ void FADE_SMALL_KERNEL pair_results_init_kernel(int64_t n, const int64_t *qoff, const int64_t *t_beg,
                                                           const int64_t *t_end, PairResult *res)
{
    for (int64_t k = (int64_t)blockIdx.x * blockDim.x + threadIdx.x; k < n; k += (int64_t)gridDim.x * blockDim.x) {
        const int64_t qlen = qoff[k + 1] - qoff[k], tlen = t_end[k] - t_beg[k];
        PairResult r;
        r.score = r.end_query = r.end_ref = r.beg_query = r.beg_ref = r.n_ops = 0;
        r.reserved = 0;
        r.flags = (qlen > 0 && tlen > 0 && (tlen > 0x7fffffff || qlen * tlen > PAIR_MAX_CELLS)) ? PAIR_R_OVERSIZE : 0u;
        res[k] = r;
    }
}

__global__ void FADE_SMALL_KERNEL pair_results_kernel(const AlnDesc *aln, const AlnOut *out, int n_aln, int64_t n,
                                                      const uint32_t *spill, int max_ops, PairResult *res, uint32_t *ops,
                                                      unsigned long long *n_ok)
{
    int ok = 0;
    for (int idx = blockIdx.x * blockDim.x + threadIdx.x; idx < n_aln; idx += gridDim.x * blockDim.x) {
        const AlnOut o = out[idx];
        const int64_t k = o.read;
        if (k < 0 || k >= n || !(o.flags & R_ALIGNED) || (o.flags & 0x80000000u)) continue;
        ++ok;
        PairResult r;
        r.score = o.score; r.end_query = o.end_query; r.end_ref = o.end_ref; r.beg_query = o.beg_query; r.beg_ref = o.beg_ref;
        r.n_ops = o.n_ops;
        r.flags = (o.flags & (R_ALIGNED | R_GENERIC)) | (o.n_ops > max_ops ? R_OPS_TRUNC : 0u);
        r.reserved = 0;
        res[k] = r;
        if (max_ops > 0) {
            uint32_t *dst = ops + (size_t)k * max_ops;
            if (o.n_ops == 0) {
                for (int w = 0; w < max_ops; ++w) dst[w] = 0;
            } else {
                const int lead = o.beg_query, trail = aln[idx].qlen - 1 - o.end_query;
                const int nrev = o.n_ops - (lead > 0) - (trail > 0);
                forward_ops(spill + (size_t)idx * max_ops, max_ops, nrev, lead, trail, dst);
            }
        }
    }
    ok = __reduce_add_sync(FULL, ok);
    if ((threadIdx.x & 31) == 0 && ok) atomicAdd(n_ok, (unsigned long long)ok);
}

__global__ void __launch_bounds__(256) alu_peak_kernel(uint32_t *out, int iters)
{
    uint32_t x0 = threadIdx.x, x1 = x0 + 1, x2 = x0 + 2, x3 = x0 + 3, x4 = x0 + 4, x5 = x0 + 5, x6 = x0 + 6, x7 = x0 + 7;
    const uint32_t c = 0x00010003u + blockIdx.x, d = 0xfffefffdu;
    for (int i = 0; i < iters; ++i) {
#pragma unroll
        for (int u = 0; u < 8; ++u) {
            x0 = __viaddmax_s16x2(x0, c, d); x1 = __viaddmax_s16x2(x1, c, d);
            x2 = __viaddmax_s16x2(x2, c, d); x3 = __viaddmax_s16x2(x3, c, d);
            x4 = __viaddmax_s16x2(x4, c, d); x5 = __viaddmax_s16x2(x5, c, d);
            x6 = __viaddmax_s16x2(x6, c, d); x7 = __viaddmax_s16x2(x7, c, d);
        }
    }
    const uint32_t r = x0 ^ x1 ^ x2 ^ x3 ^ x4 ^ x5 ^ x6 ^ x7;
    if (r == 0x12345678u) out[0] = r;
}

}

int tw_stride_for(int nblk_max) { return (FBLK * std::min(nblk_max, FILL_CHUNK_BLOCKS) + FG + 1 + 7) & ~7; }

size_t fill_smem_bytes(int tw_stride) { return (size_t)(FILL_THREADS / FG) * tw_stride * 2; }

template <int R, int STEP>
static cudaError_t launch_fill_tf(const KernelArgs &a, cudaStream_t s)
{
    const size_t smem = fill_smem_bytes(a.tw_stride);
    cudaError_t e = cudaFuncSetAttribute(sw_fill_kernel<R, STEP>, cudaFuncAttributeMaxDynamicSharedMemorySize, (int)smem);
    if (e != cudaSuccess) return e;
    const int wpb = FILL_THREADS / 32;
    const int grid = (a.n_items + wpb - 1) / wpb;
    sw_fill_kernel<R, STEP><<<grid, FILL_THREADS, smem, s>>>(a);
    return cudaGetLastError();
}

template <int R>
static cudaError_t launch_fill_t(const KernelArgs &a, cudaStream_t s)
{
    switch (score_step_for(a.k)) {
    case 2: return launch_fill_tf<R, 2>(a, s);
    case 1: return launch_fill_tf<R, 1>(a, s);
    default: return launch_fill_tf<R, 0>(a, s);
    }
}

template <int R, bool TAGGED>
static cudaError_t launch_trace_tt(KernelArgs a, cudaStream_t s, int sm_count, int *launches)
{
    const int n = a.n_aln;
    int grid = std::min((n + 127) / 128, sm_count * 8);
    trace_init_kernel<R><<<grid, 128, 0, s>>>(a);
    int nl = 1;
    constexpr int FULL_ROUNDS = 10;
    const int quads = (n + 7) / 8;
    int r = 0;
    for (; r < a.max_rounds && r < FULL_ROUNDS; ++r) {
        a.round = r;
        const int g1 = std::min((quads + 3) / 4, r < 3 ? sm_count * 4 : sm_count);
        const int g2 = std::min((n + 3) / 4, r < 3 ? sm_count * 16 : sm_count * 2);
        if (getenv("FADEGPU_DEBUG_ROUNDS")) {
            unsigned int qc[2] = { 0, 0 };
            cudaStreamSynchronize(s);
            cudaMemcpy(qc, a.qcount, sizeof(qc), cudaMemcpyDeviceToHost);
            fprintf(stderr, "[fadegpu] round %d: %u requests (n_aln %d)\n", r, qc[r & 1], n);
        }
        if (r == 0 && a.k.shortcut) {
            const int step = score_step_for(a.k);
            if (step == 2) trace_replay_kernel<R, 2, 2><<<std::max(g1, 1), 128, 0, s>>>(a);
            else if (step == 1) trace_replay_kernel<R, 2, 1><<<std::max(g1, 1), 128, 0, s>>>(a);
            else trace_replay_kernel<R, 2, 0><<<std::max(g1, 1), 128, 0, s>>>(a);
        }
        else trace_replay_kernel<R, TAGGED ? 0 : 1><<<std::max(g1, 1), 128, 0, s>>>(a);
        if (a.ops_spill) trace_advance_kernel<R, true><<<std::max(g2, 1), 128, 0, s>>>(a);
        else trace_advance_kernel<R, false><<<std::max(g2, 1), 128, 0, s>>>(a);
        nl += 2;
    }
    if (r < a.max_rounds) {
        a.round = r;
        trace_tail_kernel<R, TAGGED><<<1, 128, 0, s>>>(a);
        nl += 1;
    }
    if (launches) *launches += nl;
    return cudaGetLastError();
}

template <int R>
static cudaError_t launch_trace_t(const KernelArgs &a, cudaStream_t s, int sm_count, int *launches)
{
    return a.k.tagged_ok ? launch_trace_tt<R, true>(a, s, sm_count, launches)
                         : launch_trace_tt<R, false>(a, s, sm_count, launches);
}

cudaError_t launch_fill(int R, const KernelArgs &a, cudaStream_t s)
{
    if (a.n_items <= 0) return cudaSuccess;
    switch (R) {
    case 13: return launch_fill_t<13>(a, s);
    case 19: return launch_fill_t<19>(a, s);
    case 25: return launch_fill_t<25>(a, s);
    case 32: return launch_fill_t<32>(a, s);
    case 38: return launch_fill_t<38>(a, s);
    default: return cudaErrorInvalidValue;
    }
}

cudaError_t launch_trace(int R, const KernelArgs &a, cudaStream_t s, int sm_count, int *launches)
{
    if (a.n_items <= 0) return cudaSuccess;
    switch (R) {
    case 13: return launch_trace_t<13>(a, s, sm_count, launches);
    case 19: return launch_trace_t<19>(a, s, sm_count, launches);
    case 25: return launch_trace_t<25>(a, s, sm_count, launches);
    case 32: return launch_trace_t<32>(a, s, sm_count, launches);
    case 38: return launch_trace_t<38>(a, s, sm_count, launches);
    default: return cudaErrorInvalidValue;
    }
}

size_t trace_tile_bytes(int R)
{
    switch (R) {
    case 13: return (size_t)tile_words<13>() * 4;
    case 19: return (size_t)tile_words<19>() * 4;
    case 25: return (size_t)tile_words<25>() * 4;
    case 32: return (size_t)tile_words<32>() * 4;
    default: return (size_t)tile_words<38>() * 4;
    }
}

cudaError_t launch_bin_classify(const BinArgs &a, int sm_count, cudaStream_t s)
{
    if (a.n <= 0) return cudaSuccess;
    const int grid = (int)std::min<int64_t>((a.n + 127) / 128, (int64_t)sm_count * 16);
    bin_classify_kernel<<<grid, 128, 0, s>>>(a);
    return cudaGetLastError();
}

cudaError_t launch_bin_scatter(const BinArgs &a, int sm_count, cudaStream_t s)
{
    if (a.n <= 0) return cudaSuccess;
    const int grid = (int)std::min<int64_t>((a.n + 127) / 128, (int64_t)sm_count * 16);
    bin_scatter_kernel<<<grid, 128, 0, s>>>(a);
    return cudaGetLastError();
}

cudaError_t launch_seq_pull(const uint8_t *host_seq4, const AlnDesc *aln, const int64_t *src_off, int n_aln, uint8_t *dst, int sm_count,
                            cudaStream_t s)
{
    if (n_aln <= 0) return cudaSuccess;
    const int grid = std::min((n_aln * 8 + 127) / 128, sm_count * 16);
    seq_pull_kernel<<<grid, 128, 0, s>>>(host_seq4, aln, src_off, n_aln, dst);
    return cudaGetLastError();
}

cudaError_t launch_result_index(const AlnOut *out, int n_aln, int64_t n_reads, uint8_t *flags, int32_t *ridx, unsigned long long *n_ok,
                                int sm_count, cudaStream_t s)
{
    if (n_aln <= 0) return cudaSuccess;
    result_index_kernel<<<std::min((n_aln + 127) / 128, sm_count * 16), 128, 0, s>>>(out, n_aln, n_reads, flags, ridx, n_ok);
    return cudaGetLastError();
}

cudaError_t launch_generic(const GenericArgs &a, int n_slots, cudaStream_t s)
{
    if (a.n_aln <= 0 || n_slots <= 0) return cudaSuccess;
    const int threads = 128;
    const int grid = (n_slots + threads - 1) / threads;
    if (a.n_slots != n_slots || a.chunk <= 0) return cudaErrorInvalidValue;
    sw_generic_kernel<<<grid, threads, 0, s>>>(a);
    return cudaGetLastError();
}

cudaError_t launch_pair_prep(const PairArgs &a, int sm_count, cudaStream_t s)
{
    if (a.n <= 0) return cudaSuccess;
    const int grid = (int)std::min<int64_t>((a.n * 32 + 127) / 128, (int64_t)sm_count * 16);
    pair_prep_kernel<<<grid, 128, 0, s>>>(a);
    return cudaGetLastError();
}

cudaError_t launch_pair_pack_targets(const PairArgs &a, cudaStream_t s)
{
    if (a.n_words <= 0) return cudaSuccess;
    pair_pack_targets_kernel<<<(unsigned)((a.n_words + PAIR_CHUNK_WORDS - 1) / PAIR_CHUNK_WORDS), 256, 0, s>>>(a);
    return cudaGetLastError();
}

cudaError_t launch_pair_xlist(const PairArgs &a, cudaStream_t s)
{
    if (a.n_words <= 0) return cudaSuccess;
    pair_xlist_kernel<<<(unsigned)((a.n_words + PAIR_CHUNK_WORDS - 1) / PAIR_CHUNK_WORDS), 256, 0, s>>>(a);
    return cudaGetLastError();
}

cudaError_t launch_region_prep(const RegionArgs &a, int sm_count, cudaStream_t s)
{
    if (a.n <= 0) return cudaSuccess;
    const int grid = (int)std::min<int64_t>((a.n * 32 + 127) / 128, (int64_t)sm_count * 16);
    region_prep_kernel<<<grid, 128, 0, s>>>(a);
    return cudaGetLastError();
}

cudaError_t launch_pair_results(int64_t n, const int64_t *qoff, const int64_t *t_beg, const int64_t *t_end,
                                const AlnDesc *aln, const AlnOut *out, int n_aln, const uint32_t *spill, int max_ops,
                                PairResult *res, uint32_t *ops, unsigned long long *n_ok, int sm_count, cudaStream_t s)
{
    if (n <= 0) return cudaSuccess;
    pair_results_init_kernel<<<(int)std::min<int64_t>((n + 127) / 128, (int64_t)sm_count * 16), 128, 0, s>>>(n, qoff, t_beg,
                                                                                                             t_end, res);
    if (n_aln > 0)
        pair_results_kernel<<<std::min((n_aln + 127) / 128, sm_count * 16), 128, 0, s>>>(aln, out, n_aln, n, spill, max_ops,
                                                                                       res, ops, n_ok);
    return cudaGetLastError();
}

cudaError_t launch_alu_peak(uint32_t *out, int iters, int blocks, int threads, cudaStream_t s)
{
    alu_peak_kernel<<<blocks, threads, 0, s>>>(out, iters);
    return cudaGetLastError();
}

}
```

fade_b200/csrc/kernels.cuh:

```cuda
#pragma once
#include <cuda_runtime.h>
#include <stdint.h>
#include "sw_core.cuh"

namespace fade {

struct AlnDesc {
    int64_t gstart;
    int64_t seq_off;
    int32_t tlen;
    int32_t qlen;
    uint32_t clip_left, clip_right;
    int32_t read;
    int32_t pad;
};

struct WarpItem {
    int64_t ck_off;
    int32_t first;
    int16_t nblk;
    int16_t pad;
    int32_t nsteps;
};

struct RefDev {
    RefPlanes planes;
    const int64_t *xpos;
    const uint8_t *xchr;
    int64_t n_x;
};

struct KernelArgs {
    const AlnDesc *aln;
    int32_t n_aln;
    const WarpItem *items;
    int32_t n_items;
    const uint8_t *seq;
    RefDev ref;
    uint32_t *ck;
    uint2 *fillres;
    uint32_t *aln_flags;
    AlnOut *out;
    SwConsts k;
    int32_t min_length;
    int32_t tw_stride;
    LaneCtl *state;
    unsigned long long *queue[2];
    unsigned int *qcount;
    uint32_t *tiles;
    int32_t round, max_rounds;
    int32_t tags_only;
    uint32_t *ops_spill;
    int32_t ops_cap;
};

struct GenericArgs {
    const AlnDesc *aln;
    int32_t n_aln;
    const uint32_t *aln_flags;
    const uint8_t *seq;
    RefDev ref;
    AlnOut *out;
    unsigned int *cursor;
    uint8_t *scratch;
    int64_t slot_bytes;
    int32_t qmax, tmax;
    int32_t n_slots;
    int32_t chunk;
    int32_t open, extend, match, mismatch, min_length;
    int32_t tags_only;
    uint32_t *ops_spill;
    int32_t ops_cap;
};

struct BinArgs {
    const uint8_t *seq4;
    int64_t *seq_off;
    int32_t *l_qseq, *tid;
    int64_t *pos;
    int32_t *aligned_len, *clip_left, *clip_right;
    const int32_t *read;
    int64_t n, seq_total;
    const int64_t *clen, *coff;
    int32_t n_contigs, window, min_length;
    uint32_t flags;
    int32_t *key;
    int32_t *tlen;
    int64_t *start;
    int32_t *hist;
    unsigned long long *stats;
    const int32_t *keybase;
    int32_t *cursor;
    AlnDesc *aln;
    int64_t *aln_start;
    int32_t *over_list;
    const uint8_t *gate;
    const uint4 *host_meta;
    unsigned long long *seq_cursor;
    int64_t *src_off;
};

struct PairArgs {
    int64_t n;
    const char *query, *target;
    const int64_t *qoff, *toff;
    int64_t *seq_off, *pos;
    int32_t *l_qseq, *tid, *aligned_len, *clip_left, *clip_right;
    int64_t *clen, *coff;
    uint8_t *seq4;
    int32_t *bad;
    uint32_t *two, *nmask, *xmask;
    int64_t n_words;
    uint32_t *chunk_x;
    unsigned long long *n_x;
    int64_t *xpos;
    uint8_t *xchr;
};
constexpr int PAIR_CHUNK_WORDS = 1024;
constexpr int64_t PAIR_MAX_CELLS = (int64_t)1 << 31;
constexpr uint32_t PAIR_R_OVERSIZE = 32u;
cudaError_t launch_pair_prep(const PairArgs &a, int sm_count, cudaStream_t s);
cudaError_t launch_pair_pack_targets(const PairArgs &a, cudaStream_t s);
cudaError_t launch_pair_xlist(const PairArgs &a, cudaStream_t s);
struct RegionArgs {
    int64_t n;
    const char *query;
    const int64_t *qoff;
    const int32_t *rtid;
    const int64_t *start, *end;
    const uint8_t *strand;
    int64_t *seq_off, *pos;
    int32_t *l_qseq, *tid, *aligned_len, *clip_left, *clip_right;
    uint8_t *seq4;
    int32_t *bad;
};
cudaError_t launch_region_prep(const RegionArgs &a, int sm_count, cudaStream_t s);
struct PairResult {
    int32_t score, end_query, end_ref, beg_query, beg_ref, n_ops;
    uint32_t flags;
    int32_t reserved;
};
cudaError_t launch_pair_results(int64_t n, const int64_t *qoff, const int64_t *t_beg, const int64_t *t_end,
                                const AlnDesc *aln, const AlnOut *out, int n_aln, const uint32_t *spill, int max_ops,
                                PairResult *res, uint32_t *ops, unsigned long long *n_ok, int sm_count, cudaStream_t s);

constexpr int FILL_THREADS = 128;
constexpr int OVER_CAP = 256;
constexpr int N_ROW_CLASSES = 5;
__host__ __device__ constexpr int row_class(int k) { return k == 0 ? 13 : k == 1 ? 19 : k == 2 ? 25 : k == 3 ? 32 : 38; }
constexpr int ROW_CLASSES[N_ROW_CLASSES] = { row_class(0), row_class(1), row_class(2), row_class(3), row_class(4) };
constexpr int QMAX_FAST = FG * 38;
constexpr int TMAX_FAST = 4000;
constexpr int TLONG_STEP = 1024;
constexpr int TMAX_PACKED = 1000000;
constexpr int N_LONG_KEYS = (TMAX_PACKED - TMAX_FAST + TLONG_STEP - 1) / TLONG_STEP;
constexpr int KEYS_PER_CLASS = N_LONG_KEYS + TMAX_FAST + 2;
constexpr int FILL_CHUNK_BLOCKS = 32;

size_t fill_smem_bytes(int tw_stride);
size_t trace_tile_bytes(int R);
int tw_stride_for(int nblk_max);

constexpr int BIN_KEYS = (N_ROW_CLASSES + 1) * KEYS_PER_CLASS;
__host__ __device__ inline int bin_key(int rank, int tlen)
{
    if (rank == N_ROW_CLASSES) return rank * KEYS_PER_CLASS;
    return rank * KEYS_PER_CLASS + (tlen > TMAX_FAST ? (TMAX_PACKED - tlen) / TLONG_STEP : N_LONG_KEYS + TMAX_FAST - tlen);
}
__host__ __device__ inline int key_tlen(int key_in_class)
{
    return key_in_class < N_LONG_KEYS ? TMAX_PACKED - key_in_class * TLONG_STEP : TMAX_FAST - (key_in_class - N_LONG_KEYS);
}
__host__ __device__ inline int bin_rank(int qlen, int tlen, bool force_generic)
{
    if (force_generic || qlen > QMAX_FAST || tlen > TMAX_PACKED) return N_ROW_CLASSES;
    for (int k = 0; k < N_ROW_CLASSES; ++k) if (qlen <= FG * row_class(k)) return k;
    return N_ROW_CLASSES;
}
cudaError_t launch_bin_classify(const BinArgs &a, int sm_count, cudaStream_t s);
cudaError_t launch_bin_scatter(const BinArgs &a, int sm_count, cudaStream_t s);
cudaError_t launch_seq_pull(const uint8_t *host_seq4, const AlnDesc *aln, const int64_t *src_off, int n_aln, uint8_t *dst, int sm_count,
                            cudaStream_t s);
cudaError_t launch_result_index(const AlnOut *out, int n_aln, int64_t n_reads, uint8_t *flags, int32_t *ridx, unsigned long long *n_ok,
                                int sm_count, cudaStream_t s);
cudaError_t launch_fill(int R, const KernelArgs &a, cudaStream_t s);
cudaError_t launch_trace(int R, const KernelArgs &a, cudaStream_t s, int sm_count, int *launches);
cudaError_t launch_generic(const GenericArgs &a, int n_slots, cudaStream_t s);
cudaError_t launch_alu_peak(uint32_t *out, int iters, int blocks, int threads, cudaStream_t s);

}
```

Baseline: 273.7 million.

## Fuse trace init and round-0 scan replay into the fill kernel epilogue

The fill kernel now performs the per-alignment trace initialization and the round-0 end-cell scan itself. It replays from checkpoints still resident in the warp and advances traceback directly, using staged targets and query codes kept in shared memory when the window fits. This removes the separate trace_init kernel, the fillres global buffer round-trip and the round-0 scan-only replay launch. The cost is more shared memory and register pressure in the fill kernel, which may lower its occupancy, plus serialized per-alignment work inside the fill warps.

```diff
diff --git a/fade_b200/csrc/fadegpu.cu b/fade_b200/csrc/fadegpu.cu
--- a/fade_b200/csrc/fadegpu.cu
+++ b/fade_b200/csrc/fadegpu.cu
@@ -116,7 +116,6 @@
     uint8_t *h_seq = nullptr, *d_seq = nullptr;
     AlnOut *h_out = nullptr, *d_out = nullptr;
     uint32_t *d_flags = nullptr;
-    uint2 *d_fillres = nullptr;
     int64_t cap_items = 0, cap_seq = 0;
     std::vector<Launch> plan;
     int64_t n_reads = 0, n_aln = 0, n_items = 0, seq_bytes = 0;
@@ -376,7 +375,6 @@
             a.seq = seq;
             a.ref = pt.ref;
             a.ck = ln.d_ck;
-            a.fillres = b->d_fillres + (size_t)L.item_first * 32;
             a.aln_flags = b->d_flags + L.aln_first;
             a.out = b->d_out + L.aln_first;
             a.k = c->k;
@@ -751,7 +749,6 @@
     free_host(v.beg_ref); free_host(v.end_ref); free_host(v.win_start); free_host(v.n_ops); free_host(v.ops);
     free_host(b->h_aln); free_host(b->h_items); free_host(b->h_seq); free_host(b->h_out); free_host(b->h_ridx);
     free_dev(b->d_aln); free_dev(b->d_items); free_dev(b->d_seq); free_dev(b->d_out); free_dev(b->d_flags);
-    free_dev(b->d_fillres);
     free_dev(b->d_in_seq4); free_dev(b->d_in_seq_off); free_dev(b->d_in_pos); free_dev(b->d_in_lq); free_dev(b->d_in_tid);
     free_dev(b->d_in_alen); free_dev(b->d_in_cl); free_dev(b->d_in_cr); free_dev(b->d_key); free_dev(b->d_tlen); free_dev(b->d_start);
     free_dev(b->d_aln_start); free_dev(b->d_hist); free_dev(b->d_keybase); free_dev(b->d_cursor);
@@ -797,7 +794,6 @@
     H(&b->h_out, n * sizeof(AlnOut)); H(&b->h_ridx, n * 4);
     D(&b->d_aln, n * sizeof(AlnDesc)); D(&b->d_items, (size_t)b->cap_items * sizeof(WarpItem));
     D(&b->d_out, n * sizeof(AlnOut)); D(&b->d_flags, n * 4);
-    D(&b->d_fillres, (size_t)b->cap_items * 32 * sizeof(uint2));
     D(&b->d_in_seq4, (size_t)max_seq_bytes + 32 * n + 16); D(&b->d_in_seq_off, (n + 1) * 8); D(&b->d_in_pos, n * 8);
     D(&b->d_in_read, n * 4);
     D(&b->d_in_lq, n * 4); D(&b->d_in_tid, n * 4); D(&b->d_in_alen, n * 4); D(&b->d_in_cl, n * 4); D(&b->d_in_cr, n * 4);
diff --git a/fade_b200/csrc/kernels.cu b/fade_b200/csrc/kernels.cu
--- a/fade_b200/csrc/kernels.cu
+++ b/fade_b200/csrc/kernels.cu
@@ -10,6 +10,8 @@
 constexpr unsigned FULL = 0xffffffffu;
 
 #define FADE_SMALL_KERNEL __launch_bounds__(128, 16)
+
+__host__ __device__ inline size_t fill_tw_bytes(int tw_stride) { return (size_t)(FILL_THREADS / FG) * tw_stride * 2; }
 
 
 __device__ __forceinline__ uint32_t stage_targets(const KernelArgs &a, const AlnDesc &da, const AlnDesc &db, int g,
@@ -48,76 +50,23 @@
     wild = w;
 }
 
+__device__ __forceinline__ void stage_block_targets(const KernelArgs &a, const AlnDesc &da, const AlnDesc &db, int blk0,
+                                                    int blk1, int g, uint16_t *tws)
+{
+    for (int x = g; x < FBLK + FG - 1; x += FG) {
+        const int j0 = blk0 * FBLK - (FG - 1) + x, j1 = blk1 * FBLK - (FG - 1) + x;
+        const int ca = (j0 >= 0 && j0 < da.tlen) ? ref_code(a.ref.planes, da.gstart + j0) : C_TPAD;
+        const int cb = (j1 >= 0 && j1 < db.tlen) ? ref_code(a.ref.planes, db.gstart + j1) : C_TPAD;
+        tws[x] = (uint16_t)t_sel(ca, cb);
+    }
+}
+
 __device__ __forceinline__ AlnDesc load_desc(const KernelArgs &a, int idx)
 {
     AlnDesc d;
     if (idx < a.n_aln) d = a.aln[idx];
     else { d.gstart = 0; d.seq_off = 0; d.tlen = 0; d.qlen = 0; d.clip_left = d.clip_right = 0; d.read = -1; d.pad = 0; }
     return d;
-}
-
-template <int R, int STEP>
-__global__ void __launch_bounds__(FILL_THREADS, (R <= 19 ? 5 : 1)) sw_fill_kernel(const KernelArgs a)
-{
-    extern __shared__ __align__(16) unsigned char smem_raw[];
-    const int lane = threadIdx.x & 31, wib = threadIdx.x >> 5;
-    const int g = lane & (FG - 1), q = lane >> 3;
-    const int w = blockIdx.x * (FILL_THREADS / 32) + wib;
-    if (w >= a.n_items) return;
-    const WarpItem item = a.items[w];
-    const int ia = item.first + 2 * q, ib = ia + 1;
-    const AlnDesc da = load_desc(a, ia), db = load_desc(a, ib);
-    uint16_t *tw = reinterpret_cast<uint16_t *>(smem_raw) + (size_t)(wib * 4 + q) * a.tw_stride;
-    const int nblk = item.nblk;
-    const SwConsts k = a.k;
-
-    uint32_t H[R], E[R], qs[query_words<R, STEP>()];
-    uint32_t wild;
-    stage_pair<R, STEP>(a, da, db, g, nblk, tw, qs, nullptr, wild);
-#pragma unroll
-    for (int r = 0; r < R; ++r) { H[r] = 0u; E[r] = k.neg_o; }
-    uint32_t hu_prev = 0u, fout = k.neg_o, M = 0u, Mprev = 0u;
-    int blk_lo = 0, blk_hi = 0;
-    __syncwarp();
-
-    constexpr int CW = ck_words<R>();
-    uint32_t *ckw = a.ck + item.ck_off + lane;
-    const uint16_t *twp = tw + (FG - g);
-    const int nsteps = item.nsteps;
-    for (int c = 0; c < nblk; ++c) {
-        if (c > 0 && (c % FILL_CHUNK_BLOCKS) == 0) {
-            __syncwarp();
-            wild |= stage_targets(a, da, db, g, c * FBLK, FBLK * min(nblk - c, FILL_CHUNK_BLOCKS), tw);
-            twp = tw + (FG - g) - c * FBLK;
-            __syncwarp();
-        }
-        const int ulim = min(FBLK, nsteps - c * FBLK);
-#pragma unroll 2
-        for (int u = 0; u < ulim; ++u) {
-            const int t = c * FBLK + u;
-            uint32_t hu = __shfl_up_sync(FULL, H[R - 1], 1, FG);
-            uint32_t fin = __shfl_up_sync(FULL, fout, 1, FG);
-            if (g == 0) { hu = 0u; fin = k.neg_o; }
-            const uint32_t ts = twp[t];
-            score_step<R, STEP>(H, E, qs, M, ts, hu_prev, fin, fout, k);
-            hu_prev = hu;
-        }
-        if (c + 1 < nblk) {
-            uint32_t *p = ckw + (size_t)c * CW * 32;
-#pragma unroll
-            for (int r = 0; r < R; ++r) { p[r * 32] = H[r]; p[(R + r) * 32] = E[r]; }
-            p[(2 * R) * 32] = hu_prev;
-            p[(2 * R + 1) * 32] = fout;
-        }
-        if (M != Mprev) {
-            if ((M ^ Mprev) & 0xffffu) blk_lo = c;
-            if ((M ^ Mprev) >> 16) blk_hi = c;
-            Mprev = M;
-        }
-    }
-    a.fillres[(size_t)w * 32 + lane] = make_uint2(M, (uint32_t)blk_lo | ((uint32_t)blk_hi << 16));
-    if ((wild & 1u) && ia < a.n_aln) a.aln_flags[ia] = 1u;
-    if ((wild & 2u) && ib < a.n_aln) a.aln_flags[ib] = 1u;
 }
 
 __device__ __forceinline__ unsigned long long pack_req(int aln, int blk, uint32_t scanmask)
@@ -135,47 +84,50 @@
     __device__ __forceinline__ int tcode(int j) const { return ref_code(planes, gstart + j); }
 };
 
-template <int R>
-__global__ void FADE_SMALL_KERNEL trace_init_kernel(const KernelArgs a)
-{
-    for (int aln = blockIdx.x * blockDim.x + threadIdx.x; aln < a.n_aln; aln += gridDim.x * blockDim.x) {
-        a.out[aln].read = -1;
-        a.out[aln].flags = 0x80000000u;
-        if (a.aln_flags[aln] & 1u) continue;
-        const AlnDesc d = a.aln[aln];
-        LaneCtl &c = a.state[aln];
-        const int w = aln >> 3, q = (aln & 7) >> 1, half = aln & 1;
-        const uint2 *fr = a.fillres + (size_t)w * 32 + q * FG;
-        for (int g = 0; g < FG; ++g) {
-            const uint2 v = fr[g];
-            c.best[g] = half ? lane_hi(v.x) : lane_lo(v.x);
-            c.blk[g] = half ? (int)(v.y >> 16) : (int)(v.y & 0xffffu);
-        }
-        ctl_init(c, d.qlen, d.tlen);
-        if (c.phase != 2 && a.tags_only && !score_may_accept(c.S, d.clip_left, d.clip_right, a.min_length)) {
-            AlnOut o;
-            o.score = c.S; o.end_query = o.end_ref = o.beg_query = o.beg_ref = 0; o.n_ops = 0;
-            o.flags = R_ALIGNED | R_SCORE_ONLY; o.read = d.read;
-            for (int k = 0; k < OPS_CAP; ++k) o.ops[k] = 0;
-            a.out[aln] = o;
-        } else if (c.phase == 2) {
-            AlnOut o;
-            finalize_result(c, o, d.read, d.clip_left, d.clip_right, a.min_length);
-            a.out[aln] = o;
-        } else {
-            const unsigned slot = atomicAdd(&a.qcount[0], 1u);
-            a.queue[0][slot] = pack_req(aln, c.next_blk, ctl_scanmask(c));
-        }
-    }
-}
-
-template <int R, int MODE, int STEP = 0>
+template <int R, int MODE, int STEP, class Hit>
+__device__ __forceinline__ void replay_step(uint32_t (&H)[R], uint32_t (&E)[R], const uint32_t (&qs)[query_words<R, STEP>()],
+                                            uint32_t &hu_prev, uint32_t &fout, uint32_t ts, const SwConsts &k,
+                                            uint32_t e_init, int g, uint32_t *tile, int u, bool store, int S0, int S1,
+                                            bool &need0, bool &need1, Hit &&hit)
+{
+    constexpr int RW = trace_words<R>();
+    uint32_t hu = __shfl_up_sync(FULL, H[R - 1], 1, FG);
+    uint32_t fin = __shfl_up_sync(FULL, fout, 1, FG);
+    if (g == 0) { hu = 0u; fin = e_init; }
+    uint32_t cmax = 0u;
+    if constexpr (MODE == 2) {
+        score_step<R, STEP>(H, E, qs, cmax, ts, hu_prev, fin, fout, k);
+    } else {
+        uint32_t trw[RW];
+        if (MODE == 0) trace_step_tagged<R>(H, E, qs, ts, hu_prev, fin, fout, k, trw, cmax);
+        else trace_step_plain<R>(H, E, qs, ts, hu_prev, fin, fout, k, trw, cmax);
+        if (store) {
+#pragma unroll
+            for (int w = 0; w < RW; ++w) tile[tile_index<R>(u, g, w)] = trw[w];
+        }
+    }
+    hu_prev = hu;
+    if (need0 && lane_lo(cmax) == S0) {
+        need0 = false;
+        int fr = 0;
+#pragma unroll
+        for (int r = R - 1; r >= 0; --r) if (lane_lo(H[r]) == S0) fr = r;
+        hit(0, fr);
+    }
+    if (need1 && lane_hi(cmax) == S1) {
+        need1 = false;
+        int fr = 0;
+#pragma unroll
+        for (int r = R - 1; r >= 0; --r) if (lane_hi(H[r]) == S1) fr = r;
+        hit(1, fr);
+    }
+}
+
+template <int R, bool TAGGED>
 __device__ __forceinline__ void replay_round(const KernelArgs &a, int round, unsigned warp0, unsigned nwarps,
                                              uint16_t (*tws_all)[40])
 {
-    constexpr bool TAGGED = MODE == 0;
-    constexpr bool SCAN_ONLY = MODE == 2;
-    constexpr int RW = trace_words<R>();
+    constexpr int MODE = TAGGED ? 0 : 1, STEP = 0;
     constexpr int CW = ck_words<R>();
     constexpr int MUL = TAGGED ? 16 : 1;
     const int lane = threadIdx.x & 31, wib = threadIdx.x >> 5;
@@ -240,12 +192,7 @@
                 set_query<STEP>(qs, r, ca, cb);
             }
             __syncwarp();
-            for (int x = g; x < FBLK + FG - 1; x += FG) {
-                const int j0 = blk[0] * FBLK - (FG - 1) + x, j1 = blk[1] * FBLK - (FG - 1) + x;
-                const int ca = (j0 >= 0 && j0 < d[0].tlen) ? ref_code(a.ref.planes, d[0].gstart + j0) : C_TPAD;
-                const int cb = (j1 >= 0 && j1 < d[1].tlen) ? ref_code(a.ref.planes, d[1].gstart + j1) : C_TPAD;
-                tws[x] = (uint16_t)t_sel(ca, cb);
-            }
+            stage_block_targets(a, d[0], d[1], blk[0], blk[1], g, tws);
             __syncwarp();
         }
         uint32_t *tile = a.tiles + (size_t)pair * tile_words<R>();
@@ -253,51 +200,22 @@
         bool need0 = (smask[0] >> g) & 1u, need1 = (smask[1] >> g) & 1u;
         const uint16_t *twp = tws + (FG - 1 - g);
         for (int u = 0; u < FBLK; ++u) {
-            uint32_t hu = __shfl_up_sync(FULL, H[R - 1], 1, FG);
-            uint32_t fin = __shfl_up_sync(FULL, fout, 1, FG);
-            if (g == 0) { hu = 0u; fin = e_init; }
-            const uint32_t ts = twp[u];
-            uint32_t cmax = 0u;
-            if constexpr (SCAN_ONLY) {
-                score_step<R, STEP>(H, E, qs, cmax, ts, hu_prev, fin, fout, k);
-            } else {
-                uint32_t trw[RW];
-                if (TAGGED) trace_step_tagged<R>(H, E, qs, ts, hu_prev, fin, fout, k, trw, cmax);
-                else trace_step_plain<R>(H, E, qs, ts, hu_prev, fin, fout, k, trw, cmax);
-                if (store) {
-#pragma unroll
-                    for (int w = 0; w < RW; ++w) tile[tile_index<R>(u, g, w)] = trw[w];
-                }
-            }
-            hu_prev = hu;
-            if (need0 && lane_lo(cmax) == S[0]) {
-                need0 = false;
-                int fr = 0;
-#pragma unroll
-                for (int r = R - 1; r >= 0; --r) if (lane_lo(H[r]) == S[0]) fr = r;
-                a.state[aln[0]].fj[g] = blk[0] * FBLK + u - g;
-                a.state[aln[0]].fr[g] = fr;
-            }
-            if (need1 && lane_hi(cmax) == S[1]) {
-                need1 = false;
-                int fr = 0;
-#pragma unroll
-                for (int r = R - 1; r >= 0; --r) if (lane_hi(H[r]) == S[1]) fr = r;
-                a.state[aln[1]].fj[g] = blk[1] * FBLK + u - g;
-                a.state[aln[1]].fr[g] = fr;
-            }
-            if (SCAN_ONLY && !__any_sync(FULL, need0 || need1)) break;
-        }
-    }
-}
-
-template <int R, int MODE, int STEP = 0>
+            replay_step<R, MODE, STEP>(H, E, qs, hu_prev, fout, twp[u], k, e_init, g, tile, u, store, S[0], S[1],
+                                       need0, need1, [&](int L, int fr) {
+                                           a.state[aln[L]].fj[g] = blk[L] * FBLK + u - g;
+                                           a.state[aln[L]].fr[g] = fr;
+                                       });
+        }
+    }
+}
+
+template <int R, bool TAGGED>
 __global__ void __launch_bounds__(128) trace_replay_kernel(const KernelArgs a)
 {
     __shared__ uint16_t tws_all[16][40];
     if (blockIdx.x == 0 && threadIdx.x == 0) a.qcount[(a.round & 1) ^ 1] = 0u;
-    replay_round<R, MODE, STEP>(a, a.round, blockIdx.x * (blockDim.x >> 5) + (threadIdx.x >> 5),
-                                gridDim.x * (blockDim.x >> 5), tws_all);
+    replay_round<R, TAGGED>(a, a.round, blockIdx.x * (blockDim.x >> 5) + (threadIdx.x >> 5),
+                            gridDim.x * (blockDim.x >> 5), tws_all);
 }
 
 struct AdvanceSmem {
@@ -306,33 +224,17 @@
 };
 static_assert(sizeof(LaneCtl) % 4 == 0 && sizeof(AlnOut) % 4 == 0, "word-copyable");
 
-template <int R, bool SPILL>
-__device__ __forceinline__ void advance_round(const KernelArgs &a, int round, unsigned warp0, unsigned nwarps,
-                                              AdvanceSmem *smem_all)
-{
-    constexpr int RW = trace_words<R>();
+template <int R, bool SPILL, class Acc>
+__device__ __forceinline__ void advance_one(const KernelArgs &a, int round, int aln, const AlnDesc &d, const Acc &acc,
+                                            const uint32_t *tile, int sh, AdvanceSmem &sm)
+{
     constexpr int CTLW = (int)(sizeof(LaneCtl) / 4), OUTW = (int)(sizeof(AlnOut) / 4);
-    AdvanceSmem &sm = smem_all[threadIdx.x >> 5];
     const int rin = round & 1;
-    const unsigned cnt = a.qcount[rin];
-    const unsigned long long *queue = a.queue[rin];
     const int l = threadIdx.x & 31;
     const SwConsts &k = a.k;
-    const bool tile_valid = !(round == 0 && k.shortcut);
-    for (unsigned idx = warp0; idx < cnt; idx += nwarps) {
-        const int aln = (int)(uint32_t)(queue[idx] & 0xffffffffu);
-        const AlnDesc d = a.aln[aln];
-        LaneCtl &c = sm.ctl;
-        {
-            const uint32_t *src = reinterpret_cast<const uint32_t *>(&a.state[aln]);
-            uint32_t *dst = reinterpret_cast<uint32_t *>(&c);
-            for (int w = l; w < CTLW; w += 32) dst[w] = src[w];
-        }
-        __syncwarp();
-        const uint32_t *tile = a.tiles + (size_t)(idx >> 1) * tile_words<R>();
-        const int sh = 16 * (int)(idx & 1u);
-        GlobalAcc acc;
-        acc.seq = a.seq + d.seq_off; acc.qlen = d.qlen; acc.planes = a.ref.planes; acc.gstart = d.gstart;
+    const bool traced = tile != nullptr;
+    LaneCtl &c = sm.ctl;
+    {
         int go = 1;
         if (l == 0) {
             c.cur_blk = c.next_blk;
@@ -373,7 +275,7 @@
                     const bool valid = ii >= 0 && jj >= 0;
                     const int g = valid ? ii / R : 0, r = valid ? ii - g * R : 0;
                     const int t = jj + g;
-                    const bool inblk = valid && tile_valid && (t / FBLK) == cur_blk;
+                    const bool inblk = valid && traced && (t / FBLK) == cur_blk;
                     uint32_t nib = 0;
                     int sc = 0;
                     bool eq = false;
@@ -453,7 +355,7 @@
                 } else {
                     const int g = i / R, r = i - g * R;
                     const int t = j + g;
-                    if (t / FBLK != cur_blk || !tile_valid) { need = t / FBLK; break; }
+                    if (t / FBLK != cur_blk || !traced) { need = t / FBLK; break; }
                     const uint32_t nib = (tile[tile_index<R>(t % FBLK, g, r >> 2)] >> (sh + 4 * (r & 3))) & 0xfu;
                     if (mode == 1) {
                         if (!(nib & 2u)) { hval = gval + k.open; mode = 0; }
@@ -500,10 +402,204 @@
 }
 
 template <int R, bool SPILL>
+__device__ __forceinline__ void advance_round(const KernelArgs &a, int round, unsigned warp0, unsigned nwarps,
+                                              AdvanceSmem *smem_all)
+{
+    constexpr int CTLW = (int)(sizeof(LaneCtl) / 4);
+    AdvanceSmem &sm = smem_all[threadIdx.x >> 5];
+    const unsigned cnt = a.qcount[round & 1];
+    const unsigned long long *queue = a.queue[round & 1];
+    const int l = threadIdx.x & 31;
+    for (unsigned idx = warp0; idx < cnt; idx += nwarps) {
+        const int aln = (int)(uint32_t)(queue[idx] & 0xffffffffu);
+        const AlnDesc d = a.aln[aln];
+        {
+            const uint32_t *src = reinterpret_cast<const uint32_t *>(&a.state[aln]);
+            uint32_t *dst = reinterpret_cast<uint32_t *>(&sm.ctl);
+            for (int w = l; w < CTLW; w += 32) dst[w] = src[w];
+        }
+        __syncwarp();
+        GlobalAcc acc;
+        acc.seq = a.seq + d.seq_off; acc.qlen = d.qlen; acc.planes = a.ref.planes; acc.gstart = d.gstart;
+        advance_one<R, SPILL>(a, round, aln, d, acc, a.tiles + (size_t)(idx >> 1) * tile_words<R>(), 16 * (int)(idx & 1u), sm);
+    }
+}
+
+template <int R, bool SPILL>
 __global__ void FADE_SMALL_KERNEL trace_advance_kernel(const KernelArgs a)
 {
     __shared__ AdvanceSmem adv[4];
     advance_round<R, SPILL>(a, a.round, blockIdx.x * (blockDim.x >> 5) + (threadIdx.x >> 5), gridDim.x * (blockDim.x >> 5), adv);
+}
+
+template <int R, int STEP>
+__device__ __forceinline__ void fill_round0(const KernelArgs &a, int ia, const AlnDesc &da, const AlnDesc &db, int nblk,
+                                            const uint32_t *ckw, uint16_t *tw, const uint8_t *qc_warp,
+                                            const uint32_t (&qs)[query_words<R, STEP>()], uint32_t (&H)[R], uint32_t (&E)[R],
+                                            uint32_t M, int blk_lo, int blk_hi, uint32_t wild, AdvanceSmem &sm)
+{
+    const int lane = threadIdx.x & 31, g = lane & (FG - 1), q = lane >> 3;
+    const int first = ia - 2 * q, ib = ia + 1;
+    const SwConsts &k = a.k;
+    const int best0 = lane_lo(M), best1 = lane_hi(M);
+    int S0 = max(best0, 0), S1 = max(best1, 0);
+#pragma unroll
+    for (int o = 1; o < FG; o <<= 1) {
+        S0 = max(S0, __shfl_xor_sync(FULL, S0, o));
+        S1 = max(S1, __shfl_xor_sync(FULL, S1, o));
+        wild |= __shfl_xor_sync(FULL, wild, o);
+    }
+    int nb0 = best0 == S0 ? blk_lo : 0x7fffffff, nb1 = best1 == S1 ? blk_hi : 0x7fffffff;
+#pragma unroll
+    for (int o = 1; o < FG; o <<= 1) {
+        nb0 = min(nb0, __shfl_xor_sync(FULL, nb0, o));
+        nb1 = min(nb1, __shfl_xor_sync(FULL, nb1, o));
+    }
+    if (g == 0 && ia < a.n_aln) { a.out[ia].read = -1; a.out[ia].flags = 0x80000000u; }
+    if (g == 1 && ib < a.n_aln) { a.out[ib].read = -1; a.out[ib].flags = 0x80000000u; }
+    auto traced = [&](const AlnDesc &d, int idx, int S, uint32_t wl) {
+        return idx < a.n_aln && !wl && S > 0 && d.qlen > 0 && d.tlen > 0 &&
+               !(a.tags_only && !score_may_accept(S, d.clip_left, d.clip_right, a.min_length));
+    };
+    const bool scan0 = traced(da, ia, S0, wild & 1u), scan1 = traced(db, ib, S1, wild & 2u);
+    bool need0 = scan0 && best0 == S0 && blk_lo == nb0, need1 = scan1 && best1 == S1 && blk_hi == nb1;
+    int fj0 = 0, fr0 = 0, fj1 = 0, fr1 = 0;
+    if (__any_sync(FULL, need0 || need1)) {
+        const int b0 = scan0 ? nb0 : scan1 ? nb1 : nblk - 1, b1 = scan1 ? nb1 : b0;
+        const int c0 = (nblk - 1) / FILL_CHUNK_BLOCKS * FILL_CHUNK_BLOCKS;
+        const bool restage = min(b0, b1) < c0;
+        const uint16_t *tw0 = restage ? tw + (FG - 1 - g) : tw + (b0 - c0) * FBLK + FG - g;
+        const uint16_t *tw1 = restage ? tw0 : tw + (b1 - c0) * FBLK + FG - g;
+        __syncwarp();
+        if (restage) stage_block_targets(a, da, db, b0, b1, g, tw);
+        __syncwarp();
+        constexpr int CW = ck_words<R>();
+        const uint32_t *p0 = ckw + (size_t)(b0 > 0 ? b0 - 1 : 0) * CW * 32, *p1 = ckw + (size_t)(b1 > 0 ? b1 - 1 : 0) * CW * 32;
+        const bool z0 = b0 == 0, z1 = b1 == 0;
+        auto mix = [&](uint32_t w0, uint32_t w1) { return (w0 & 0xffffu) | (w1 & 0xffff0000u); };
+#pragma unroll
+        for (int r = 0; r < R; ++r) {
+            H[r] = mix(z0 ? 0u : p0[r * 32], z1 ? 0u : p1[r * 32]);
+            E[r] = mix(z0 ? k.neg_o : p0[(R + r) * 32], z1 ? k.neg_o : p1[(R + r) * 32]);
+        }
+        uint32_t hu_prev = mix(z0 ? 0u : p0[(2 * R) * 32], z1 ? 0u : p1[(2 * R) * 32]);
+        uint32_t fout = mix(z0 ? k.neg_o : p0[(2 * R + 1) * 32], z1 ? k.neg_o : p1[(2 * R + 1) * 32]);
+        for (int u = 0; u < FBLK; ++u) {
+            const uint32_t ts = (tw0[u] & 0x00ffu) | (tw1[u] & 0xff00u);
+            replay_step<R, 2, STEP>(H, E, qs, hu_prev, fout, ts, k, k.neg_o, g, nullptr, u, false, S0, S1, need0, need1,
+                                    [&](int L, int fr) {
+                                        if (L == 0) { fj0 = b0 * FBLK + u - g; fr0 = fr; }
+                                        else { fj1 = b1 * FBLK + u - g; fr1 = fr; }
+                                    });
+            if (!__any_sync(FULL, need0 || need1)) break;
+        }
+    }
+    LaneCtl &c = sm.ctl;
+    for (int x = 0; x < 8; ++x) {
+        const int aln = first + x;
+        if (aln >= a.n_aln) break;
+        const int src = (x >> 1) * FG + g, hi = x & 1;
+        const uint32_t Mx = __shfl_sync(FULL, M, src), wx = __shfl_sync(FULL, wild, src);
+        const int bx = __shfl_sync(FULL, hi ? blk_hi : blk_lo, src);
+        const int fjx = __shfl_sync(FULL, hi ? fj1 : fj0, src), frx = __shfl_sync(FULL, hi ? fr1 : fr0, src);
+        if ((wx >> hi) & 1u) continue;
+        if (lane < FG) { c.best[g] = hi ? lane_hi(Mx) : lane_lo(Mx); c.blk[g] = bx; c.fj[g] = fjx; c.fr[g] = frx; }
+        const AlnDesc d = a.aln[aln];
+        __syncwarp();
+        int walk = 0;
+        if (lane == 0) {
+            ctl_init(c, d.qlen, d.tlen);
+            if (c.phase != 2 && a.tags_only && !score_may_accept(c.S, d.clip_left, d.clip_right, a.min_length)) {
+                AlnOut o;
+                o.score = c.S; o.end_query = o.end_ref = o.beg_query = o.beg_ref = 0; o.n_ops = 0;
+                o.flags = R_ALIGNED | R_SCORE_ONLY; o.read = d.read;
+                for (int kk = 0; kk < OPS_CAP; ++kk) o.ops[kk] = 0;
+                a.out[aln] = o;
+            } else if (c.phase == 2) {
+                AlnOut o;
+                finalize_result(c, o, d.read, d.clip_left, d.clip_right, a.min_length);
+                a.out[aln] = o;
+            } else walk = 1;
+        }
+        if (__shfl_sync(FULL, walk, 0)) {
+            if (nblk <= FILL_CHUNK_BLOCKS) {
+                StagedAcc acc;
+                acc.tw = tw + ((x >> 1) - q) * a.tw_stride; acc.qc = qc_warp + (x >> 1) * FG * R; acc.lane = hi;
+                advance_one<R, true>(a, 0, aln, d, acc, nullptr, 0, sm);
+            } else {
+                GlobalAcc acc;
+                acc.seq = a.seq + d.seq_off; acc.qlen = d.qlen; acc.planes = a.ref.planes; acc.gstart = d.gstart;
+                advance_one<R, true>(a, 0, aln, d, acc, nullptr, 0, sm);
+            }
+        }
+        __syncwarp();
+    }
+}
+
+template <int R, int STEP>
+__global__ void __launch_bounds__(FILL_THREADS, (R <= 19 ? 5 : 1)) sw_fill_kernel(const KernelArgs a)
+{
+    extern __shared__ __align__(16) unsigned char smem_raw[];
+    const int lane = threadIdx.x & 31, wib = threadIdx.x >> 5;
+    const int g = lane & (FG - 1), q = lane >> 3;
+    const int w = blockIdx.x * (FILL_THREADS / 32) + wib;
+    if (w >= a.n_items) return;
+    const WarpItem item = a.items[w];
+    const int ia = item.first + 2 * q, ib = ia + 1;
+    const AlnDesc da = load_desc(a, ia), db = load_desc(a, ib);
+    uint16_t *tw = reinterpret_cast<uint16_t *>(smem_raw) + (size_t)(wib * 4 + q) * a.tw_stride;
+    const int nblk = item.nblk;
+    const SwConsts k = a.k;
+
+    uint32_t H[R], E[R], qs[query_words<R, STEP>()];
+    uint32_t wild;
+    uint8_t *qc_warp = smem_raw + fill_tw_bytes(a.tw_stride) + (FILL_THREADS / 32) * sizeof(AdvanceSmem) + (size_t)wib * 4 * FG * R;
+    stage_pair<R, STEP>(a, da, db, g, nblk, tw, qs, qc_warp + q * FG * R, wild);
+#pragma unroll
+    for (int r = 0; r < R; ++r) { H[r] = 0u; E[r] = k.neg_o; }
+    uint32_t hu_prev = 0u, fout = k.neg_o, M = 0u, Mprev = 0u;
+    int blk_lo = 0, blk_hi = 0;
+    __syncwarp();
+
+    constexpr int CW = ck_words<R>();
+    uint32_t *ckw = a.ck + item.ck_off + lane;
+    const uint16_t *twp = tw + (FG - g);
+    const int nsteps = item.nsteps;
+    for (int c = 0; c < nblk; ++c) {
+        if (c > 0 && (c % FILL_CHUNK_BLOCKS) == 0) {
+            __syncwarp();
+            wild |= stage_targets(a, da, db, g, c * FBLK, FBLK * min(nblk - c, FILL_CHUNK_BLOCKS), tw);
+            twp = tw + (FG - g) - c * FBLK;
+            __syncwarp();
+        }
+        const int ulim = min(FBLK, nsteps - c * FBLK);
+#pragma unroll 2
+        for (int u = 0; u < ulim; ++u) {
+            const int t = c * FBLK + u;
+            uint32_t hu = __shfl_up_sync(FULL, H[R - 1], 1, FG);
+            uint32_t fin = __shfl_up_sync(FULL, fout, 1, FG);
+            if (g == 0) { hu = 0u; fin = k.neg_o; }
+            const uint32_t ts = twp[t];
+            score_step<R, STEP>(H, E, qs, M, ts, hu_prev, fin, fout, k);
+            hu_prev = hu;
+        }
+        if (c + 1 < nblk) {
+            uint32_t *p = ckw + (size_t)c * CW * 32;
+#pragma unroll
+            for (int r = 0; r < R; ++r) { p[r * 32] = H[r]; p[(R + r) * 32] = E[r]; }
+            p[(2 * R) * 32] = hu_prev;
+            p[(2 * R + 1) * 32] = fout;
+        }
+        if (M != Mprev) {
+            if ((M ^ Mprev) & 0xffffu) blk_lo = c;
+            if ((M ^ Mprev) >> 16) blk_hi = c;
+            Mprev = M;
+        }
+    }
+    if ((wild & 1u) && ia < a.n_aln) a.aln_flags[ia] = 1u;
+    if ((wild & 2u) && ib < a.n_aln) a.aln_flags[ib] = 1u;
+    AdvanceSmem *adv = reinterpret_cast<AdvanceSmem *>(smem_raw + fill_tw_bytes(a.tw_stride));
+    fill_round0<R, STEP>(a, ia, da, db, nblk, ckw, tw, qc_warp, qs, H, E, M, blk_lo, blk_hi, wild, adv[wib]);
 }
 
 template <int R, bool TAGGED>
@@ -516,7 +612,7 @@
         __syncthreads();
         if (threadIdx.x == 0) a.qcount[(r & 1) ^ 1] = 0u;
         __syncthreads();
-        replay_round<R, TAGGED ? 0 : 1>(a, r, threadIdx.x >> 5, blockDim.x >> 5, tws_all);
+        replay_round<R, TAGGED>(a, r, threadIdx.x >> 5, blockDim.x >> 5, tws_all);
         __threadfence_block();
         __syncthreads();
         advance_round<R, true>(a, r, threadIdx.x >> 5, blockDim.x >> 5, adv);
@@ -1072,12 +1168,15 @@
 
 int tw_stride_for(int nblk_max) { return (FBLK * std::min(nblk_max, FILL_CHUNK_BLOCKS) + FG + 1 + 7) & ~7; }
 
-size_t fill_smem_bytes(int tw_stride) { return (size_t)(FILL_THREADS / FG) * tw_stride * 2; }
+size_t fill_smem_bytes(int tw_stride, int R)
+{
+    return fill_tw_bytes(tw_stride) + (FILL_THREADS / 32) * sizeof(AdvanceSmem) + (size_t)(FILL_THREADS / FG) * FG * R;
+}
 
 template <int R, int STEP>
 static cudaError_t launch_fill_tf(const KernelArgs &a, cudaStream_t s)
 {
-    const size_t smem = fill_smem_bytes(a.tw_stride);
+    const size_t smem = fill_smem_bytes(a.tw_stride, R);
     cudaError_t e = cudaFuncSetAttribute(sw_fill_kernel<R, STEP>, cudaFuncAttributeMaxDynamicSharedMemorySize, (int)smem);
     if (e != cudaSuccess) return e;
     const int wpb = FILL_THREADS / 32;
@@ -1100,12 +1199,10 @@
 static cudaError_t launch_trace_tt(KernelArgs a, cudaStream_t s, int sm_count, int *launches)
 {
     const int n = a.n_aln;
-    int grid = std::min((n + 127) / 128, sm_count * 8);
-    trace_init_kernel<R><<<grid, 128, 0, s>>>(a);
-    int nl = 1;
+    int nl = 0;
     constexpr int FULL_ROUNDS = 10;
     const int quads = (n + 7) / 8;
-    int r = 0;
+    int r = 1;
     for (; r < a.max_rounds && r < FULL_ROUNDS; ++r) {
         a.round = r;
         const int g1 = std::min((quads + 3) / 4, r < 3 ? sm_count * 4 : sm_count);
@@ -1116,13 +1213,7 @@
             cudaMemcpy(qc, a.qcount, sizeof(qc), cudaMemcpyDeviceToHost);
             fprintf(stderr, "[fadegpu] round %d: %u requests (n_aln %d)\n", r, qc[r & 1], n);
         }
-        if (r == 0 && a.k.shortcut) {
-            const int step = score_step_for(a.k);
-            if (step == 2) trace_replay_kernel<R, 2, 2><<<std::max(g1, 1), 128, 0, s>>>(a);
-            else if (step == 1) trace_replay_kernel<R, 2, 1><<<std::max(g1, 1), 128, 0, s>>>(a);
-            else trace_replay_kernel<R, 2, 0><<<std::max(g1, 1), 128, 0, s>>>(a);
-        }
-        else trace_replay_kernel<R, TAGGED ? 0 : 1><<<std::max(g1, 1), 128, 0, s>>>(a);
+        trace_replay_kernel<R, TAGGED><<<std::max(g1, 1), 128, 0, s>>>(a);
         if (a.ops_spill) trace_advance_kernel<R, true><<<std::max(g2, 1), 128, 0, s>>>(a);
         else trace_advance_kernel<R, false><<<std::max(g2, 1), 128, 0, s>>>(a);
         nl += 2;
diff --git a/fade_b200/csrc/kernels.cuh b/fade_b200/csrc/kernels.cuh
--- a/fade_b200/csrc/kernels.cuh
+++ b/fade_b200/csrc/kernels.cuh
@@ -38,7 +38,6 @@
     const uint8_t *seq;
     RefDev ref;
     uint32_t *ck;
-    uint2 *fillres;
     uint32_t *aln_flags;
     AlnOut *out;
     SwConsts k;
@@ -157,7 +156,7 @@
 constexpr int KEYS_PER_CLASS = N_LONG_KEYS + TMAX_FAST + 2;
 constexpr int FILL_CHUNK_BLOCKS = 32;
 
-size_t fill_smem_bytes(int tw_stride);
+size_t fill_smem_bytes(int tw_stride, int R);
 size_t trace_tile_bytes(int R);
 int tw_stride_for(int nblk_max);
 
```

Measured after the change: 278.4 million, median of 6. 1.02x the previous value.
